# vLAR-group/OGC

Measured on AMD Instinct MI355X. Metric: point-clouds/sec (8192 pts) segnet fwd+bwd, higher is better.
Workload: dtype f32; 1 GPU; C4 KITTI-SF train_seg unsup: segnet_kitti fwd + OGC loss (dynamic+smooth+invariance) + bwd + Adam, 4 samples x 4 views x 8192 pts per GPU; n_point=8192, n_slot=10, parallelism=dp1, optimizer_stepped=True

## Files before the change

include/ogc_ops.h:

```cpp
#ifndef OGC_OPS_H
#define OGC_OPS_H

#ifdef __cplusplus
extern "C" {
#endif

typedef void *ogc_stream_t;
typedef unsigned short ogc_bf16_t;

enum {
    OGC_OK = 0,
    OGC_ERR_INVALID_ARG = -1,
    OGC_ERR_LAUNCH = -2,
    OGC_ERR_UNSUPPORTED = -3
};

#define OGC_VERSION 205
int ogc_version(void);
int ogc_distance_contracted(void);
int ogc_set_deterministic(int on);
int ogc_get_deterministic(void);
const char *ogc_last_error(void);

int ogc_furthest_point_sampling(int b, int n, int m, const float *xyz, float *temp,
                                int *idx, ogc_stream_t stream);

int ogc_furthest_point_sampling_chain(int b, int n, int m, const float *xyz, float *temp, int *idx,
                                      const int *ties_in, int *ties_out, ogc_stream_t stream);

int ogc_gather_points(int b, int c, int n, int npoints, const float *points, const int *idx,
                      float *out, ogc_stream_t stream);

int ogc_gather_points_grad(int b, int c, int n, int npoints, const float *grad_out,
                           const int *idx, float *grad_points, ogc_stream_t stream);

int ogc_knn(int b, int n, int m, int k, const float *unknown, const float *known,
            float *dist2, int *idx, ogc_stream_t stream);

int ogc_three_nn(int b, int n, int m, const float *unknown, const float *known, float *dist2,
                 int *idx, ogc_stream_t stream);

int ogc_three_interpolate(int b, int c, int m, int n, const float *points, const int *idx,
                          const float *weight, float *out, ogc_stream_t stream);

int ogc_three_interpolate_grad(int b, int c, int n, int m, const float *grad_out,
                               const int *idx, const float *weight, float *grad_points,
                               ogc_stream_t stream);

int ogc_group_points(int b, int c, int n, int npoints, int nsample, const float *points,
                     const int *idx, float *out, ogc_stream_t stream);

int ogc_group_points_grad(int b, int c, int n, int npoints, int nsample, const float *grad_out,
                          const int *idx, float *grad_points, ogc_stream_t stream);

int ogc_ball_query(int b, int n, int m, float radius, int nsample, const float *new_xyz,
                   const float *xyz, int *idx, ogc_stream_t stream);


int ogc_knn_clamped(int b, int n, int m, int k, float radius, const float *unknown,
                    const float *known, float *dist, int *idx, ogc_stream_t stream);

long long ogc_cell_grid_bytes(int b, int n);
int ogc_cell_grid_build(int b, int n, float radius, const float *xyz, void *grid, ogc_stream_t stream);
int ogc_ball_query_cells(int b, int n, float radius, int nsample, const float *xyz, const void *grid, float grid_radius, int *idx,
                         ogc_stream_t stream);
int ogc_knn_clamped_cells(int b, int n, int k, float radius, const float *xyz, void *grid, float grid_radius, float *dist, int *idx,
                          ogc_stream_t stream);

int ogc_adam_max_tensors(void);
int ogc_adam_chunk(void);
int ogc_adam_step(int n_tensors, int n_chunks, const long long *table, const int *chunks, const void *const *grad_ptrs,
                  float *step_snapshot, int *flag, double lr, double beta1, double beta2, double eps, double weight_decay,
                  ogc_stream_t stream);

int ogc_kabsch_rotation(int nb, const float *S, float *R, int *valid, ogc_stream_t stream);

int ogc_group_concat(int b, int c, int n, int npoints, int nsample, const float *xyz, const float *new_xyz,
                     const float *points, const int *idx, float *out, ogc_stream_t stream);

int ogc_group_concat_grad(int b, int c, int n, int npoints, int nsample, const float *grad_out, const int *idx,
                          float *grad_points, ogc_stream_t stream);

int ogc_group_linear_fwd(int b, int m, int n, int npoints, int nsample, int groups, const float *P, const int *idx,
                         const float *rel, const float *wx, float *y, double *stats, ogc_stream_t stream);
int ogc_group_linear_fwd_direct(int b, int m, int cf, int n, int npoints, int nsample, int groups, const float *feats,
                                const int *idx, const float *rel, const float *w, float *y, double *stats, ogc_stream_t stream);
int ogc_group_linear_fwd_direct_h(int b, int m, int cf, int n, int npoints, int nsample, int groups, const float *feats,
                                  const int *idx, const float *rel, const float *w, ogc_bf16_t *y, double *stats, ogc_stream_t stream);
int ogc_group_linear_bwd(int b, int m, int n, int npoints, int nsample, const float *grad_y, const int *idx,
                         const float *rel, float *grad_p, float *dwx, ogc_stream_t stream);

int ogc_group_reverse_chunk(int n, int npoints, int nsample);
int ogc_group_reverse(int b, int n, int npoints, int nsample, const int *idx, int *rev_start, unsigned short *rev_pos,
                      unsigned short *heads, ogc_stream_t stream);
int ogc_group_points_grad_rev(int b, int c, int n, int npoints, int nsample, const float *grad_out, const int *rev_start,
                              const unsigned short *rev_pos, const unsigned short *heads, float *grad_points,
                              ogc_stream_t stream);

int ogc_group_points_grad_rev_dwx(int b, int c, int n, int npoints, int nsample, const float *grad_out, const int *rev_start,
                                  const unsigned short *rev_pos, const unsigned short *heads, const float *rel,
// ... 61 lines not shown
                              ogc_stream_t stream);

int ogc_group_norm_maxpool_bwd_sparse(int b, int c, int p, int s, int groups, int relu, const float *x,
                                      const float *x_at_argmax, const float *gamma, const float *mean, const float *rstd, const float *out, const int *argmax,
                                      const float *grad_out, float *coef2, float *inj, float *grad_gamma,
                                      float *grad_beta, double *ws, ogc_stream_t stream);
int ogc_conv1x1_wgrad_moments_pooled(int b, int cin, int cout, int hw, int relu, int nsample, const float *y_prev,
                                     const float *pa, const float *pb, const float *y, const float *coef2,
                                     const float *inj, float *moments, ogc_stream_t stream);
int ogc_conv1x1_dgrad_adjoint_pooled(int b, int cin, int cout, int hw, int relu, int nsample, const float *w, const float *y,
                                     const float *coef2, const float *inj, const float *y_prev, const float *pa,
                                     const float *pb, const float *coef, float *grad_prev, ogc_stream_t stream);

int ogc_mlp_chain_pool_supported(int c0, int c1, int c2, int c3, int nsample);
int ogc_mlp_chain_pool(int b, int c0, int c1, int c2, int c3, int p, int nsample, const float *x, const float *wt1,
                       const float *b1, const float *wt2, const float *b2, const float *wt3, const float *b3, float *out,
                       ogc_stream_t stream);

int ogc_corr_layer_pool_supported(int cf, int c1, int c2, int c3, int nsample);
int ogc_corr_layer_pool(int b, int cf, int c1, int c2, int c3, int n1, int n2, int nsample, const float *pos1,
                        const float *pos2, const float *feat1, const float *feat2, const int *idx, const float *wt1,
                        const float *b1, const float *wt2, const float *b2, const float *wt3, const float *b3, float *out,
                        ogc_stream_t stream);

long long ogc_slot_masks_ws_floats(int b, int d, int n, int k);
int ogc_slot_masks_fwd(int b, int d, int n, int k, float temperature, const float *feats, const float *slots,
                       float *mask, ogc_stream_t stream);
int ogc_slot_masks_bwd(int b, int d, int n, int k, float temperature, const float *feats, const float *slots,
                       const float *mask, const float *grad_mask, float *grad_feats, float *grad_slots, float *ws,
                       ogc_stream_t stream);

int ogc_group_norm_stats_slots(void);
int ogc_group_norm_bwd_slots(void);
int ogc_group_norm_fwd(int b, int c, int hw, int groups, float eps, int relu, const float *x,
                       const float *gamma, const float *beta, float *y, float *mean, float *rstd,
                       double *ws, ogc_stream_t stream);
int ogc_group_norm_bwd(int b, int c, int hw, int groups, int relu, const float *x, const float *gamma,
                       const float *beta, const float *mean, const float *rstd, const float *grad_y,
                       float *grad_x, float *grad_gamma, float *grad_beta, double *ws, ogc_stream_t stream);

int ogc_group_norm_maxpool_fwd(int b, int c, int p, int s, int groups, float eps, int relu, const float *x,
                               const float *gamma, const float *beta, float *out, int *argmax, float *mean,
                               float *rstd, double *ws, ogc_stream_t stream);
int ogc_group_norm_maxpool_bwd(int b, int c, int p, int s, int groups, int relu, const float *x,
                               const float *gamma, const float *mean, const float *rstd, const float *out,
                               const int *argmax, const float *grad_out, float *grad_x, float *grad_gamma,
                               float *grad_beta, double *ws, ogc_stream_t stream);
int ogc_group_norm_maxpool_bwd_ext(int b, int c, int p, int s, int groups, int relu, const float *x,
                                   const float *x_at_argmax, const float *gamma, const float *mean, const float *rstd,
                                   const float *out, const int *argmax, const float *grad_out, float *grad_x,
                                   float *grad_gamma, float *grad_beta, double *ws, ogc_stream_t stream);

int ogc_batch_norm_fwd(int b, int c, int hw, float eps, int relu, int training, float momentum, const float *x,
                       const float *gamma, const float *beta, float *running_mean, float *running_var, float *y,
                       float *mean, float *rstd, double *ws, const double *stats, int slots, ogc_stream_t stream);
int ogc_batch_norm_bwd(int b, int c, int hw, int relu, int training, const float *x, const float *gamma,
                       const float *beta, const float *mean, const float *rstd, const float *grad_y, float *grad_x,
                       float *grad_gamma, float *grad_beta, double *ws, ogc_stream_t stream);
int ogc_batch_norm_maxpool_fwd(int b, int c, int p, int s, float eps, int relu, int training, float momentum,
                               const float *x, const float *gamma, const float *beta, float *running_mean,
                               float *running_var, float *out, int *argmax, float *mean, float *rstd, double *ws,
                               const double *stats, int slots, ogc_stream_t stream);
int ogc_batch_norm_maxpool_bwd(int b, int c, int p, int s, int relu, int training, const float *x, const float *gamma,
                               const float *mean, const float *rstd, const float *out, const int *argmax,
                               const float *grad_out, float *grad_x, float *grad_gamma, float *grad_beta, double *ws,
                               ogc_stream_t stream);

int ogc_conv1x1_wgrad(int b, int cin, int cout, int hw, const float *x, const float *dy, float *dw,
                      ogc_stream_t stream);

int ogc_conv1x1_gemm(int b, int M, int K, int hw, int transpose_a, const float *w, const float *in,
                     float *out, ogc_stream_t stream);

int ogc_conv1x1_gn_slots(void);
int ogc_conv1x1_gemm_stats_supported(int b, int M, int K, int hw, int affine);
int ogc_conv1x1_gemm_stream_supported(int b, int M, int K, int hw);
int ogc_conv1x1_gemm_any(int b, int M, int K, int hw, int transpose_a, const float *w, const float *in, float *out,
                         ogc_stream_t stream);

int ogc_set_matmul_precision(int bf16);
int ogc_conv1x1_gemm_gnstats(int b, int M, int K, int hw, int groups, const float *w, const float *in, float *out,
                             double *stats, ogc_stream_t stream);

int ogc_group_norm_coeffs(int b, int c, int hw, int groups, float eps, const float *x, const float *gamma,
                          const float *beta, const double *stats, int slots, double *ws, float *mean, float *rstd,
                          float *a, float *bb, ogc_stream_t stream);
int ogc_conv1x1_gemm_affine(int b, int M, int K, int hw, int relu, int groups, const float *w, const float *in,
                            const float *pa, const float *pb, float *out, double *stats, ogc_stream_t stream);
int ogc_conv1x1_wgrad_affine(int b, int cin, int cout, int hw, int relu, const float *x, const float *pa,
                             const float *pb, const float *dy, float *dw, ogc_stream_t stream);
int ogc_conv1x1_wgrad_affine_pooled(int b, int cin, int cout, int hw, int relu, int nsample, const float *x, const float *pa,
                                    const float *pb, const float *y, const float *coef2, const float *inj, float *dw,
                                    ogc_stream_t stream);
int ogc_conv1x1_dgrad_pooled(int b, int cin, int cout, int hw, int nsample, const float *w, const float *y, const float *coef2,
                             const float *inj, float *grad_z, ogc_stream_t stream);

int ogc_group_norm_fwd_stats(int b, int c, int hw, int groups, float eps, int relu, const float *x,
                             const float *gamma, const float *beta, float *y, float *mean, float *rstd,
                             const double *stats, int slots, ogc_stream_t stream);
int ogc_group_norm_maxpool_fwd_stats(int b, int c, int p, int s, int groups, float eps, int relu, const float *x,
                                     const float *gamma, const float *beta, float *out, int *argmax, float *mean,
                                     float *rstd, const double *stats, int slots, ogc_stream_t stream);

int ogc_conv1x1_gemm_affine_pool(int b, int M, int K, int hw, int relu, int groups, int nsample, const float *w,
                                 const float *in, const float *pa, const float *pb, const float *next_gamma,
                                 float *out, double *stats, float *yext, int *aext, ogc_stream_t stream);
int ogc_group_norm_pool_extremes(int b, int c, int p, int s, int groups, float eps, int relu, const float *yext,
                                 const int *aext, const float *gamma, const float *beta, float *out, int *argmax,
                                 float *mean, float *rstd, const double *stats, int slots, ogc_stream_t stream);

int ogc_chamfer_terms(int b, int n1, int n2, int p, const float *p1, const float *pc2, const int *idx12, const int *idx21,
                      float *dist1, float *dist2, ogc_stream_t stream);
int ogc_chamfer_terms_grad(int b, int n1, int n2, int p, const float *p1, const float *pc2, const int *idx12, const int *idx21,
                           const float *g1, const float *g2, float *grad_p1, ogc_stream_t stream);

int ogc_gather_xyz_pair(int b, int n, int m, const float *xyz, const int *idx, float *out, float *out_t, ogc_stream_t stream);
int ogc_flow_advance(int b, int n, float scale, const float *cur, const float *delta, const float *ref, float *out_delta,
                     float *out_new, float *out_new_t, float *out_flow, ogc_stream_t stream);
int ogc_linear_cn(int b, int cin, int cout, int n, const float *x, const float *weight, const float *bias, float *y,
                  ogc_stream_t stream);
int ogc_three_nn_weights(int b, int n, int mode, const float *dist2, float *weight, ogc_stream_t stream);
int ogc_soft_corr_flow(int b, int n1, int n2, int c, float support, const float *epsilon, const float *pc1, const float *pc2,
                       const float *f1, const float *f2, float *flow, ogc_stream_t stream);
int ogc_gru_reset(int b, int c, int cx, int n, int s, const float *rc, long long rc_batch_stride, const float *hx, float *out,
                  ogc_stream_t stream);
int ogc_gru_blend(int b, int c, int n, int s, const float *zc, long long zc_batch_stride, const float *qc,
                  long long qc_batch_stride, const float *h, long long h_batch_stride, float *out, ogc_stream_t stream);

int ogc_zero_arena_begin(void *base, int bytes, ogc_stream_t stream);
int ogc_zero_arena_end(void);

int ogc_group_linear_fwd_h(int b, int m, int n, int npoints, int nsample, int groups, const float *P, const int *idx,
                           const float *rel, const float *wx, ogc_bf16_t *y, double *stats, ogc_stream_t stream);
int ogc_group_linear_fwd_pt_h(int b, int m, int n, int npoints, int nsample, int groups, const float *Pt, const int *idx,
                              const float *rel, const float *wx, ogc_bf16_t *y, double *stats, ogc_stream_t stream);
int ogc_group_points_grad_rev_h(int b, int c, int n, int npoints, int nsample, const ogc_bf16_t *grad_out, const int *rev_start,
                                const unsigned short *rev_pos, const unsigned short *heads, float *grad_points,
                                ogc_stream_t stream);
int ogc_group_points_grad_rev_dwx_h(int b, int c, int n, int npoints, int nsample, const ogc_bf16_t *grad_out, const int *rev_start,
                                    const unsigned short *rev_pos, const unsigned short *heads, const float *rel,
                                    float *grad_points, float *dwx, ogc_stream_t stream);
int ogc_conv1x1_gemm_h(int b, int M, int K, int hw, int transpose_a, const float *w, const ogc_bf16_t *in, ogc_bf16_t *out,
                       ogc_stream_t stream);
int ogc_conv1x1_gemm_affine_h(int b, int M, int K, int hw, int relu, int groups, const float *w, const ogc_bf16_t *in,
                              const float *pa, const float *pb, ogc_bf16_t *out, double *stats, ogc_stream_t stream);
int ogc_conv1x1_gemm_affine_pool_h(int b, int M, int K, int hw, int relu, int groups, int nsample, const float *w,
                                   const ogc_bf16_t *in, const float *pa, const float *pb, const float *next_gamma,
                                   ogc_bf16_t *out, double *stats, float *yext, int *aext, ogc_stream_t stream);
int ogc_conv1x1_wgrad_xf_h(int b, int cin, int cout, int hw, const float *x, const ogc_bf16_t *dy, float *dw,
                           ogc_stream_t stream);
int ogc_conv1x1_wgrad_affine_h(int b, int cin, int cout, int hw, int relu, const ogc_bf16_t *x, const float *pa,
                               const float *pb, const ogc_bf16_t *dy, float *dw, ogc_stream_t stream);
int ogc_conv1x1_wgrad_affine_pooled_h(int b, int cin, int cout, int hw, int relu, int nsample, const ogc_bf16_t *x,
                                      const float *pa, const float *pb, const ogc_bf16_t *y, const float *coef2,
                                      const float *inj, float *dw, ogc_stream_t stream);
int ogc_conv1x1_dgrad_pooled_h(int b, int cin, int cout, int hw, int nsample, const float *w, const ogc_bf16_t *y,
                               const float *coef2, const float *inj, ogc_bf16_t *grad_z, ogc_stream_t stream);
int ogc_conv1x1_wgrad_moments_h(int b, int cin, int cout, int hw, int relu, const ogc_bf16_t *y_prev, const float *pa,
                                const float *pb, const ogc_bf16_t *grad_y, float *moments, ogc_stream_t stream);
int ogc_conv1x1_wgrad_moments_pooled_h(int b, int cin, int cout, int hw, int relu, int nsample, const ogc_bf16_t *y_prev,
                                       const float *pa, const float *pb, const ogc_bf16_t *y, const float *coef2,
                                       const float *inj, float *moments, ogc_stream_t stream);
int ogc_conv1x1_dgrad_adjoint_h(int b, int cin, int cout, int hw, int relu, const float *w, const ogc_bf16_t *grad_y,
                                const ogc_bf16_t *y_prev, const float *pa, const float *pb, const float *coef,
                                ogc_bf16_t *grad_prev, ogc_stream_t stream);
int ogc_conv1x1_dgrad_adjoint_pooled_h(int b, int cin, int cout, int hw, int relu, int nsample, const float *w,
// ... 16 lines not shown
```

ogc_amd/_lib.py:

```python
import ctypes
import os

_HERE = os.path.dirname(os.path.abspath(__file__))
FMAD = os.environ.get("OGC_FMAD", "0") == "1"
DETERMINISTIC = os.environ.get("OGC_DETERMINISTIC", "0") == "1"
LIB_PATH = os.path.join(_HERE, "csrc", "libogc_ops_fmad.so" if FMAD else "libogc_ops.so")

_vp = ctypes.c_void_p
_int = ctypes.c_int
_flt = ctypes.c_float
_dbl = ctypes.c_double
_ll = ctypes.c_longlong

SIGNATURES = {
    "ogc_set_deterministic": [_int],
    "ogc_group_linear_fwd_direct": [_int, _int, _int, _int, _int, _int, _int, _vp, _vp, _vp, _vp, _vp, _vp, _vp],
    "ogc_get_deterministic": [],
    "ogc_furthest_point_sampling": [_int, _int, _int, _vp, _vp, _vp, _vp],
    "ogc_furthest_point_sampling_chain": [_int, _int, _int, _vp, _vp, _vp, _vp, _vp, _vp],
    "ogc_gather_points": [_int, _int, _int, _int, _vp, _vp, _vp, _vp],
    "ogc_gather_points_grad": [_int, _int, _int, _int, _vp, _vp, _vp, _vp],
    "ogc_knn": [_int, _int, _int, _int, _vp, _vp, _vp, _vp, _vp],
    "ogc_three_nn": [_int, _int, _int, _vp, _vp, _vp, _vp, _vp],
    "ogc_three_interpolate": [_int, _int, _int, _int, _vp, _vp, _vp, _vp, _vp],
# ... 7 lines not shown
    "ogc_view_means_grad": [_int, _vp, _vp, _vp, _vp, _vp, _vp],
    "ogc_sum_ranges": [_int, _vp, _vp, _vp, _ll, _vp, _vp],
    "ogc_three_interpolate_grad_rev_bs": [_int, _int, _int, _int, _vp, _ll, _vp, _vp, _vp, _vp, _vp, _vp],
    "ogc_group_points_grad_rev": [_int, _int, _int, _int, _int, _vp, _vp, _vp, _vp, _vp, _vp],
    "ogc_group_points_grad_rev_dwx": [_int, _int, _int, _int, _int, _vp, _vp, _vp, _vp, _vp, _vp, _vp, _vp],
    "ogc_ball_query": [_int, _int, _int, _flt, _int, _vp, _vp, _vp, _vp],
    "ogc_knn_clamped": [_int, _int, _int, _int, _flt, _vp, _vp, _vp, _vp, _vp],
    "ogc_cell_grid_bytes": [_int, _int],
    "ogc_cell_grid_build": [_int, _int, _flt, _vp, _vp, _vp],
    "ogc_ball_query_cells": [_int, _int, _flt, _int, _vp, _vp, _flt, _vp, _vp],
    "ogc_knn_clamped_cells": [_int, _int, _int, _flt, _vp, _vp, _flt, _vp, _vp, _vp],
    "ogc_chamfer_terms": [_int, _int, _int, _int, _vp, _vp, _vp, _vp, _vp, _vp, _vp],
    "ogc_chamfer_terms_grad": [_int, _int, _int, _int, _vp, _vp, _vp, _vp, _vp, _vp, _vp, _vp],
    "ogc_gather_xyz_pair": [_int, _int, _int, _vp, _vp, _vp, _vp, _vp],
    "ogc_flow_advance": [_int, _int, _flt, _vp, _vp, _vp, _vp, _vp, _vp, _vp, _vp],
    "ogc_linear_cn": [_int, _int, _int, _int, _vp, _vp, _vp, _vp, _vp],
    "ogc_three_nn_weights": [_int, _int, _int, _vp, _vp, _vp],
    "ogc_soft_corr_flow": [_int, _int, _int, _int, _flt, _vp, _vp, _vp, _vp, _vp, _vp, _vp],
    "ogc_gru_reset": [_int, _int, _int, _int, _int, _vp, _ll, _vp, _vp, _vp],
    "ogc_gru_blend": [_int, _int, _int, _int, _vp, _ll, _vp, _ll, _vp, _ll, _vp, _vp],
    "ogc_zero_arena_begin": [_vp, _int, _vp],
    "ogc_zero_arena_end": [],
    "ogc_adam_max_tensors": [],
    "ogc_adam_chunk": [],
    "ogc_adam_step": [_int, _int, _vp, _vp, _vp, _vp, _vp, _dbl, _dbl, _dbl, _dbl, _dbl, _vp],
    "ogc_kabsch_rotation": [_int, _vp, _vp, _vp, _vp],
    "ogc_lsap_maximize": [_int, _int, _vp, _vp, _vp],
    "ogc_rigid_moments": [_int, _int, _int, _vp, _vp, _vp, _vp, _vp, _vp, _vp],
    "ogc_rigid_translation": [_int, _vp, _vp, _vp, _vp, _vp],
    "ogc_rigid_blend": [_int, _int, _int, _int, _int, _vp, _vp, _vp, _vp, _vp, _vp, _vp, _vp],
    "ogc_mask_iou": [_int, _int, _int, _vp, _vp, _vp, _vp, _vp],
    "ogc_matched_distance": [_int, _int, _int, _int, _int, _vp, _vp, _vp, _vp, _vp, _vp, _vp, _vp, _vp],
    "ogc_soft_nn_target": [_int, _int, _int, _int, _flt, _vp, _vp, _vp, _vp, _vp, _vp],
    "ogc_group_concat": [_int, _int, _int, _int, _int, _vp, _vp, _vp, _vp, _vp, _vp],
    "ogc_group_linear_fwd": [_int, _int, _int, _int, _int, _int, _vp, _vp, _vp, _vp, _vp, _vp, _vp],
    "ogc_group_linear_bwd": [_int, _int, _int, _int, _int, _vp, _vp, _vp, _vp, _vp, _vp],
    "ogc_group_concat_grad": [_int, _int, _int, _int, _int, _vp, _vp, _vp, _vp],
    "ogc_neighbour_consistency_fwd": [_int, _int, _int, _int, _int, _vp, _vp, _vp, _vp],
    "ogc_reverse_neighbours": [_int, _int, _int, _vp, _vp, _vp, _vp, _vp, _vp],
    "ogc_neighbour_consistency_bwd": [_int, _int, _int, _int, _int, _vp, _vp, _vp, _vp, _vp, _vp, _vp, _vp],
    "ogc_sym_eigvals": [_int, _int, _vp, _vp, _vp],
    "ogc_group_norm_fwd": [_int, _int, _int, _int, _flt, _int, _vp, _vp, _vp, _vp, _vp, _vp, _vp, _vp],
    "ogc_group_norm_bwd": [_int, _int, _int, _int, _int, _vp, _vp, _vp, _vp, _vp, _vp, _vp, _vp, _vp, _vp, _vp],
    "ogc_group_norm_maxpool_fwd": [_int, _int, _int, _int, _int, _flt, _int, _vp, _vp, _vp, _vp, _vp, _vp, _vp, _vp, _vp],
    "ogc_conv1x1_gemm": [_int, _int, _int, _int, _int, _vp, _vp, _vp, _vp],
    "ogc_attention_fwd": [_int, _int, _int, _int, _int, _flt, _vp, _int, _vp, _int, _vp, _int, _vp, _vp, _vp],
    "ogc_attention_bwd": [_int, _int, _int, _int, _int, _flt, _vp, _int, _vp, _int, _vp, _int, _vp, _vp, _vp, _vp, _int,
                          _vp, _int, _vp, _int, _vp],
    "ogc_conv1x1_gemm_affine_pool": [_int, _int, _int, _int, _int, _int, _int, _vp, _vp, _vp, _vp, _vp, _vp, _vp, _vp, _vp,
                                     _vp],
    "ogc_group_norm_pool_extremes": [_int, _int, _int, _int, _int, _flt, _int, _vp, _vp, _vp, _vp, _vp, _vp, _vp, _vp, _vp,
                                     _int, _vp],
    "ogc_small_linear_fwd": [_int, _int, _int, _vp, _vp, _vp, _vp, _vp],
    "ogc_small_linear_bwd": [_int, _int, _int, _vp, _vp, _vp, _vp, _vp, _vp, _vp],
    "ogc_conv1x1_wgrad_moments": [_int, _int, _int, _int, _int, _vp, _vp, _vp, _vp, _vp, _vp],
    "ogc_gn_moments_combine": [_int, _int, _int, _int, _int, _vp, _vp, _vp, _vp, _vp, _vp, _vp, _vp, _vp, _vp, _vp, _vp],
    "ogc_conv1x1_dgrad_adjoint": [_int, _int, _int, _int, _int, _vp, _vp, _vp, _vp, _vp, _vp, _vp, _vp],
    "ogc_group_norm_maxpool_bwd_sparse": [_int, _int, _int, _int, _int, _int, _vp, _vp, _vp, _vp, _vp, _vp, _vp, _vp, _vp, _vp,
                                          _vp, _vp, _vp, _vp],
    "ogc_group_norm_maxpool_bwd_ext": [_int, _int, _int, _int, _int, _int, _vp, _vp, _vp, _vp, _vp, _vp, _vp, _vp, _vp, _vp,
                                       _vp, _vp, _vp],
    "ogc_conv1x1_wgrad_moments_pooled": [_int, _int, _int, _int, _int, _int, _vp, _vp, _vp, _vp, _vp, _vp, _vp, _vp],
    "ogc_conv1x1_dgrad_adjoint_pooled": [_int, _int, _int, _int, _int, _int, _vp, _vp, _vp, _vp, _vp, _vp, _vp, _vp, _vp, _vp],
    "ogc_mlp_chain_pool_supported": [_int, _int, _int, _int, _int],
    "ogc_mlp_chain_pool": [_int, _int, _int, _int, _int, _int, _int, _vp, _vp, _vp, _vp, _vp, _vp, _vp, _vp, _vp],
    "ogc_corr_layer_pool_supported": [_int, _int, _int, _int, _int],
    "ogc_corr_layer_pool": [_int, _int, _int, _int, _int, _int, _int, _int, _vp, _vp, _vp, _vp, _vp, _vp, _vp, _vp, _vp, _vp,
                            _vp, _vp, _vp],
    "ogc_slot_masks_ws_floats": [_int, _int, _int, _int],
    "ogc_slot_masks_fwd": [_int, _int, _int, _int, _flt, _vp, _vp, _vp, _vp],
    "ogc_slot_masks_bwd": [_int, _int, _int, _int, _flt, _vp, _vp, _vp, _vp, _vp, _vp, _vp, _vp],
    "ogc_conv1x1_gn_slots": [],
    "ogc_conv1x1_gemm_stats_supported": [_int, _int, _int, _int, _int],
    "ogc_conv1x1_gemm_stream_supported": [_int, _int, _int, _int],
    "ogc_conv1x1_gemm_any": [_int, _int, _int, _int, _int, _vp, _vp, _vp, _vp],
    "ogc_set_matmul_precision": [_int],
    "ogc_group_norm_stats_slots": [],
    "ogc_group_norm_bwd_slots": [],
    "ogc_group_norm_coeffs": [_int, _int, _int, _int, _flt, _vp, _vp, _vp, _vp, _int, _vp, _vp, _vp, _vp, _vp, _vp],
    "ogc_conv1x1_gemm_affine": [_int, _int, _int, _int, _int, _int, _vp, _vp, _vp, _vp, _vp, _vp, _vp],
    "ogc_conv1x1_wgrad_affine": [_int, _int, _int, _int, _int, _vp, _vp, _vp, _vp, _vp, _vp],
    "ogc_conv1x1_wgrad_affine_pooled": [_int, _int, _int, _int, _int, _int, _vp, _vp, _vp, _vp, _vp, _vp, _vp, _vp],
    "ogc_conv1x1_dgrad_pooled": [_int, _int, _int, _int, _int, _vp, _vp, _vp, _vp, _vp, _vp],
    "ogc_batch_norm_fwd": [_int, _int, _int, _flt, _int, _int, _flt, _vp, _vp, _vp, _vp, _vp, _vp, _vp, _vp, _vp, _vp,
                           _int, _vp],
    "ogc_batch_norm_bwd": [_int, _int, _int, _int, _int, _vp, _vp, _vp, _vp, _vp, _vp, _vp, _vp, _vp, _vp, _vp],
    "ogc_batch_norm_maxpool_fwd": [_int, _int, _int, _int, _flt, _int, _int, _flt, _vp, _vp, _vp, _vp, _vp, _vp, _vp,
                                   _vp, _vp, _vp, _vp, _int, _vp],
    "ogc_batch_norm_maxpool_bwd": [_int, _int, _int, _int, _int, _int, _vp, _vp, _vp, _vp, _vp, _vp, _vp, _vp, _vp,
                                   _vp, _vp, _vp],
    "ogc_conv1x1_gemm_gnstats": [_int, _int, _int, _int, _int, _vp, _vp, _vp, _vp, _vp],
    "ogc_group_norm_fwd_stats": [_int, _int, _int, _int, _flt, _int, _vp, _vp, _vp, _vp, _vp, _vp, _vp, _int, _vp],
    "ogc_group_norm_maxpool_fwd_stats": [_int, _int, _int, _int, _int, _flt, _int, _vp, _vp, _vp, _vp, _vp, _vp, _vp,
                                         _vp, _int, _vp],
    "ogc_conv1x1_wgrad": [_int, _int, _int, _int, _vp, _vp, _vp, _vp],
    "ogc_group_norm_maxpool_bwd": [_int, _int, _int, _int, _int, _int, _vp, _vp, _vp, _vp, _vp, _vp, _vp, _vp, _vp, _vp,
                                   _vp, _vp],
}

for _n in ("ogc_group_linear_fwd", "ogc_group_points_grad_rev", "ogc_conv1x1_gemm", "ogc_conv1x1_gemm_affine",
           "ogc_conv1x1_gemm_affine_pool", "ogc_conv1x1_wgrad_affine", "ogc_conv1x1_wgrad_affine_pooled",
           "ogc_conv1x1_dgrad_pooled", "ogc_conv1x1_wgrad_moments", "ogc_conv1x1_wgrad_moments_pooled",
           "ogc_conv1x1_dgrad_adjoint", "ogc_conv1x1_dgrad_adjoint_pooled", "ogc_group_norm_bwd",
           "ogc_group_norm_maxpool_bwd_sparse", "ogc_group_points_grad_rev_dwx"):
    SIGNATURES[_n + "_h"] = SIGNATURES[_n]
SIGNATURES["ogc_group_linear_fwd_direct_h"] = SIGNATURES["ogc_group_linear_fwd_direct"]
SIGNATURES["ogc_conv1x1_wgrad_xf_h"] = SIGNATURES["ogc_conv1x1_wgrad"]
SIGNATURES["ogc_group_linear_fwd_pt_h"] = SIGNATURES["ogc_group_linear_fwd"]

HEADER_VERSION = 205
_lib = None
_fns = {}


class OgcOpsError(RuntimeError):
    pass


def load():
    global _lib
    if _lib is None:
        if not os.path.exists(LIB_PATH):
            raise OgcOpsError(
                "libogc_ops.so not found at %s — build it with `python ogc_amd/csrc/build.py` "
                "(there is no CPU fallback)" % LIB_PATH)
        L = ctypes.CDLL(LIB_PATH)
        for name, argtypes in SIGNATURES.items():
            fn = getattr(L, name)
            fn.argtypes = argtypes
            fn.restype = _int
        L.ogc_version.restype = _int
        if L.ogc_version() != HEADER_VERSION:
            raise OgcOpsError("libogc_ops.so at %s is version %d, this package binds version %d of include/ogc_ops.h — rebuild it "
                              "with `python ogc_amd/csrc/build.py --force`" % (LIB_PATH, L.ogc_version(), HEADER_VERSION))
        L.ogc_distance_contracted.restype = _int
        if bool(L.ogc_distance_contracted()) != FMAD:
            raise OgcOpsError("%s evaluates distances %s, OGC_FMAD asked for the other form" %
                              (LIB_PATH, "contracted (fma)" if L.ogc_distance_contracted() else "un-contracted"))
        L.ogc_slot_masks_ws_floats.restype = ctypes.c_longlong
        L.ogc_cell_grid_bytes.restype = ctypes.c_longlong
        L.ogc_last_error.restype = ctypes.c_char_p
        L.ogc_set_deterministic(1 if DETERMINISTIC else 0)
        _lib = L
    return _lib


def set_deterministic(on):
    global DETERMINISTIC
    DETERMINISTIC = bool(on)
    load().ogc_set_deterministic(1 if on else 0)


CALL_COUNTS = None

ROCTX_NAMES = {
    "ogc_furthest_point_sampling": "K1 furthest_point_sampling", "ogc_furthest_point_sampling_chain": "K1 furthest_point_sampling (chain)",
    "ogc_gather_points": "K2 gather_points", "ogc_gather_points_grad": "K3 gather_points_grad",
    "ogc_knn": "K4 knn", "ogc_knn_clamped": "K4 knn (+ sqrt + radius clamp)", "ogc_knn_clamped_cells": "K4 knn (shared cell grid)",
    "ogc_three_nn": "K5 three_nn", "ogc_three_interpolate": "K6 three_interpolate",
    "ogc_three_interpolate_grad": "K7 three_interpolate_grad", "ogc_three_interpolate_grad_rev": "K7 three_interpolate_grad (gather form)",
    "ogc_three_interpolate_grad_rev_bs": "K7 three_interpolate_grad (gather form)",
    "ogc_group_points": "K8 group_points", "ogc_group_points_grad": "K9 group_points_grad",
    "ogc_group_points_grad_rev": "K9 group_points_grad (gather form)",
    "ogc_ball_query": "K10 ball_query", "ogc_ball_query_cells": "K10 ball_query (shared cell grid)",
}
_roctx = None


def _roctx_lib():
    global _roctx
    if _roctx is None:
        _roctx = False
        if os.environ.get("OGC_ROCTX", "0") == "1":
            for name in ("librocprofiler-sdk-roctx.so", "libroctx64.so"):
                try:
                    lib = ctypes.CDLL(os.path.join(os.environ.get("ROCM_PATH", "/opt/rocm"), "lib", name))
                    lib.roctxRangePushA.argtypes = [ctypes.c_char_p]
                    lib.roctxRangePushA.restype = ctypes.c_int
                    lib.roctxRangePop.restype = ctypes.c_int
                    _roctx = lib
                    break
                except (OSError, AttributeError):
                    continue
    return _roctx


def call(name, *args):
    if CALL_COUNTS is not None:
        CALL_COUNTS[name] += 1
    fn = _fns.get(name)
    if fn is None:
        fn = _fns[name] = getattr(load(), name)
    tx = _roctx_lib()
# ... 13 lines not shown
```

ogc_amd/csrc/build.py:

```python
import os
import subprocess
import sys
from concurrent.futures import ThreadPoolExecutor

HERE = os.path.dirname(os.path.abspath(__file__))
SOURCES = ["api.hip", "det.hip", "knn.hip", "ball_query.hip", "fps.hip", "gather_group.hip", "interpolate.hip", "kabsch.hip", "small_solvers.hip", "neighbour_loss.hip", "soft_nn.hip", "seg_loss.hip", "group_norm.hip", "batch_norm.hip", "grid.hip", "conv1x1.hip", "conv1x1_h.hip", "conv1x1_wgrad.hip", "attention.hip", "slot_masks.hip", "small_linear.hip", "loss_glue.hip", "mlp_chain.hip", "gn_fused_bwd.hip", "adam.hip", "gemm_chunk.hip", "chamfer.hip", "flow_step.hip"]
HEADERS = ["ogc_common.h", "grid.h", "conv_stage.h", "conv1x1_shared.h", "act_io.h", "conv1x1_epilogue.h", os.path.join("..", "..", "include", "ogc_ops.h")]
LIB = os.path.join(HERE, "libogc_ops.so")
FMAD_SOURCES = ["knn.hip", "ball_query.hip", "fps.hip", "grid.hip"]
LIB_FMAD = os.path.join(HERE, "libogc_ops_fmad.so")
HIPCC = os.environ.get("HIPCC", "/opt/rocm/bin/hipcc")
FLAGS = [
    "--offload-arch=gfx950", "-O3", "-std=c++17", "-fPIC",
    "-ffp-contract=off",
    "-munsafe-fp-atomics",
    "-mllvm", "-amdgpu-mfma-vgpr-form=1",
    "-Wall", "-Wno-unused-function",
]


def _newer(target, deps):
    if not os.path.exists(target):
        return True
    t = os.path.getmtime(target)
    return any(os.path.getmtime(d) > t for d in deps)


def build(force=False, verbose=False):
    hdrs = [os.path.join(HERE, h) for h in HEADERS] + [os.path.abspath(__file__)]
    objs, objs_fmad, jobs = [], [], []
    for s in SOURCES:
        src = os.path.join(HERE, s)
        obj = os.path.join(HERE, s.replace(".hip", ".o"))
        objs.append(obj)
        if force or _newer(obj, [src] + hdrs):
            jobs.append([HIPCC] + FLAGS + ["-c", src, "-o", obj])
        if s in FMAD_SOURCES:
            obj_f = os.path.join(HERE, s.replace(".hip", ".fmad.o"))
            objs_fmad.append(obj_f)
            if force or _newer(obj_f, [src] + hdrs):
                jobs.append([HIPCC] + FLAGS + ["-DOGC_FMAD=1", "-c", src, "-o", obj_f])
        else:
            objs_fmad.append(obj)

    def run(cmd):
        if verbose:
            print(" ".join(cmd), flush=True)
        subprocess.check_call(cmd)

    with ThreadPoolExecutor(max_workers=min(8, max(1, len(jobs)))) as ex:
        list(ex.map(run, jobs))
    if force or jobs or _newer(LIB, objs):
        run([HIPCC, "--offload-arch=gfx950", "-shared", "-fPIC", "-o", LIB] + objs)
    if force or jobs or _newer(LIB_FMAD, objs_fmad):
        run([HIPCC, "--offload-arch=gfx950", "-shared", "-fPIC", "-o", LIB_FMAD] + objs_fmad)
    return LIB


if __name__ == "__main__":
    print(build(force="--force" in sys.argv, verbose="--verbose" in sys.argv))
```

ogc_amd/csrc/conv1x1.hip:

```cpp
#include "conv1x1_shared.h"
#include "act_io.h"
#include "conv1x1_epilogue.h"

int ogc_g_matmul_bf16 = 0;


namespace {


template <bool TRANSPOSE_A, int KQ, bool STATS, bool PRO, bool BF, bool POOL = false, typename IT = float, typename OT = float>
__global__ __launch_bounds__(WG_WAVES *OGC_WAVE) void conv1x1_gemm_kernel(int M, int K, int hw, int groups,
                                                                          const float *__restrict__ w,
                                                                          const IT *__restrict__ in,
                                                                          OT *__restrict__ out,
                                                                          double *__restrict__ stats,
                                                                          const float *__restrict__ pa,
                                                                          const float *__restrict__ pb, int pro_relu,
                                                                          PoolOut pool = PoolOut()) {
    extern __shared__ __attribute__((aligned(16))) float a_lds[];
    __shared__ double s_stats[STATS ? 64 : 1];
    __shared__ __attribute__((aligned(16))) float s_sign[POOL ? 64 : 4];
    const int lane = threadIdx.x & 63, wave = threadIdx.x >> 6;
    const int j = lane & 15, kk = lane >> 4;
    const int b = blockIdx.y;
    const int p0 = (blockIdx.x * WG_WAVES + wave) * 64;
    const int Kq = (K + 3) >> 2, a_ld = ogc_a_ld(Kq);
    const bool live = p0 < hw;
    const IT *inb = in + (size_t)b * K * hw;
    OT *outb = out + (size_t)b * M * hw;
    if (STATS && threadIdx.x < 2 * groups) s_stats[threadIdx.x] = 0.0;

    float4 xin[KQ];
#pragma unroll
    for (int q = 0; q < KQ; ++q) {
        const int row = q * 4 + kk;
        xin[q] = (live && q < Kq && row < K) ? ogc_ld4(inb + (size_t)row * hw + p0 + 4 * j) : make_float4(0.f, 0.f, 0.f, 0.f);
    }
    if (PRO) {
        constexpr int CH = 8;
#pragma unroll
        for (int q0 = 0; q0 < KQ; q0 += CH) {
            float ca[CH], cb[CH];
#pragma unroll
            for (int u = 0; u < CH; ++u) {
                const int q = q0 + u, row = q * 4 + kk;
                const bool have = q < KQ && live && q < Kq && row < K;
                ca[u] = have ? pa[(size_t)b * K + row] : 0.f;
                cb[u] = have ? pb[(size_t)b * K + row] : 0.f;
            }
#pragma unroll
            for (int u = 0; u < CH; ++u) {
                const int q = q0 + u;
                if (q < KQ) {
                    float4 v = xin[q];
                    v.x = fmaf(ca[u], v.x, cb[u]); v.y = fmaf(ca[u], v.y, cb[u]);
                    v.z = fmaf(ca[u], v.z, cb[u]); v.w = fmaf(ca[u], v.w, cb[u]);
                    if (pro_relu) { v.x = fmaxf(v.x, 0.f); v.y = fmaxf(v.y, 0.f); v.z = fmaxf(v.z, 0.f); v.w = fmaxf(v.w, 0.f); }
                    xin[q] = v;
                }
            }
        }
    }
    constexpr int GQ = (KQ + 3) / 4;
    v4s xb[BF ? GQ : 1][4];
    if constexpr (BF) {
#pragma unroll
        for (int g = 0; g < GQ; ++g) {
            float4 r[4];
#pragma unroll
            for (int i = 0; i < 4; ++i) r[i] = 4 * g + i < KQ ? xin[4 * g + i] : make_float4(0.f, 0.f, 0.f, 0.f);
            xb[g][0] = ogc_pack_bf16(r[0].x, r[1].x, r[2].x, r[3].x);
            xb[g][1] = ogc_pack_bf16(r[0].y, r[1].y, r[2].y, r[3].y);
            xb[g][2] = ogc_pack_bf16(r[0].z, r[1].z, r[2].z, r[3].z);
            xb[g][3] = ogc_pack_bf16(r[0].w, r[1].w, r[2].w, r[3].w);
        }
    }
    const int cpg = STATS ? M / groups : 1;
    for (int m0 = 0; m0 < M; m0 += 64) {
        __syncthreads();
        if constexpr (BF) {
            v4s *a_bf = reinterpret_cast<v4s *>(a_lds);
            const int Gq = (Kq + 3) >> 2;
            for (int t = threadIdx.x; t < Gq * 256; t += WG_WAVES * OGC_WAVE) {
                const int kr = t & 3, mi = (t >> 2) & 63, g = t >> 8;
                const int m = m0 + mi;
// ... 71 lines not shown
#pragma unroll
        for (int q = 0; q < KQ; ++q) {
            if (q < Kq) {
                float av[4];
#pragma unroll
                for (int a = 0; a < 4; ++a) av[a] = a_lds[(a * 16 + j) * a_ld + q * 4 + kk];
#pragma unroll
                for (int a = 0; a < 4; ++a) {
                    if (a < nblk) {
                        acc[a][0] = __builtin_amdgcn_mfma_f32_16x16x4f32(av[a], xin[q].x, acc[a][0], 0, 0, 0);
                        acc[a][1] = __builtin_amdgcn_mfma_f32_16x16x4f32(av[a], xin[q].y, acc[a][1], 0, 0, 0);
                        acc[a][2] = __builtin_amdgcn_mfma_f32_16x16x4f32(av[a], xin[q].z, acc[a][2], 0, 0, 0);
                        acc[a][3] = __builtin_amdgcn_mfma_f32_16x16x4f32(av[a], xin[q].w, acc[a][3], 0, 0, 0);
                    }
                }
            }
        }
        }
        if (live) {
            if constexpr (sizeof(OT) == 2 && (STATS || POOL)) {
#pragma unroll
                for (int a = 0; a < 4; ++a)
#pragma unroll
                    for (int c = 0; c < 4; ++c)
#pragma unroll
                        for (int r = 0; r < 4; ++r) acc[a][c][r] = ogc_as_stored<OT>(acc[a][c][r]);
            }
#pragma unroll
            for (int a = 0; a < 4; ++a)
#pragma unroll
                for (int r = 0; r < 4; ++r) {
                    const int m = m0 + a * 16 + kk * 4 + r;
                    if (m < M) {
                        const float4 o = make_float4(acc[a][0][r], acc[a][1][r], acc[a][2][r], acc[a][3][r]);
                        ogc_st4(outb + (size_t)m * hw + p0 + 4 * j, o);
                    }
                }
            if constexpr (POOL) {
                const int centres = hw / pool.s;
                const int centre = (p0 + 4 * j) / pool.s;
                const size_t o0 = ((size_t)b * M + m0 + kk * 4) * centres + centre;
                if (pool.s == 64) ogc_pool_extremes_epilogue<16>(acc, nblk, s_sign, j, kk, m0, M, centres, 64, pool.yext + o0, pool.aext + o0);
                else if (pool.s == 32) ogc_pool_extremes_epilogue<8>(acc, nblk, s_sign, j, kk, m0, M, centres, 32, pool.yext + o0, pool.aext + o0);
                else ogc_pool_extremes_epilogue<4>(acc, nblk, s_sign, j, kk, m0, M, centres, 16, pool.yext + o0, pool.aext + o0);
            }
            if (STATS) {
#pragma unroll
                for (int a = 0; a < 4; ++a) {
                    if (a < nblk) {
                        float sm = 0.f, sq = 0.f;
#pragma unroll
                        for (int r = 0; r < 4; ++r)
#pragma unroll
                            for (int c = 0; c < 4; ++c) {
                                const float v = acc[a][c][r];
                                sm += v;
                                sq += v * v;
                            }
                        sm += ogc_dpp_f32<0xB1>(sm); sq += ogc_dpp_f32<0xB1>(sq);
                        sm += ogc_dpp_f32<0x4E>(sm); sq += ogc_dpp_f32<0x4E>(sq);
                        sm += ogc_dpp_f32<0x141>(sm); sq += ogc_dpp_f32<0x141>(sq);
                        sm += ogc_dpp_f32<0x140>(sm); sq += ogc_dpp_f32<0x140>(sq);
                        const int m = m0 + a * 16 + kk * 4;
                        if (j == 0 && m < M) {
                            const int g = m / cpg;
                            atomicAdd(&s_stats[2 * g], (double)sm);
                            atomicAdd(&s_stats[2 * g + 1], (double)sq);
                        }
                    }
                }
            }
        }
    }
    if (STATS) {
        __syncthreads();
        if (threadIdx.x < 2 * groups) {
            const int slot = blockIdx.x % GN_SLOTS;
            double *dst = stats + ((size_t)slot * gridDim.y + b) * 2 * groups;
            atomicAdd(dst + threadIdx.x, s_stats[threadIdx.x]);
        }
    }
}

template <int KQ, bool PRO, bool EXACT, bool STATS = false, bool POOL = false, bool DUAL = false, bool TRANS = false>
__global__ __launch_bounds__(WG_WAVES *OGC_WAVE, DUAL ? 2 : 1) void conv1x1_gemm_stream_kernel(int M, int K, int hw, int ntiles,
                                                                                 const float *__restrict__ w,
                                                                                 const float *__restrict__ in,
                                                                                 float *__restrict__ out,
                                                                                 const float *__restrict__ pa,
                                                                                 const float *__restrict__ pb, int pro_relu,
                                                                                 int groups = 1, int nbatch = 1,
                                                                                 double *__restrict__ stats = nullptr,
                                                                                 PoolOut pool = PoolOut()) {
    extern __shared__ __attribute__((aligned(16))) float a_lds[];
    const int lane = threadIdx.x & 63, wave = __builtin_amdgcn_readfirstlane(threadIdx.x >> 6);
    const int j = lane & 15, kk = lane >> 4;
    const int Kq = (K + 3) >> 2, Mt = (M + 63) >> 6, a_ld = ogc_a_ld(Kq);
    const int tiles_per_img = hw >> 6;
    for (int mt = 0; mt < Mt; ++mt)
        ogc_stage_weight_tile<TRANS, WG_WAVES>(a_lds + (size_t)mt * 64 * a_ld, w, mt * 64, M, K, Kq);
    float *sgn_all = a_lds + (size_t)Mt * 64 * a_ld + (PRO ? WG_WAVES * 2 * FW_KQ_MAX * 4 : 0) + WG_WAVES * 4 * 16 * 2 * 2;
    if constexpr (POOL) {
        for (int t = threadIdx.x; t < Mt * 64; t += WG_WAVES * OGC_WAVE) sgn_all[t] = (t < M && pool.sign[t] < 0.f) ? -1.f : 1.f;
    }
    __syncthreads();
    const int nw = gridDim.x * WG_WAVES;
    const unsigned off_main = (unsigned)(kk * hw + 4 * j);
    const unsigned off_last = (unsigned)(min(kk, K - 1 - (Kq - 1) * 4) * hw + 4 * j);
    auto load_tile = [&](int t, float4(&x)[KQ]) {
        t = min(t, ntiles - 1);
        const int b = t / tiles_per_img, p0 = (t - b * tiles_per_img) * 64;
        const float *inb = in + (size_t)b * K * hw + p0;
#pragma unroll
        for (int q = 0; q < KQ; ++q)
            if (EXACT || q < Kq) {
                const float *rowq = inb + (size_t)(q * 4) * hw;
                x[q] = *reinterpret_cast<const float4 *>(rowq + ((EXACT ? q == KQ - 1 : q == Kq - 1) ? off_last : off_main));
            }
    };
    float *cw = a_lds + (size_t)Mt * 64 * a_ld + wave * (2 * KQ * 4);
    int coef_b = -1;
    double *sacc = reinterpret_cast<double *>(a_lds + (size_t)Mt * 64 * a_ld + (PRO ? WG_WAVES * 2 * FW_KQ_MAX * 4 : 0)) +
                   wave * (4 * 16 * 2);
    int stat_b = -1;
    auto flush_stats = [&]() {
        if constexpr (STATS) {
            if (stat_b >= 0) {
                const int cpg = M / groups;
                double *dst = stats + ((size_t)(blockIdx.x % GN_SLOTS) * nbatch + stat_b) * 2 * groups;
                if (lane < Mt * 16) {
                    const int m = (lane >> 4) * 64 + ((lane >> 2) & 3) * 16 + (lane & 3) * 4;
                    if (m < M) {
                        unsafeAtomicAdd(dst + 2 * (m / cpg), sacc[2 * lane]);
                        unsafeAtomicAdd(dst + 2 * (m / cpg) + 1, sacc[2 * lane + 1]);
                    }
                }
            }
            if (lane < 64) { sacc[2 * lane] = 0.0; sacc[2 * lane + 1] = 0.0; }
            __builtin_amdgcn_wave_barrier();
        }
    };
    auto compute_store = [&](int t, float4(&x)[KQ]) {
        const int b = t / tiles_per_img, p0 = (t - b * tiles_per_img) * 64;
        if constexpr (STATS) {
            if (b != stat_b) { flush_stats(); stat_b = b; }
        }
        if (PRO) {
            if (b != coef_b) {
                coef_b = b;
                for (int r = lane; r < KQ * 4; r += OGC_WAVE) {
                    cw[r] = r < K ? pa[(size_t)b * K + r] : 0.f;
                    cw[KQ * 4 + r] = r < K ? pb[(size_t)b * K + r] : 0.f;
                }
                __builtin_amdgcn_wave_barrier();
            }
#pragma unroll
            for (int q = 0; q < KQ; ++q) {
                if (EXACT || q < Kq) {
                    const float ca = cw[q * 4 + kk], cb = cw[KQ * 4 + q * 4 + kk];
                    float4 v = x[q];
                    v.x = fmaf(ca, v.x, cb); v.y = fmaf(ca, v.y, cb);
                    v.z = fmaf(ca, v.z, cb); v.w = fmaf(ca, v.w, cb);
                    if (pro_relu) { v.x = fmaxf(v.x, 0.f); v.y = fmaxf(v.y, 0.f); v.z = fmaxf(v.z, 0.f); v.w = fmaxf(v.w, 0.f); }
                    x[q] = v;
                }
            }
        }
        float *outb = out + (size_t)b * M * hw + p0;
        const unsigned off_out = (unsigned)(kk * 4 * hw + 4 * j);
        for (int mt = 0; mt < Mt; ++mt) {
            const float *at = a_lds + (size_t)mt * 64 * a_ld;
            const int nblk = EXACT ? 4 : min(4, (M - mt * 64 + 15) >> 4);
            v4f acc[4][4];
#pragma unroll
            for (int a = 0; a < 4; ++a)
#pragma unroll
                for (int c = 0; c < 4; ++c) acc[a][c] = (v4f){0.f, 0.f, 0.f, 0.f};
#pragma unroll
            for (int q = 0; q < KQ; ++q) {
                if (EXACT || q < Kq) {
                    float av[4];
#pragma unroll
                    for (int a = 0; a < 4; ++a) av[a] = at[(a * 16 + j) * a_ld + q * 4 + kk];
#pragma unroll
                    for (int a = 0; a < 4; ++a) {
                        if (EXACT || a < nblk) {
                            acc[a][0] = __builtin_amdgcn_mfma_f32_16x16x4f32(av[a], x[q].x, acc[a][0], 0, 0, 0);
                            acc[a][1] = __builtin_amdgcn_mfma_f32_16x16x4f32(av[a], x[q].y, acc[a][1], 0, 0, 0);
                            acc[a][2] = __builtin_amdgcn_mfma_f32_16x16x4f32(av[a], x[q].z, acc[a][2], 0, 0, 0);
                            acc[a][3] = __builtin_amdgcn_mfma_f32_16x16x4f32(av[a], x[q].w, acc[a][3], 0, 0, 0);
                        }
                    }
                }
            }
#pragma unroll
            for (int a = 0; a < 4; ++a)
#pragma unroll
                for (int r = 0; r < 4; ++r) {
                    const int m0 = mt * 64 + a * 16 + r;
                    if (EXACT || m0 + kk * 4 < M)
                        *reinterpret_cast<float4 *>(outb + (size_t)m0 * hw + off_out) =
                            make_float4(acc[a][0][r], acc[a][1][r], acc[a][2][r], acc[a][3][r]);
                }
            if constexpr (POOL) {
                const int m0p = mt * 64;
                const int centres = hw / pool.s;
                const int centre = (p0 + 4 * j) / pool.s;
                const size_t o0 = ((size_t)b * M + m0p + kk * 4) * centres + centre;
                const float *sg = sgn_all + m0p;
                if (pool.s == 64) ogc_pool_extremes_epilogue<16>(acc, nblk, sg, j, kk, m0p, M, centres, 64, pool.yext + o0, pool.aext + o0);
                else if (pool.s == 32) ogc_pool_extremes_epilogue<8>(acc, nblk, sg, j, kk, m0p, M, centres, 32, pool.yext + o0, pool.aext + o0);
                else ogc_pool_extremes_epilogue<4>(acc, nblk, sg, j, kk, m0p, M, centres, 16, pool.yext + o0, pool.aext + o0);
            }
            if constexpr (STATS) {
#pragma unroll
                for (int a = 0; a < 4; ++a) {
                    if (EXACT || a < nblk) {
                        float sm = 0.f, sq = 0.f;
#pragma unroll
                        for (int r = 0; r < 4; ++r)
#pragma unroll
                            for (int c = 0; c < 4; ++c) {
                                const float v = acc[a][c][r];
                                sm += v;
                                sq += v * v;
                            }
                        sm += ogc_dpp_f32<0xB1>(sm); sq += ogc_dpp_f32<0xB1>(sq);
                        sm += ogc_dpp_f32<0x4E>(sm); sq += ogc_dpp_f32<0x4E>(sq);
                        sm += ogc_dpp_f32<0x141>(sm); sq += ogc_dpp_f32<0x141>(sq);
                        sm += ogc_dpp_f32<0x140>(sm); sq += ogc_dpp_f32<0x140>(sq);
                        if (j == 0) {
                            const int slot = (mt * 4 + a) * 4 + kk;
                            sacc[2 * slot] += (double)sm;
                            sacc[2 * slot + 1] += (double)sq;
                        }
                    }
                }
            }
        }
    };
    const int per = (ntiles + nw - 1) / nw;
    int t = (blockIdx.x * WG_WAVES + wave) * per;
    const int t_end = min(ntiles, t + per);
    if (STATS) flush_stats();
    if constexpr (DUAL) {
        float4 x1[KQ];
        for (; t < t_end; ++t) {
            load_tile(t, x1);
            compute_store(t, x1);
        }
        if (STATS) flush_stats();
        return;
    }
    float4 xa[KQ], xb[KQ];
    if (t < t_end) {
        load_tile(t, xa);
        for (; t + 1 < t_end; t += 2) {
            load_tile(t + 1, xb);
            compute_store(t, xa);
            load_tile(t + 2, xa);
            compute_store(t + 1, xb);
        }
        if (t < t_end) compute_store(t, xa);
    }
    if (STATS) flush_stats();
}

bool gemm_stream_eligible(int b, int M, int K, int hw, bool pro, bool pool = false, bool any_precision = false) {
    const int Kq = (K + 3) / 4, Mt = (M + 63) / 64;
    const long long ntiles = (long long)b * (hw / 64);
    const size_t lds = ((size_t)Mt * 64 * ogc_a_ld(Kq) + (pro ? WG_WAVES * 2 * FW_KQ_MAX * 4 : 0)) * sizeof(float) +
                       WG_WAVES * 4 * 16 * 2 * sizeof(double) + (pool ? (size_t)Mt * 64 * sizeof(float) : 0);
    static const bool off = getenv("OGC_GEMM_STREAM") && getenv("OGC_GEMM_STREAM")[0] == '0';
    return !(off || (g_matmul_bf16 && !any_precision) || (hw & 63) != 0 || Kq <= 25 || Kq > FW_KQ_MAX || lds > 156 * 1024 || ntiles < 2048 ||
             ntiles >= (1ll << 31));
}

template <bool PRO, bool STATS = false, bool POOL = false, bool TRANS = false>
bool gemm_stream_launch(int b, int M, int K, int hw, const float *w, const float *in, float *out, const float *pa,
                        const float *pb, int pro_relu, hipStream_t s, int groups = 1, double *stats = nullptr,
                        PoolOut pool = PoolOut()) {
    const int Kq = (K + 3) / 4, Mt = (M + 63) / 64;
    const long long ntiles = (long long)b * (hw / 64);
    const size_t lds = ((size_t)Mt * 64 * ogc_a_ld(Kq) + (PRO ? WG_WAVES * 2 * FW_KQ_MAX * 4 : 0)) * sizeof(float) +
                       WG_WAVES * 4 * 16 * 2 * sizeof(double) + (POOL ? (size_t)Mt * 64 * sizeof(float) : 0);
    if (!gemm_stream_eligible(b, M, K, hw, PRO, POOL, STATS) || lds > 156 * 1024) return false;
    const int wgs = (int)(ntiles / WG_WAVES < 256 ? ntiles / WG_WAVES : 256);
#define OGC_STREAM_D(KQV, EX, DU, WGS)                                                                                       \
    do {                                                                                                                     \
        static bool raised = false;                                                                                          \
        const void *fn = reinterpret_cast<const void *>(&conv1x1_gemm_stream_kernel<KQV, PRO, EX, STATS, POOL, DU, TRANS>);         \
        if (!raised) {                                                                                                       \
            if (hipFuncSetAttribute(fn, hipFuncAttributeMaxDynamicSharedMemorySize, 156 * 1024) != hipSuccess) return false;  \
            raised = true;                                                                                                   \
        }                                                                                                                    \
        hipLaunchKernelGGL((conv1x1_gemm_stream_kernel<KQV, PRO, EX, STATS, POOL, DU, TRANS>), dim3(WGS), dim3(WG_WAVES * OGC_WAVE), \
                           lds, s, M, K, hw, (int)ntiles, w, in, out, pa, pb, pro_relu, groups, b, stats, pool);             \
    } while (0)
    static const bool dual_on = !(getenv("OGC_GEMM_STREAM_DUAL") && getenv("OGC_GEMM_STREAM_DUAL")[0] == '0');
    const bool dual = dual_on && !POOL && 2 * (lds + 1024) <= 156 * 1024 && ntiles >= 4096;
    const int wgs2 = (int)(ntiles / WG_WAVES < 512 ? ntiles / WG_WAVES : 512);
#define OGC_STREAM(KQV, EX)                                                                                                  \
    do {                                                                                                                     \
        if (dual) OGC_STREAM_D(KQV, EX, true, wgs2);                                                                         \
        else OGC_STREAM_D(KQV, EX, false, wgs);                                                                              \
    } while (0)
    const bool full_rows = M % 64 == 0;
    if (Kq == 32 && full_rows) OGC_STREAM(32, true);
    else if (Kq == 33 && full_rows) OGC_STREAM(33, true);
    else if (Kq <= 33) OGC_STREAM(33, false);
    else OGC_STREAM(40, false);
#undef OGC_STREAM
#undef OGC_STREAM_D
    return true;
}

template <bool T, bool STATS, bool PRO, bool POOL = false, typename AT = float>
int gemm_launch(int b, int M, int K, int hw, int groups, const float *w, const AT *in, AT *out, double *stats,
                const float *pa, const float *pb, int pro_relu, hipStream_t s, PoolOut pool = PoolOut()) {
    const int Kq = (K + 3) / 4;
    constexpr bool F32 = sizeof(AT) == 4;
    if constexpr (F32 && !T && (!POOL || (STATS && PRO))) {
        static const bool wide_fp32 = [] { const char *e = getenv("OGC_BF16_WIDE_STATS"); return e && e[0] == '1'; }();
        if ((!g_matmul_bf16 || (STATS && wide_fp32)) &&
            gemm_stream_launch<PRO, STATS, POOL>(b, M, K, hw, w, in, out, pa, pb, pro_relu, s, groups, stats, pool))
            return OGC_OK;
    }
    if constexpr (F32 && T && !STATS && !PRO && !POOL) {
        if (!g_matmul_bf16 && gemm_stream_launch<false, false, false, true>(b, M, K, hw, w, in, out, pa, pb, pro_relu, s))
            return OGC_OK;
    }
    if constexpr (F32) {
        if (!g_matmul_bf16 && ogc_gemm32_launch(T, STATS, PRO, POOL, b, M, K, hw, groups, w, in, out, stats, pa, pb, pro_relu, s,
                                                pool.sign, pool.yext, pool.aext, pool.s))
            return OGC_OK;
    }
    if constexpr (!F32) {
        if (ogc_gemm16_launch(T, STATS, PRO, POOL, b, M, K, hw, groups, w, in, out, stats, pa, pb, pro_relu, s, pool.sign, pool.yext,
                              pool.aext, pool.s))
            return OGC_OK;
    }
    const size_t lds = (size_t)64 * ogc_a_ld(Kq) * sizeof(float);
    dim3 grid(ogc_divup(hw, 64 * WG_WAVES), b);
#define OGC_GEMM(KQV)                                                                                                  \
    do {                                                                                                               \
        if constexpr (!F32)                                                                                            \
            hipLaunchKernelGGL((conv1x1_gemm_kernel<T, KQV, STATS, PRO, true, POOL, AT, AT>), grid,                     \
                               dim3(WG_WAVES * OGC_WAVE), lds, s, M, K, hw, groups, w, in, out, stats, pa, pb, pro_relu, pool); \
        else if (g_matmul_bf16)                                                                                        \
            hipLaunchKernelGGL((conv1x1_gemm_kernel<T, KQV, STATS, PRO, true, POOL>), grid, dim3(WG_WAVES * OGC_WAVE), \
                               lds, s, M, K, hw, groups, w, in, out, stats, pa, pb, pro_relu, pool);                   \
        else                                                                                                           \
            hipLaunchKernelGGL((conv1x1_gemm_kernel<T, KQV, STATS, PRO, false, POOL>), grid, dim3(WG_WAVES * OGC_WAVE), \
                               lds, s, M, K, hw, groups, w, in, out, stats, pa, pb, pro_relu, pool);                   \
    } while (0)
    if (Kq <= 2) OGC_GEMM(2);
    else if (Kq <= 8) OGC_GEMM(8);
    else if (Kq <= 16) OGC_GEMM(16);
    else if (Kq <= 25) OGC_GEMM(25);
    else if (POOL && !g_matmul_bf16) return OGC_ERR_UNSUPPORTED;
    else {
        if (Kq <= 33) OGC_GEMM(33);
        else OGC_GEMM(40);
    }
#undef OGC_GEMM
    return OGC_OK;
}

template <typename AT>
int gemm_check(const char *name, int b, int M, int K, int hw, const float *w, const AT *in, const AT *out) {
    OGC_REQUIRE(b >= 0 && M >= 1 && K >= 1 && hw >= 1, "%s: bad shape", name);
    OGC_REQUIRE(w && in && out, "%s: null pointer", name);
    if ((hw & 63) != 0 || K > 4 * FW_KQ_MAX || (((uintptr_t)in | (uintptr_t)out) & ogc_act_mask<AT>()) != 0) {
        ogc_set_error("%s: needs hw %% 64 == 0, K <= %d and 16-byte aligned tensors (hw=%d, K=%d)", name,
                      4 * FW_KQ_MAX, hw, K);
        return OGC_ERR_UNSUPPORTED;
    }
    if (sizeof(AT) == 2 && !g_matmul_bf16) {
        ogc_set_error("%s: 16-bit activations need ogc_set_matmul_precision(1)", name);
        return OGC_ERR_UNSUPPORTED;
    }
    OGC_REQUIRE((long long)M * hw < (1ll << 31) && (long long)K * hw < (1ll << 31) && b <= 65535,
                "%s: one sample exceeds 32-bit indexing", name);
    return OGC_OK;
}

}

namespace {
template <typename AT>
int gemm_plain_impl(const char *name, int b, int M, int K, int hw, int transpose_a, const float *w, const AT *in, AT *out,
                    ogc_stream_t stream) {
    const int rc = gemm_check(name, b, M, K, hw, w, in, out);
    if (rc != OGC_OK) return rc;
    if (b == 0) return OGC_OK;
    if (transpose_a)
        gemm_launch<true, false, false, false, AT>(b, M, K, hw, 1, w, in, out, nullptr, nullptr, nullptr, 0, (hipStream_t)stream);
    else
        gemm_launch<false, false, false, false, AT>(b, M, K, hw, 1, w, in, out, nullptr, nullptr, nullptr, 0, (hipStream_t)stream);
    OGC_CHECK_LAUNCH(name);
    return OGC_OK;
}
}

extern "C" int ogc_conv1x1_gemm(int b, int M, int K, int hw, int transpose_a, const float *w, const float *in,
                                float *out, ogc_stream_t stream) {
    return gemm_plain_impl<float>("ogc_conv1x1_gemm", b, M, K, hw, transpose_a, w, in, out, stream);
}

extern "C" int ogc_conv1x1_gemm_h(int b, int M, int K, int hw, int transpose_a, const float *w, const ogc_bf16_t *in,
                                  ogc_bf16_t *out, ogc_stream_t stream) {
    return gemm_plain_impl<ogc_bf16>("ogc_conv1x1_gemm_h", b, M, K, hw, transpose_a, w, in, out, stream);
}

extern "C" int ogc_conv1x1_gn_slots(void) { return GN_SLOTS; }

extern "C" int ogc_conv1x1_gemm_stats_supported(int b, int M, int K, int hw, int affine) {
    if (b < 1 || M < 1 || K < 1 || hw < 1) return 0;
    return (K <= 100 || g_matmul_bf16 || gemm_stream_eligible(b, M, K, hw, affine != 0, false, true)) ? 1 : 0;
}

extern "C" int ogc_conv1x1_gemm_stream_supported(int b, int M, int K, int hw) {
    if (b < 1 || M < 1 || K < 1 || hw < 1) return 0;
    return gemm_stream_eligible(b, M, K, hw, false) ? 1 : 0;
}

extern "C" int ogc_set_matmul_precision(int bf16) {
    const int previous = g_matmul_bf16;
    g_matmul_bf16 = bf16 ? 1 : 0;
    return previous;
}

extern "C" int ogc_conv1x1_gemm_gnstats(int b, int M, int K, int hw, int groups, const float *w, const float *in,
                                        float *out, double *stats, ogc_stream_t stream) {
    const int rc = gemm_check<float>("ogc_conv1x1_gemm_gnstats", b, M, K, hw, w, in, out);
    if (rc != OGC_OK) return rc;
    OGC_REQUIRE(stats, "ogc_conv1x1_gemm_gnstats: null pointer");
    if (groups < 1 || groups > 32 || M % groups != 0 || (M / groups) % 4 != 0) {
        ogc_set_error("ogc_conv1x1_gemm_gnstats: needs 1 <= groups <= 32 and (M / groups) %% 4 == 0 (M=%d, groups=%d)", M,
                      groups);
        return OGC_ERR_UNSUPPORTED;
    }
    if (K > 100 && !g_matmul_bf16 && !gemm_stream_eligible(b, M, K, hw, false, false, true)) {
        ogc_set_error("ogc_conv1x1_gemm_gnstats: not profitable for K > 100 (K=%d) on this shape; use ogc_conv1x1_gemm", K);
        return OGC_ERR_UNSUPPORTED;
    }
    if (b == 0) return OGC_OK;
    if (ogc_zero_async(stats, sizeof(double) * 2 * GN_SLOTS * (size_t)b * groups, (hipStream_t)stream) != hipSuccess) {
        ogc_set_error("ogc_conv1x1_gemm_gnstats: memset failed");
        return OGC_ERR_LAUNCH;
    }
// ... 93 lines not shown
```

ogc_amd/csrc/gemm_chunk.hip:

```cpp
#include <stdlib.h>

#include "ogc_common.h"
#include "act_io.h"
#include "conv1x1_shared.h"

namespace {

constexpr int GC_WAVES = 4;

__device__ __forceinline__ v4s gc_pack_bf16(float a, float b, float c, float d) { return ogc_pack_bf16_rr(a, b, c, d); }

template <int RB, int KQ, bool SPLIT_M, bool TRANS, bool POOLED = false, int KA = 1, typename AT = float, bool BF = false,
          bool TAB = false>
__global__ __launch_bounds__(GC_WAVES *OGC_WAVE, 2) void gemm_chunk_kernel(int M, int K, int hw, const float *__restrict__ w,
                                                                         const AT *__restrict__ in,
                                                                         AT *__restrict__ out,
                                                                         const float2 *__restrict__ coef2 = nullptr,
                                                                         const float2 *__restrict__ inj = nullptr,
                                                                         int s_shift = 0) {
    constexpr int KC = 4 * KQ, KCA = KC * KA, LD = 4 * ((KQ * KA) | 1);
    constexpr int MT = SPLIT_M ? 64 * RB : 16 * RB;
    constexpr int PER = (MT * KCA) / (GC_WAVES * OGC_WAVE);
    static_assert((MT * KCA) % (GC_WAVES * OGC_WAVE) == 0 && PER >= 1 && (KA == 1 || KA == 2), "staging split");
    extern __shared__ __attribute__((aligned(16))) float gc_lds[];
    const int t = threadIdx.x, lane = t & 63, wave = __builtin_amdgcn_readfirstlane(t >> 6);
    const int j = lane & 15, kk = lane >> 4;
    const int b = blockIdx.z;
    const int m0 = blockIdx.y * MT;
    const int wrow = SPLIT_M ? wave * 16 * RB : 0;
    const int p0 = SPLIT_M ? blockIdx.x * 64 : (blockIdx.x * GC_WAVES + wave) * 64;
    const bool active = p0 < hw;
    const int pl = active ? p0 : 0;
    const int nblk = min(RB, (M - m0 - wrow + 15) >> 4);
    const AT *inb = in + (size_t)b * K * hw + pl + 4 * j;
    const int nchunks = (K + KC - 1) / KC;

    v4f acc[RB][4];
#pragma unroll
    for (int a = 0; a < RB; ++a)
#pragma unroll
        for (int c = 0; c < 4; ++c) acc[a][c] = (v4f){0.f, 0.f, 0.f, 0.f};

    auto load_a = [&](int k0, float(&av)[PER]) {
#pragma unroll
        for (int i = 0; i < PER; ++i) {
            const int e = t + i * (GC_WAVES * OGC_WAVE);
            int mi, ki;
            if (TRANS) { mi = e % MT; ki = e / MT; } else { mi = e / KCA; ki = e % KCA; }
            const int m = m0 + mi, k = k0 + ki;
            const bool ok = m < M && k < K;
            const int mc = min(m, M - 1), kc = min(k, K - 1);
            const float v = TRANS ? w[(size_t)kc * M + mc] : w[(size_t)mc * K + kc];
            av[i] = ok ? v : 0.f;
        }
    };
    auto store_a = [&](float *dst, const float(&av)[PER]) {
#pragma unroll
        for (int i = 0; i < PER; ++i) {
            const int e = t + i * (GC_WAVES * OGC_WAVE);
            int mi, ki;
            if (TRANS) { mi = e % MT; ki = e / MT; } else { mi = e / KCA; ki = e % KCA; }
            dst[mi * LD + ki] = av[i];
        }
    };
    constexpr int NP = (POOLED && !TAB) ? KQ : 1;
    const int centres = hw >> s_shift;
    const int my_centre = (pl + 4 * j) >> s_shift, jpos = (pl + 4 * j) & ((1 << s_shift) - 1);
    const int cpw = 64 >> s_shift;
    float4 *tab = reinterpret_cast<float4 *>(gc_lds + 2 * MT * LD) + (size_t)wave * K * cpw;
    if constexpr (POOLED && TAB) {
        for (int e = lane; e < K * cpw; e += OGC_WAVE) {
            const int row = e / cpw, centre = (pl >> s_shift) + (e - row * cpw);
            const float2 c2v = coef2[(size_t)b * K + row];
            const float2 jj = centre < centres ? inj[((size_t)b * K + row) * centres + centre] : make_float2(0.f, __int_as_float(-1));
            tab[e] = make_float4(c2v.x, c2v.y, jj.x, jj.y);
        }
        __builtin_amdgcn_wave_barrier();
    }
    const int mine_c = (4 * j) >> s_shift;
    auto load_in = [&](int k0, float4(&xv)[KQ], float2(&cc)[NP], float2(&jv)[NP]) {
#pragma unroll
        for (int q = 0; q < KQ; ++q) {
            const int k = min(k0 + 4 * q + kk, K - 1);
            xv[q] = ogc_ld4(inb + (size_t)k * hw);
            if constexpr (POOLED && !TAB) {
                cc[q] = coef2[(size_t)b * K + k];
                jv[q] = inj[((size_t)b * K + k) * centres + my_centre];
            }
        }
    };
    auto rebuild = [&](int k0, float4(&xv)[KQ], const float2(&cc)[NP], const float2(&jv)[NP]) {
        if constexpr (POOLED && TAB) {
#pragma unroll
            for (int q = 0; q < KQ; ++q) {
                const float4 te = tab[min(k0 + 4 * q + kk, K - 1) * cpw + mine_c];
                const int rel = __float_as_int(te.w) - jpos;
                xv[q].x = fmaf(te.x, xv[q].x, te.y) + (rel == 0 ? te.z : 0.f);
                xv[q].y = fmaf(te.x, xv[q].y, te.y) + (rel == 1 ? te.z : 0.f);
                xv[q].z = fmaf(te.x, xv[q].z, te.y) + (rel == 2 ? te.z : 0.f);
                xv[q].w = fmaf(te.x, xv[q].w, te.y) + (rel == 3 ? te.z : 0.f);
            }
        } else if constexpr (POOLED) {
#pragma unroll
            for (int q = 0; q < KQ; ++q) {
                const int rel = __float_as_int(jv[q].y) - jpos;
                const float ag = jv[q].x;
                xv[q].x = fmaf(cc[q].x, xv[q].x, cc[q].y) + (rel == 0 ? ag : 0.f);
                xv[q].y = fmaf(cc[q].x, xv[q].y, cc[q].y) + (rel == 1 ? ag : 0.f);
                xv[q].z = fmaf(cc[q].x, xv[q].z, cc[q].y) + (rel == 2 ? ag : 0.f);
                xv[q].w = fmaf(cc[q].x, xv[q].w, cc[q].y) + (rel == 3 ? ag : 0.f);
            }
        }
        if (k0 + KC > K) {
#pragma unroll
            for (int q = 0; q < KQ; ++q)
                if (k0 + 4 * q + kk >= K) xv[q] = make_float4(0.f, 0.f, 0.f, 0.f);
        }
    };
    auto compute = [&](const float *a_lds, const float4(&xv)[KQ], int koff = 0) {
        if constexpr (BF) {
            static_assert(!BF || KQ % 4 == 0, "bf16 operands: whole groups of four row quads per input chunk");
#pragma unroll
            for (int g = 0; g < KQ / 4; ++g) {
                const float4 v0 = xv[4 * g], v1 = xv[4 * g + 1], v2 = xv[4 * g + 2], v3 = xv[4 * g + 3];
                const v4s bx = gc_pack_bf16(v0.x, v1.x, v2.x, v3.x);
                const v4s by = gc_pack_bf16(v0.y, v1.y, v2.y, v3.y);
                const v4s bz = gc_pack_bf16(v0.z, v1.z, v2.z, v3.z);
                const v4s bw = gc_pack_bf16(v0.w, v1.w, v2.w, v3.w);
                const float *ar = a_lds + (wrow + j) * LD + koff + 16 * g + kk;
#pragma unroll
                for (int a = 0; a < RB; ++a) {
                    const v4s av = gc_pack_bf16(ar[a * 16 * LD], ar[a * 16 * LD + 4], ar[a * 16 * LD + 8], ar[a * 16 * LD + 12]);
                    acc[a][0] = __builtin_amdgcn_mfma_f32_16x16x16bf16_1k(av, bx, acc[a][0], 0, 0, 0);
                    acc[a][1] = __builtin_amdgcn_mfma_f32_16x16x16bf16_1k(av, by, acc[a][1], 0, 0, 0);
                    acc[a][2] = __builtin_amdgcn_mfma_f32_16x16x16bf16_1k(av, bz, acc[a][2], 0, 0, 0);
                    acc[a][3] = __builtin_amdgcn_mfma_f32_16x16x16bf16_1k(av, bw, acc[a][3], 0, 0, 0);
                }
            }
        } else {
#pragma unroll
            for (int q = 0; q < KQ; ++q) {
                const float bx = xv[q].x, by = xv[q].y, bz = xv[q].z, bw = xv[q].w;
#pragma unroll
                for (int a = 0; a < RB; ++a) {
                    const float av = a_lds[(wrow + a * 16 + j) * LD + koff + q * 4 + kk];
                    acc[a][0] = __builtin_amdgcn_mfma_f32_16x16x4f32(av, bx, acc[a][0], 0, 0, 0);
                    acc[a][1] = __builtin_amdgcn_mfma_f32_16x16x4f32(av, by, acc[a][1], 0, 0, 0);
                    acc[a][2] = __builtin_amdgcn_mfma_f32_16x16x4f32(av, bz, acc[a][2], 0, 0, 0);
                    acc[a][3] = __builtin_amdgcn_mfma_f32_16x16x4f32(av, bw, acc[a][3], 0, 0, 0);
                }
            }
        }
    };

    float *buf0 = gc_lds, *buf1 = gc_lds + MT * LD;
    float4 x0[KQ], x1[KQ];
    float2 c0[NP], c1[NP], j0[NP], j1[NP];
    float a_next[PER];
    load_a(0, a_next);
    load_in(0, x0, c0, j0);
    store_a(buf0, a_next);
    __syncthreads();
    const bool work = nblk > 0;
    if constexpr (KA == 2) {
        const int npairs = (nchunks + 1) / 2;
        for (int p = 0; p < npairs; ++p) {
            const bool more = p + 1 < npairs;
            if (more) load_a((p + 1) * KCA, a_next);
            load_in((2 * p + 1) * KC, x1, c1, j1);
            rebuild(2 * p * KC, x0, c0, j0);
            if (work) compute(buf0, x0, 0);
            if (more) load_in((2 * p + 2) * KC, x0, c0, j0);
            rebuild((2 * p + 1) * KC, x1, c1, j1);
            if (work) compute(buf0, x1, KC);
            if (more) store_a(buf1, a_next);
            __syncthreads();
            float *tmp = buf0; buf0 = buf1; buf1 = tmp;
        }
    } else
    for (int i = 0; i < nchunks; i += 2) {
        const bool more1 = i + 1 < nchunks, more2 = i + 2 < nchunks;
        if (more1) {
            load_a((i + 1) * KC, a_next);
            load_in((i + 1) * KC, x1, c1, j1);
        }
        rebuild(i * KC, x0, c0, j0);
        if (work) compute(buf0, x0);
        if (more1) store_a(buf1, a_next);
        __syncthreads();
        if (!more1) break;
        if (more2) {
            load_a((i + 2) * KC, a_next);
            load_in((i + 2) * KC, x0, c0, j0);
        }
        rebuild((i + 1) * KC, x1, c1, j1);
        if (work) compute(buf1, x1);
        if (more2) store_a(buf0, a_next);
        __syncthreads();
    }
    if (!active) return;
    AT *ob = out + (size_t)b * M * hw + p0 + 4 * j;
#pragma unroll
    for (int a = 0; a < RB; ++a) {
        if (a < nblk) {
#pragma unroll
            for (int r = 0; r < 4; ++r) {
                const int m = m0 + wrow + a * 16 + kk * 4 + r;
                if (m < M) ogc_st4(ob + (size_t)m * hw, make_float4(acc[a][0][r], acc[a][1][r], acc[a][2][r], acc[a][3][r]));
            }
        }
    }
}

template <int RB, int KQ, bool SPLIT_M, int KA = 1>
void gemm_chunk_launch(int b, int M, int K, int hw, int transpose_a, const float *w, const float *in, float *out,
                       hipStream_t s) {
    constexpr int MT = SPLIT_M ? 64 * RB : 16 * RB;
    const size_t lds = (size_t)2 * MT * 4 * ((KQ * KA) | 1) * sizeof(float);
    dim3 grid(SPLIT_M ? hw / 64 : ogc_divup(hw, 64 * GC_WAVES), ogc_divup(M, MT), b);
#define GC_GO(TR, BFV)                                                                                                           \
    hipLaunchKernelGGL((gemm_chunk_kernel<RB, KQ, SPLIT_M, TR, false, KA, float, BFV>), grid, dim3(GC_WAVES * OGC_WAVE), lds, s, M, K, \
                       hw, w, in, out, nullptr, nullptr, 0)
    if (ogc_g_matmul_bf16) {
        if (transpose_a) GC_GO(true, true);
        else GC_GO(false, true);
    } else {
        if (transpose_a) GC_GO(true, false);
        else GC_GO(false, false);
    }
#undef GC_GO
}

}

extern "C" int ogc_conv1x1_gemm_any(int b, int M, int K, int hw, int transpose_a, const float *w, const float *in, float *out,
                                    ogc_stream_t stream) {
    OGC_REQUIRE(b >= 0 && M >= 1 && K >= 1 && hw >= 1, "ogc_conv1x1_gemm_any: bad shape");
    OGC_REQUIRE(w && in && out, "ogc_conv1x1_gemm_any: null pointer");
    if ((hw & 63) != 0 || (((uintptr_t)in | (uintptr_t)out) & 15) != 0) {
        ogc_set_error("ogc_conv1x1_gemm_any: needs hw %% 64 == 0 and 16-byte aligned tensors (hw=%d)", hw);
        return OGC_ERR_UNSUPPORTED;
    }
    OGC_REQUIRE((long long)M * hw < (1ll << 31) && (long long)K * hw < (1ll << 31) && b <= 65535,
                "ogc_conv1x1_gemm_any: one sample exceeds 32-bit indexing");
    if (b == 0) return OGC_OK;
    hipStream_t s = (hipStream_t)stream;
    const long long tiles = (long long)b * (hw / 64);
#define GC_CASE(RBV, KQV, SPLIT)                                                              \
    case RBV: gemm_chunk_launch<RBV, KQV, SPLIT>(b, M, K, hw, transpose_a, w, in, out, s); break
    if (tiles >= 4096) {
        const int ntile = ogc_divup(M, 128), rb = ogc_divup(M, 16 * ntile);
        switch (rb) {
            GC_CASE(1, 8, false); GC_CASE(2, 8, false); GC_CASE(3, 8, false); GC_CASE(4, 8, false);
            GC_CASE(5, 8, false); GC_CASE(6, 8, false); GC_CASE(7, 4, false);
            default: {
                static const char *kq = getenv("OGC_GEMM_CHUNK_KQ");
                if (kq && kq[0] == '4') gemm_chunk_launch<8, 4, false>(b, M, K, hw, transpose_a, w, in, out, s);
                else gemm_chunk_launch<8, 4, false, 2>(b, M, K, hw, transpose_a, w, in, out, s);
            }
        }
    } else {
        const bool same_rows = 128 * ogc_divup(M, 128) == 64 * ogc_divup(M, 64);
        const int rb = (M > 64 && same_rows && tiles * ogc_divup(M, 128) >= 512) ? 2 : 1;
        switch (rb) {
            GC_CASE(2, 8, true);
            default: gemm_chunk_launch<1, 8, true>(b, M, K, hw, transpose_a, w, in, out, s);
        }
    }
#undef GC_CASE
    OGC_CHECK_LAUNCH("ogc_conv1x1_gemm_any");
    return OGC_OK;
}

namespace {
template <typename AT>
int dgrad_pooled_impl(int b, int cin, int cout, int hw, int nsample, const float *w, const AT *y, const float *coef2,
                      const float *inj, AT *grad_z, ogc_stream_t stream) {
    constexpr bool BF = sizeof(AT) == 2;
    OGC_REQUIRE(b >= 0 && cin >= 1 && cout >= 1 && hw >= 1, "ogc_conv1x1_dgrad_pooled: bad shape");
    OGC_REQUIRE(w && y && coef2 && inj && grad_z, "ogc_conv1x1_dgrad_pooled: null pointer");
    const int sh = nsample == 16 ? 4 : nsample == 32 ? 5 : nsample == 64 ? 6 : -1;
    if (sh < 0 || hw % nsample != 0 || (hw & 63) != 0 || (long long)b * (hw / 64) < 1024 ||
        (((uintptr_t)y | (uintptr_t)grad_z) & ogc_act_mask<AT>()) != 0 || (((uintptr_t)coef2 | (uintptr_t)inj) & 7) != 0 ||
        (BF && !ogc_g_matmul_bf16)) {
        ogc_set_error("ogc_conv1x1_dgrad_pooled: needs nsample in {16, 32, 64} dividing hw, hw %% 64 == 0, >= 1024 tiles of 64 "
                      "positions and aligned tensors (hw=%d, nsample=%d, b=%d)", hw, nsample, b);
        return OGC_ERR_UNSUPPORTED;
    }
    OGC_REQUIRE((long long)cin * hw < (1ll << 31) && (long long)cout * hw < (1ll << 31) && b <= 65535,
                "ogc_conv1x1_dgrad_pooled: one sample exceeds 32-bit indexing");
    if (b == 0) return OGC_OK;
    hipStream_t s = (hipStream_t)stream;
    const float2 *c2 = reinterpret_cast<const float2 *>(coef2), *ij = reinterpret_cast<const float2 *>(inj);
    const int M = cin, K = cout;
    static const bool tab_off = [] { const char *e = getenv("OGC_DGRAD_POOLED_TAB"); return e && e[0] == '0'; }();
    const size_t tab_bytes = (size_t)GC_WAVES * K * (64 >> sh) * sizeof(float4);
    const bool tab = !tab_off && tab_bytes <= 24 * 1024;
    if (M <= 64) {
        constexpr int RB = 4, KQ = 4, KA = 2;
        dim3 grid(ogc_divup(hw, 64 * GC_WAVES), ogc_divup(M, 16 * RB), b);
        const size_t lds = (size_t)2 * 16 * RB * 4 * ((KQ * KA) | 1) * sizeof(float);
        if (tab)
            hipLaunchKernelGGL((gemm_chunk_kernel<RB, KQ, false, true, true, KA, AT, BF, true>), grid, dim3(GC_WAVES * OGC_WAVE),
                               lds + tab_bytes, s, M, K, hw, w, y, grad_z, c2, ij, sh);
        else
            hipLaunchKernelGGL((gemm_chunk_kernel<RB, KQ, false, true, true, KA, AT, BF>), grid, dim3(GC_WAVES * OGC_WAVE), lds, s, M,
                               K, hw, w, y, grad_z, c2, ij, sh);
    } else {
        constexpr int RB = 8, KQ = 4;
        dim3 grid(ogc_divup(hw, 64 * GC_WAVES), ogc_divup(M, 16 * RB), b);
        const size_t lds = (size_t)2 * 16 * RB * 4 * (KQ | 1) * sizeof(float);
        if (tab)
            hipLaunchKernelGGL((gemm_chunk_kernel<RB, KQ, false, true, true, 1, AT, BF, true>), grid, dim3(GC_WAVES * OGC_WAVE),
                               lds + tab_bytes, s, M, K, hw, w, y, grad_z, c2, ij, sh);
        else
            hipLaunchKernelGGL((gemm_chunk_kernel<RB, KQ, false, true, true, 1, AT, BF>), grid, dim3(GC_WAVES * OGC_WAVE), lds, s, M, K,
                               hw, w, y, grad_z, c2, ij, sh);
    }
    OGC_CHECK_LAUNCH("ogc_conv1x1_dgrad_pooled");
    return OGC_OK;
}
}

extern "C" int ogc_conv1x1_dgrad_pooled(int b, int cin, int cout, int hw, int nsample, const float *w, const float *y,
                                        const float *coef2, const float *inj, float *grad_z, ogc_stream_t stream) {
    return dgrad_pooled_impl<float>(b, cin, cout, hw, nsample, w, y, coef2, inj, grad_z, stream);
}

extern "C" int ogc_conv1x1_dgrad_pooled_h(int b, int cin, int cout, int hw, int nsample, const float *w, const ogc_bf16_t *y,
                                          const float *coef2, const float *inj, ogc_bf16_t *grad_z, ogc_stream_t stream) {
    return dgrad_pooled_impl<ogc_bf16>(b, cin, cout, hw, nsample, w, y, coef2, inj, grad_z, stream);
}
```

ogc_amd/csrc/group_norm.hip:

```cpp
#include "ogc_common.h"
#include "act_io.h"

namespace {

constexpr int GN_THREADS = 256;

__device__ __forceinline__ void gn_block_sum2(double &a, double &b, double *smem ) {
#pragma unroll
    for (int off = 32; off > 0; off >>= 1) {
        a += __shfl_down(a, off, 64);
        b += __shfl_down(b, off, 64);
    }
    const int lane = threadIdx.x & 63, wave = threadIdx.x >> 6;
    if (lane == 0) {
        smem[wave * 2] = a;
        smem[wave * 2 + 1] = b;
    }
    __syncthreads();
    if (threadIdx.x == 0) {
        a = 0.0;
        b = 0.0;
        for (int w = 0; w < GN_THREADS / 64; ++w) {
            a += smem[w * 2];
            b += smem[w * 2 + 1];
        }
    }
}

__global__ __launch_bounds__(GN_THREADS) void gn_stats_kernel(long long row_len, long long chunk_len,
                                                              const float *__restrict__ x, double *__restrict__ ws) {
    __shared__ double smem[2 * GN_THREADS / 64];
    const long long row = blockIdx.y;
    const long long begin = (long long)blockIdx.x * chunk_len;
    const long long end = min(row_len, begin + chunk_len);
    const float *p = x + row * row_len;
    double s = 0.0, ss = 0.0;
    if (((row_len | chunk_len) & 3) == 0 && ((uintptr_t)p & 15) == 0) {
        for (long long i = begin + threadIdx.x * 4; i < end; i += GN_THREADS * 4 * 4) {
            float fs = 0.0f, fss = 0.0f;
#pragma unroll
            for (int u = 0; u < 4; ++u) {
                const long long j = i + (long long)u * GN_THREADS * 4;
                if (j < end) {
                    const float4 v = *reinterpret_cast<const float4 *>(p + j);
                    fs += (v.x + v.y) + (v.z + v.w);
                    fss += (v.x * v.x + v.y * v.y) + (v.z * v.z + v.w * v.w);
                }
            }
            s += fs;
            ss += fss;
        }
    } else {
        for (long long i = begin + threadIdx.x; i < end; i += GN_THREADS) {
            const float v = p[i];
            s += v;
            ss += (double)v * v;
        }
    }
    gn_block_sum2(s, ss, smem);
    if (threadIdx.x == 0) {
        double *dst = ws + ((size_t)blockIdx.x * gridDim.y + row) * 2;
        dst[0] = s;
        dst[1] = ss;
    }
}

__device__ __forceinline__ void gn_sum_slots(const double *__restrict__ first, size_t stride, int slots, double &sum,
                                             double &sumsq) {
    for (int s0 = 0; s0 < slots; s0 += 8) {
        double2 v[8];
#pragma unroll
        for (int u = 0; u < 8; ++u)
            v[u] = *reinterpret_cast<const double2 *>(first + (size_t)min(s0 + u, slots - 1) * stride);
#pragma unroll
        for (int u = 0; u < 8; ++u)
            if (s0 + u < slots) {
                sum += v[u].x;
                sumsq += v[u].y;
            }
    }
}

template <bool RELU>
__global__ __launch_bounds__(GN_THREADS) void gn_apply_kernel(int c, int hw, int groups, float eps,
// ... 280 lines not shown
    if (xext && !(rstd[b * groups + ch / (c / groups)] * gamma[ch] != 0.f)) xext = nullptr;
    const size_t base = ((size_t)b * c + ch) * p;
    double ds = 0.0, db = 0.0;
    for (int pr = blockIdx.x * GN_THREADS + threadIdx.x; pr < p; pr += gridDim.x * GN_THREADS) {
        float g = gout[base + pr];
        if (RELU && !(out[base + pr] > 0.f)) g = 0.f;
        ds += (double)g * (double)(xext ? xext[base + pr] : ogc_ld1(x + (base + pr) * s + arg[base + pr]));
        db += g;
    }
    gn_block_sum2(ds, db, smem);
    if (threadIdx.x == 0) {
        double *dst = dsdb + (((size_t)blockIdx.x * gridDim.z + b) * c + ch) * 2;
        dst[0] = ds;
        dst[1] = db;
    }
}

template <bool RELU>
__global__ __launch_bounds__(GN_THREADS) void gn_maxpool_bwd_dx_kernel(int c, int p, int s, int groups,
                                                                       const float *__restrict__ x,
                                                                       const float *__restrict__ gamma,
                                                                       const float *__restrict__ mean,
                                                                       const float *__restrict__ rstd,
                                                                       const double *__restrict__ dsdb, int slots,
                                                                       const float *__restrict__ out,
                                                                       const int *__restrict__ arg,
                                                                       const float *__restrict__ gout,
                                                                       float *__restrict__ dx,
                                                                       float *__restrict__ dgamma,
                                                                       float *__restrict__ dbeta) {
    const int b = blockIdx.z, ch = blockIdx.y;
    const int cg = c / groups, row = b * groups + ch / cg;
    const float a = rstd[row] * gamma[ch];
    float c2, c3;
    gn_bwd_prologue(c, groups, (double)cg * p * s, slots, gamma, mean, rstd, dsdb, dgamma, dbeta, c2, c3);
    const int L = s >> 2;
    const int rows_per_block = GN_THREADS / L;
    const int sub = threadIdx.x % L;
    const size_t base = ((size_t)b * c + ch) * p;
    for (int pr = blockIdx.x * rows_per_block + threadIdx.x / L; pr < p; pr += gridDim.x * rows_per_block) {
        const size_t off = (base + pr) * s + sub * 4;
        const float4 v = *reinterpret_cast<const float4 *>(x + off);
        float g = gout[base + pr];
        if (RELU && !(out[base + pr] > 0.f)) g = 0.f;
        const int rel = arg[base + pr] - sub * 4;
        const float ag = a * g;
        float4 o;
        o.x = fmaf(c2, v.x, c3) + (rel == 0 ? ag : 0.f);
        o.y = fmaf(c2, v.y, c3) + (rel == 1 ? ag : 0.f);
        o.z = fmaf(c2, v.z, c3) + (rel == 2 ? ag : 0.f);
        o.w = fmaf(c2, v.w, c3) + (rel == 3 ? ag : 0.f);
        *reinterpret_cast<float4 *>(dx + off) = o;
    }
}

template <bool RELU>
__global__ __launch_bounds__(GN_THREADS) void gn_maxpool_bwd_sparse_kernel(int c, int p, int s, int groups,
                                                                           const float *__restrict__ gamma,
                                                                           const float *__restrict__ mean,
                                                                           const float *__restrict__ rstd,
                                                                           const double *__restrict__ dsdb, int slots,
                                                                           const float *__restrict__ out,
                                                                           const int *__restrict__ arg,
                                                                           const float *__restrict__ gout,
                                                                           float2 *__restrict__ coef2,
                                                                           float2 *__restrict__ inj,
                                                                           float *__restrict__ dgamma,
                                                                           float *__restrict__ dbeta) {
    const int b = blockIdx.z, ch = blockIdx.y;
    const int cg = c / groups, row = b * groups + ch / cg;
    const float a = rstd[row] * gamma[ch];
    float c2, c3;
    gn_bwd_prologue(c, groups, (double)cg * p * s, slots, gamma, mean, rstd, dsdb, dgamma, dbeta, c2, c3);
    const size_t base = ((size_t)b * c + ch) * p;
    for (int pr = blockIdx.x * GN_THREADS + threadIdx.x; pr < p; pr += gridDim.x * GN_THREADS) {
        float g = gout[base + pr];
        if (RELU && !(out[base + pr] > 0.f)) g = 0.f;
        inj[base + pr] = make_float2(a * g, __int_as_float(arg[base + pr]));
    }
    if (blockIdx.x == 0 && threadIdx.x == 0) coef2[(size_t)b * c + ch] = make_float2(c2, c3);
}

constexpr int GN_STATS_SLOTS = 32;
constexpr int GN_BWD_SLOTS = 8;

int hw_chunks(int b, int c, int hw) {
    int chunks = 1;
    while ((long long)b * c * chunks < 2048 && hw / (chunks * 2) >= 4096 && chunks < GN_BWD_SLOTS) chunks *= 2;
    return chunks;
}

int launch_gn_stats(int rows, long long row_len, const float *x, double *ws, hipStream_t s) {
    int chunks = 1;
    while ((long long)rows * chunks < 2048 && row_len / (chunks * 2) >= 16384 && chunks < GN_STATS_SLOTS) chunks *= 2;
    long long chunk_len = (row_len + chunks - 1) / chunks;
    chunk_len = (chunk_len + 3) / 4 * 4;
    const int slots = (int)ogc_divup(row_len, chunk_len);
    hipLaunchKernelGGL(gn_stats_kernel, dim3(slots, rows), dim3(GN_THREADS), 0, s, row_len, chunk_len, x, ws);
    return slots;
}

}

namespace {
int gn_fwd_impl(const char *name, int b, int c, int hw, int groups, float eps, int relu, const float *x,
                const float *gamma, const float *beta, float *y, float *mean, float *rstd, double *ws,
                const double *stats, int slots, ogc_stream_t stream) {
    OGC_REQUIRE(b >= 0 && c >= 1 && hw >= 1 && groups >= 1 && c % groups == 0, "%s: bad shape", name);
    if (b == 0) return OGC_OK;
    OGC_REQUIRE(x && gamma && beta && y && mean && rstd && (ws || stats), "%s: null pointer", name);
    OGC_REQUIRE((long long)c * hw < (1ll << 31) && b <= 65535, "%s: one sample exceeds 32-bit indexing", name);
    hipStream_t s = (hipStream_t)stream;
    if (!stats) {
        const int rows = b * groups;
        const long long row_len = (long long)(c / groups) * hw;
        slots = launch_gn_stats(rows, row_len, x, ws, s);
        stats = ws;
    }
    dim3 grid(hw_chunks(b, c, hw), c, b);
    if (relu)
        hipLaunchKernelGGL(gn_apply_kernel<true>, grid, dim3(GN_THREADS), 0, s, c, hw, groups, eps, x, gamma, beta, stats,
                           slots, y, mean, rstd);
    else
        hipLaunchKernelGGL(gn_apply_kernel<false>, grid, dim3(GN_THREADS), 0, s, c, hw, groups, eps, x, gamma, beta,
                           stats, slots, y, mean, rstd);
    OGC_CHECK_LAUNCH(name);
    return OGC_OK;
}
}

namespace {
__global__ void gn_coeffs_kernel(int b, int c, int hw, int groups, float eps, const float *__restrict__ gamma,
                                 const float *__restrict__ beta, const double *__restrict__ stats, int slots,
                                 float *__restrict__ mean_out, float *__restrict__ rstd_out, float *__restrict__ a_out,
                                 float *__restrict__ bb_out) {
    const int t = blockIdx.x * blockDim.x + threadIdx.x;
    if (t >= b * c) return;
    const int bi = t / c, ch = t % c;
    const int cg = c / groups, g = ch / cg, row = bi * groups + g;
    const double n = (double)cg * hw;
    double sum = 0.0, sumsq = 0.0;
    gn_sum_slots(stats + (size_t)row * 2, (size_t)b * groups * 2, slots, sum, sumsq);
    const double m = sum / n;
    const double var = fmax(sumsq / n - m * m, 0.0);
    const float mean = (float)m;
    const float rstd = (float)(1.0 / sqrt(var + (double)eps));
    if (ch == g * cg) {
        mean_out[row] = mean;
        rstd_out[row] = rstd;
    }
    const float a = rstd * gamma[ch];
    a_out[t] = a;
    bb_out[t] = beta[ch] - mean * a;
}
}

extern "C" int ogc_group_norm_coeffs(int b, int c, int hw, int groups, float eps, const float *x, const float *gamma,
                                     const float *beta, const double *stats, int slots, double *ws, float *mean,
                                     float *rstd, float *a, float *bb, ogc_stream_t stream) {
    OGC_REQUIRE(b >= 0 && c >= 1 && hw >= 1 && groups >= 1 && c % groups == 0, "ogc_group_norm_coeffs: bad shape");
    if (b == 0) return OGC_OK;
    OGC_REQUIRE(gamma && beta && mean && rstd && a && bb && (stats || (ws && x)), "ogc_group_norm_coeffs: null pointer");
    hipStream_t s = (hipStream_t)stream;
    if (!stats) {
        const int rows = b * groups;
        const long long row_len = (long long)(c / groups) * hw;
        slots = launch_gn_stats(rows, row_len, x, ws, s);
        stats = ws;
    }
    hipLaunchKernelGGL(gn_coeffs_kernel, dim3(ogc_divup(b * c, 256)), dim3(256), 0, s, b, c, hw, groups, eps, gamma, beta,
                       stats, slots, mean, rstd, a, bb);
    OGC_CHECK_LAUNCH("ogc_group_norm_coeffs");
    return OGC_OK;
}

extern "C" int ogc_group_norm_stats_slots(void) { return GN_STATS_SLOTS; }
extern "C" int ogc_group_norm_bwd_slots(void) { return GN_BWD_SLOTS; }

extern "C" int ogc_group_norm_fwd(int b, int c, int hw, int groups, float eps, int relu, const float *x,
                                  const float *gamma, const float *beta, float *y, float *mean, float *rstd,
                                  double *ws, ogc_stream_t stream) {
    return gn_fwd_impl("ogc_group_norm_fwd", b, c, hw, groups, eps, relu, x, gamma, beta, y, mean, rstd, ws, nullptr, 0,
                       stream);
}

extern "C" int ogc_group_norm_fwd_stats(int b, int c, int hw, int groups, float eps, int relu, const float *x,
                                        const float *gamma, const float *beta, float *y, float *mean, float *rstd,
                                        const double *stats, int slots, ogc_stream_t stream) {
    OGC_REQUIRE(stats && slots >= 1, "ogc_group_norm_fwd_stats: no statistics");
    return gn_fwd_impl("ogc_group_norm_fwd_stats", b, c, hw, groups, eps, relu, x, gamma, beta, y, mean, rstd, nullptr,
                       stats, slots, stream);
}

namespace {
template <typename AT>
int gn_bwd_impl(int b, int c, int hw, int groups, int relu, const AT *x, const float *gamma, const float *beta, const float *mean,
                const float *rstd, const AT *grad_y, AT *grad_x, float *grad_gamma, float *grad_beta, double *ws,
                ogc_stream_t stream) {
    OGC_REQUIRE(b >= 0 && c >= 1 && hw >= 1 && groups >= 1 && c % groups == 0, "ogc_group_norm_bwd: bad shape");
    if (b == 0) return OGC_OK;
    if (sizeof(AT) == 2 && ((hw & 3) != 0 || (((uintptr_t)x | (uintptr_t)grad_y | (uintptr_t)grad_x) & 7) != 0)) {
        ogc_set_error("ogc_group_norm_bwd_h: needs hw %% 4 == 0 and 8-byte aligned tensors");
        return OGC_ERR_UNSUPPORTED;
    }
    OGC_REQUIRE(x && gamma && beta && mean && rstd && grad_y && grad_x && grad_gamma && grad_beta && ws,
                "ogc_group_norm_bwd: null pointer");
    hipStream_t s = (hipStream_t)stream;
    double *dsdb = ws;
    dim3 grid(hw_chunks(b, c, hw), c, b);
    const int slots = (int)grid.x;
    if (relu) {
        hipLaunchKernelGGL((gn_bwd_sums_kernel<true, AT>), grid, dim3(GN_THREADS), 0, s, c, hw, groups, x, gamma, beta, mean,
                           rstd, grad_y, dsdb);
        hipLaunchKernelGGL((gn_bwd_dx_kernel<true, AT>), grid, dim3(GN_THREADS), 0, s, c, hw, groups, x, gamma, beta, mean,
                           rstd, dsdb, slots, grad_y, grad_x, grad_gamma, grad_beta);
    } else {
        hipLaunchKernelGGL((gn_bwd_sums_kernel<false, AT>), grid, dim3(GN_THREADS), 0, s, c, hw, groups, x, gamma, beta, mean,
                           rstd, grad_y, dsdb);
        hipLaunchKernelGGL((gn_bwd_dx_kernel<false, AT>), grid, dim3(GN_THREADS), 0, s, c, hw, groups, x, gamma, beta, mean,
                           rstd, dsdb, slots, grad_y, grad_x, grad_gamma, grad_beta);
    }
    OGC_CHECK_LAUNCH("ogc_group_norm_bwd");
    return OGC_OK;
}
}

extern "C" int ogc_group_norm_bwd(int b, int c, int hw, int groups, int relu, const float *x, const float *gamma,
                                  const float *beta, const float *mean, const float *rstd, const float *grad_y,
                                  float *grad_x, float *grad_gamma, float *grad_beta, double *ws,
                                  ogc_stream_t stream) {
    return gn_bwd_impl<float>(b, c, hw, groups, relu, x, gamma, beta, mean, rstd, grad_y, grad_x, grad_gamma, grad_beta, ws, stream);
}

extern "C" int ogc_group_norm_bwd_h(int b, int c, int hw, int groups, int relu, const ogc_bf16_t *x, const float *gamma,
                                    const float *beta, const float *mean, const float *rstd, const ogc_bf16_t *grad_y,
                                    ogc_bf16_t *grad_x, float *grad_gamma, float *grad_beta, double *ws,
                                    ogc_stream_t stream) {
    return gn_bwd_impl<ogc_bf16>(b, c, hw, groups, relu, x, gamma, beta, mean, rstd, grad_y, grad_x, grad_gamma, grad_beta, ws, stream);
}

static bool gn_pool_shape_ok(int s) { return s >= 4 && s <= 256 && (s & (s - 1)) == 0; }

namespace {
int gn_pool_fwd_impl(const char *name, int b, int c, int p, int s, int groups, float eps, int relu, const float *x,
                     const float *gamma, const float *beta, float *out, int *argmax, float *mean, float *rstd,
                     double *ws, const double *stats, int slots, ogc_stream_t stream) {
    OGC_REQUIRE(b >= 0 && c >= 1 && p >= 1 && groups >= 1 && c % groups == 0, "%s: bad shape", name);
    if (!gn_pool_shape_ok(s) || ((uintptr_t)x & 15) != 0) {
        ogc_set_error("%s: nsample=%d must be a power of two in [4,256] and x 16-byte aligned", name, s);
        return OGC_ERR_UNSUPPORTED;
    }
    if (b == 0) return OGC_OK;
    OGC_REQUIRE(x && gamma && beta && out && argmax && mean && rstd && (ws || stats), "%s: null pointer", name);
    OGC_REQUIRE((long long)c * p * s < (1ll << 31) && b <= 65535, "%s: one sample exceeds 32-bit indexing", name);
    hipStream_t st = (hipStream_t)stream;
    if (!stats) {
        const int rows = b * groups;
        const long long row_len = (long long)(c / groups) * p * s;
        slots = launch_gn_stats(rows, row_len, x, ws, st);
        stats = ws;
    }
    const int rows_per_block = GN_THREADS / (s / 4);
    int bx = ogc_divup(p, rows_per_block);
    while (bx > 1 && (long long)bx * c * b > 8192) bx = (bx + 1) / 2;
    dim3 grid(bx, c, b);
    if (relu)
        hipLaunchKernelGGL(gn_apply_maxpool_kernel<true>, grid, dim3(GN_THREADS), 0, st, c, p, s, groups, eps, x, gamma,
                           beta, stats, slots, out, argmax, mean, rstd);
    else
        hipLaunchKernelGGL(gn_apply_maxpool_kernel<false>, grid, dim3(GN_THREADS), 0, st, c, p, s, groups, eps, x,
                           gamma, beta, stats, slots, out, argmax, mean, rstd);
    OGC_CHECK_LAUNCH(name);
    return OGC_OK;
}
}

extern "C" int ogc_group_norm_maxpool_fwd(int b, int c, int p, int s, int groups, float eps, int relu, const float *x,
                                          const float *gamma, const float *beta, float *out, int *argmax,
                                          float *mean, float *rstd, double *ws, ogc_stream_t stream) {
    return gn_pool_fwd_impl("ogc_group_norm_maxpool_fwd", b, c, p, s, groups, eps, relu, x, gamma, beta, out, argmax,
                            mean, rstd, ws, nullptr, 0, stream);
}

extern "C" int ogc_group_norm_maxpool_fwd_stats(int b, int c, int p, int s, int groups, float eps, int relu,
                                                const float *x, const float *gamma, const float *beta, float *out,
                                                int *argmax, float *mean, float *rstd, const double *stats, int slots,
                                                ogc_stream_t stream) {
    OGC_REQUIRE(stats && slots >= 1, "ogc_group_norm_maxpool_fwd_stats: no statistics");
    return gn_pool_fwd_impl("ogc_group_norm_maxpool_fwd_stats", b, c, p, s, groups, eps, relu, x, gamma, beta, out,
                            argmax, mean, rstd, nullptr, stats, slots, stream);
}

extern "C" int ogc_group_norm_pool_extremes(int b, int c, int p, int s, int groups, float eps, int relu,
                                            const float *yext, const int *aext, const float *gamma, const float *beta,
                                            float *out, int *argmax, float *mean, float *rstd, const double *stats,
                                            int slots, ogc_stream_t stream) {
    OGC_REQUIRE(b >= 0 && c >= 1 && p >= 1 && s >= 1 && groups >= 1 && c % groups == 0 && slots >= 1,
                "ogc_group_norm_pool_extremes: bad shape");
    if (b == 0) return OGC_OK;
    OGC_REQUIRE(yext && aext && gamma && beta && out && argmax && mean && rstd && stats,
                "ogc_group_norm_pool_extremes: null pointer");
    OGC_REQUIRE(b <= 65535, "ogc_group_norm_pool_extremes: too many samples for one grid");
    const dim3 grid(c, b);
    hipStream_t st = (hipStream_t)stream;
    if (relu)
        hipLaunchKernelGGL(gn_pool_extremes_kernel<true>, grid, dim3(GN_THREADS), 0, st, c, p, s, groups, eps, yext, aext,
                           gamma, beta, stats, slots, out, argmax, mean, rstd);
    else
        hipLaunchKernelGGL(gn_pool_extremes_kernel<false>, grid, dim3(GN_THREADS), 0, st, c, p, s, groups, eps, yext, aext,
                           gamma, beta, stats, slots, out, argmax, mean, rstd);
    OGC_CHECK_LAUNCH("ogc_group_norm_pool_extremes");
    return OGC_OK;
}

// ... 112 lines not shown
```

ogc_amd/fused.py:

```python
import weakref

import torch
import torch.nn.functional as F
from torch.autograd import Function

from .pointnet2 import pointnet2 as _api



import collections as _collections
import functools as _functools

from .utils.zero_arena import zeroed_empty

GATE_MISSES = _collections.Counter()


def deterministic():
    from . import _lib
    return _lib.DETERMINISTIC

ACT16 = __import__("os").environ.get("OGC_ACT16", "1") != "0"


# ... 564 lines not shown


@_gate
def rigid_residual_available(mask, loss_norm):
    return (mask.is_cuda and mask.dtype == torch.float32 and loss_norm in (1, 2) and mask.shape[-1] <= 32
            and getattr(_api._native, "rigid_blend_wrapper", None) is not None)


def rigid_residual(pc, pc2, mask, loss_norm):
    nat = _api._native
    pc, pc2, mask = pc.contiguous(), pc2.contiguous(), mask.contiguous()
    VB, N, K = mask.shape
    dev = mask.device
    with torch.no_grad():
        mom = zeroed_empty(VB * K * 16, torch.float64, dev)
        S = torch.empty(VB * K, 3, 3, dtype=torch.float32, device=dev)
        means = torch.empty(VB * K, 6, dtype=torch.float32, device=dev)
        nat.rigid_moments_wrapper(VB, N, K, pc, pc2, mask.detach(), mom, S, means)
        R = torch.empty_like(S)
        valid = torch.empty(VB * K, dtype=torch.int32, device=dev)
        nat.kabsch_rotation_wrapper(VB * K, S, R, valid)
        t = torch.empty(VB * K, 3, dtype=torch.float32, device=dev)
        nat.rigid_translation_wrapper(VB * K, means, valid, R, t)
    return _RigidBlend.apply(pc, pc2, mask, R, t, int(loss_norm))


class _MatchedDistance(Function):

    @staticmethod
    def forward(ctx, mask1, mask2, col12, col21, p):
        nat = _api._native
        PB, N, K = mask1.shape
        d12 = torch.empty(PB, N, dtype=torch.float32, device=mask1.device)
        d21 = torch.empty_like(d12)
        nat.matched_distance_wrapper(PB, N, K, p, 0, mask1, mask2, col12, col21, None, None, d12, d21)
        ctx.save_for_backward(mask1, mask2, col12, col21)
        ctx.p = p
        return d12, d21

    @staticmethod
    def backward(ctx, g12, g21):
        nat = _api._native
        mask1, mask2, col12, col21 = ctx.saved_tensors
        PB, N, K = mask1.shape
        gm1, gm2 = torch.empty_like(mask1), torch.empty_like(mask2)
        nat.matched_distance_wrapper(PB, N, K, ctx.p, 1, mask1, mask2, col12, col21, g12.contiguous(), g21.contiguous(),
                                     gm1, gm2)
        return gm1, gm2, None, None, None


@_gate
def matched_distance_available(mask, loss_norm, cross_entropy):
    return (mask.is_cuda and mask.dtype == torch.float32 and not cross_entropy and loss_norm in (1, 2)
            and mask.shape[-1] <= 32 and getattr(_api._native, "matched_distance_wrapper", None) is not None
            and getattr(_api._native, "lsap_maximize_wrapper", None) is not None)


def matched_distances(mask1, mask2, loss_norm):
    nat = _api._native
    mask1, mask2 = mask1.contiguous(), mask2.contiguous()
    PB, N, K = mask1.shape
    dev = mask1.device
    with torch.no_grad():
        counts = zeroed_empty(PB * K * K, torch.int32, dev)
        iou = torch.empty(PB, K, K, dtype=torch.float32, device=dev)
        nat.mask_iou_wrapper(PB, N, K, mask1.detach(), mask2.detach(), counts, iou)
        both = torch.stack([iou, iou.transpose(1, 2)]).contiguous()
        cols = torch.empty(2 * PB, K, dtype=torch.int32, device=dev)
        nat.lsap_maximize_wrapper(2 * PB, K, both, cols)
    return _MatchedDistance.apply(mask1, mask2, cols[:PB], cols[PB:], int(loss_norm))


FUSED_GN_BACKWARD_MAX_WIDTH = 64
FUSED_GN_BACKWARD = True
ACT16_MOMENT_WIDTH = int(__import__("os").environ.get("OGC_ACT16_MOMENT_WIDTH", "64"))


def _moment_width(t):
    return ACT16_MOMENT_WIDTH if t.dtype is torch.bfloat16 else FUSED_GN_BACKWARD_MAX_WIDTH


def _pool_moment_cout(t):
    return ACT16_MOMENT_WIDTH if t.dtype is torch.bfloat16 else max(FUSED_GN_BACKWARD_MAX_WIDTH, SPARSE_POOL_MAX_COUT)


def _norm_act_conv_forward(y_prev, stats_prev, gn_weight, gn_bias, conv_weight, gn_groups, eps, relu, next_groups, pool,
                           next_gamma):
    nat = _api._native
    B, cin = y_prev.shape[0], y_prev.shape[1]
    cout = conv_weight.shape[0]
    hw = y_prev.numel() // (B * cin)
    dev = y_prev.device
    mean = torch.empty(B * gn_groups, dtype=torch.float32, device=dev)
    rstd = torch.empty_like(mean)
    a = torch.empty(B * cin, dtype=torch.float32, device=dev)
    bb = torch.empty_like(a)
    gamma, beta = gn_weight.contiguous(), gn_bias.contiguous()
    if stats_prev is not None:
        nat.group_norm_coeffs_wrapper(B, cin, hw, gn_groups, eps, None, gamma, beta, stats_prev,
                                      stats_prev.numel() // (2 * B * gn_groups), None, mean, rstd, a, bb)
    else:
        ws = nat.group_norm_ws(B, cin, gn_groups, False, dev)
        nat.group_norm_coeffs_wrapper(B, cin, hw, gn_groups, eps, y_prev, gamma, beta, None, 0, ws, mean, rstd, a, bb)
    y = torch.empty((B, cout) + tuple(y_prev.shape[2:]), dtype=y_prev.dtype, device=dev)
    w = conv_weight.contiguous()
    stats = extremes = None
    if (next_groups > 0 and next_groups <= 32 and cout % next_groups == 0 and (cout // next_groups) % 4 == 0
            and (cin <= 100 or _stats_ok(nat, B, cout, cin, hw, True))):
        stats = zeroed_empty(nat.conv1x1_gn_slots() * B * next_groups * 2, torch.float64, dev)
        if (pool and next_gamma is not None and (cin <= 100 or POOL_EXTREMES_WIDE)
                and getattr(nat, "conv1x1_gemm_affine_pool_wrapper", None) is not None):
            centres = hw // pool
            yext = torch.empty(B, cout, centres, dtype=torch.float32, device=dev)
            aext = torch.empty(B, cout, centres, dtype=torch.int32, device=dev)
            nat.conv1x1_gemm_affine_pool_wrapper(B, cout, cin, hw, relu, next_groups, pool, w, y_prev, a, bb,
                                                 next_gamma.contiguous(), y, stats, yext, aext)
            extremes = (yext, aext)
        else:
            nat.conv1x1_gemm_affine_wrapper(B, cout, cin, hw, relu, next_groups, w, y_prev, a, bb, y, stats)
    else:
        nat.conv1x1_gemm_affine_wrapper(B, cout, cin, hw, relu, 0, w, y_prev, a, bb, y, None)
    return y, stats, extremes, mean, rstd, a, bb


class _NormActConv(Function):

    @staticmethod
    def forward(ctx, y_prev, stats_prev, gn_weight, gn_bias, conv_weight, gn_groups, eps, relu, next_groups, pool=0,
                next_gamma=None):
        ctx.set_materialize_grads(False)
        y_prev = y_prev.contiguous()
        y, stats, extremes, mean, rstd, a, bb = _norm_act_conv_forward(y_prev, stats_prev, gn_weight, gn_bias, conv_weight,
                                                                       gn_groups, eps, relu, next_groups, pool, next_gamma)
        hw = y_prev.numel() // (y_prev.shape[0] * y_prev.shape[1])
        ctx.save_for_backward(y_prev, gn_weight, gn_bias, conv_weight, mean, rstd, a, bb)
        ctx.cfg = (gn_groups, relu, hw)
        if extremes is not None:
            ctx.mark_non_differentiable(stats, *extremes)
            return (y, stats) + extremes
        if stats is not None:
            ctx.mark_non_differentiable(stats)
        return y, stats

    @staticmethod
    def backward(ctx, grad_y, _grad_stats=None, *_grad_extremes):
        if grad_y is None:
            return (None,) * 11
        nat = _api._native
        y_prev, gn_weight, gn_bias, conv_weight, mean, rstd, a, bb = ctx.saved_tensors
        gn_groups, relu, hw = ctx.cfg
        B, cin = y_prev.shape[0], y_prev.shape[1]
        cout = conv_weight.shape[0]
        grad_y = grad_y.contiguous()
        w = conv_weight.contiguous()
        grad_w = zeroed_empty((cout, cin), torch.float32, y_prev.device)
        if (FUSED_GN_BACKWARD and getattr(nat, "conv1x1_dgrad_adjoint_wrapper", None) is not None and hw % 64 == 0
                and cout <= _moment_width(y_prev) and cin <= _moment_width(y_prev) and gn_groups <= 32
                and cin % gn_groups == 0):
            dev = y_prev.device
            moments = zeroed_empty((B, 2, cout, cin), torch.float32, dev)
            nat.conv1x1_wgrad_moments_wrapper(B, cin, cout, hw, relu, y_prev, a, bb, grad_y, moments)
            coef = torch.empty(B, cin, 3, dtype=torch.float32, device=dev)
            ggb = zeroed_empty((2, cin), torch.float32, dev)
            gw, gb = ggb[0], ggb[1]
            nat.gn_moments_combine_wrapper(B, cin, cout, hw, gn_groups, moments, w.view(cout, cin), a, bb, mean, rstd,
                                           gn_weight.contiguous(), grad_w, coef, gw, gb)
            grad_prev = torch.empty_like(y_prev)
            nat.conv1x1_dgrad_adjoint_wrapper(B, cin, cout, hw, relu, w.view(cout, cin), grad_y, y_prev, a, bb, coef, grad_prev)
            return grad_prev, None, gw, gb, grad_w.view_as(conv_weight), None, None, None, None, None, None
        nat.conv1x1_wgrad_affine_wrapper(B, cin, cout, hw, relu, y_prev, a, bb, grad_y, grad_w)
        if y_prev.dtype is torch.bfloat16 or (_gemm_ok(cout, hw) and _plain_gemm_mine(cout, (B, cin, hw))):
            grad_z = torch.empty_like(y_prev)
            nat.conv1x1_gemm_wrapper(B, cin, cout, hw, 1, w, grad_y, grad_z)
        else:
            grad_z = _product(w.view(cout, cin), grad_y.reshape(B, cout, hw), True).view_as(y_prev)
        grad_prev = torch.empty_like(y_prev)
        gw, gb = torch.empty_like(gn_weight), torch.empty_like(gn_bias)
        ws = nat.group_norm_ws(B, cin, gn_groups, True, y_prev.device)
        nat.group_norm_bwd_wrapper(B, cin, hw, gn_groups, relu, y_prev, gn_weight.contiguous(),
                                   gn_bias.contiguous(), mean, rstd, grad_z, grad_prev, gw, gb, ws)
        return grad_prev, None, gw, gb, grad_w.view_as(conv_weight), None, None, None, None, None, None


@_gate
def norm_act_conv_available(y_prev, gn, conv):
    if deterministic():
        return False
    if not (y_prev.is_cuda and _is_act(y_prev) and gn.affine and conv.bias is None and conv.groups == 1
            and all(k == 1 for k in conv.kernel_size) and all(v == 1 for v in conv.stride)
            and all(v == 0 for v in conv.padding)
            and getattr(_api._native, "conv1x1_gemm_affine_wrapper", None) is not None):
        return False
    hw = y_prev.numel() // max(y_prev.shape[0] * y_prev.shape[1], 1)
    if y_prev.dtype is torch.bfloat16 and _api._native.get_matmul_precision() != "bf16":
        return False
    return _gemm_ok(y_prev.shape[1], hw)


def act16_middle_ok(y_prev, gn, conv):
    return norm_act_conv_available(y_prev, gn, conv) and conv.weight.shape[0] <= 160


def norm_act_conv(y_prev, stats_prev, gn, relu, conv, next_gn=None, pool=0):
    next_groups = next_gn.num_groups if (next_gn is not None and next_gn.affine) else 0
    res = _NormActConv.apply(y_prev, stats_prev, gn.weight, gn.bias, conv.weight, gn.num_groups, gn.eps, bool(relu),
                             next_groups, int(pool) if (pool in (16, 32, 64) and next_groups) else 0,
                             next_gn.weight if next_groups else None)
    if pool:
        return res[0], res[1], (tuple(res[2:]) if len(res) > 2 else None)
    return res[0], res[1]


SPARSE_POOL_BACKWARD = True
SPARSE_POOL_MAX_COUT = 64
WIDE_POOL_BACKWARD = _os.environ.get("OGC_WIDE_POOL", "1") != "0"

class _NormActConvPool(Function):

    @staticmethod
    def forward(ctx, y_prev, stats_prev, gn_weight, gn_bias, conv_weight, gn_groups, eps, relu, gn2_weight, gn2_bias,
                groups2, eps2, relu2):
        nat = _api._native
        y_prev = y_prev.contiguous()
        B, cin, P, S = y_prev.shape
        cout = conv_weight.shape[0]
        y, stats, extremes, mean, rstd, a, bb = _norm_act_conv_forward(y_prev, stats_prev, gn_weight, gn_bias, conv_weight,
                                                                       gn_groups, eps, relu, groups2, S, gn2_weight)
        dev = y_prev.device
        out = torch.empty(B, cout, P, dtype=torch.float32, device=dev)
        arg = torch.empty(B, cout, P, dtype=torch.int32, device=dev)
        mean2 = torch.empty(B * groups2, dtype=torch.float32, device=dev)
        rstd2 = torch.empty_like(mean2)
        g2, b2 = gn2_weight.contiguous(), gn2_bias.contiguous()
        nat.group_norm_pool_extremes_wrapper(B, cout, P, S, groups2, eps2, relu2, extremes[0], extremes[1], g2, b2, out, arg,
                                             mean2, rstd2, stats, stats.numel() // (2 * B * groups2))
        ctx.save_for_backward(y_prev, gn_weight, gn_bias, conv_weight, mean, rstd, a, bb, y, gn2_weight, mean2, rstd2, out, arg,
                              extremes[0])
        ctx.cfg = (gn_groups, relu, groups2, relu2)
        return out

    @staticmethod
    def backward(ctx, grad_out):
        nat = _api._native
        (y_prev, gn_weight, gn_bias, conv_weight, mean, rstd, a, bb, y, gn2_weight, mean2, rstd2, out, arg,
         yext) = ctx.saved_tensors
        gn_groups, relu, groups2, relu2 = ctx.cfg
        B, cin, P, S = y_prev.shape
        cout, hw, dev = conv_weight.shape[0], P * S, y_prev.device
        coef2 = torch.empty(B, cout, 2, dtype=torch.float32, device=dev)
        inj = torch.empty(B, cout, P, 2, dtype=torch.float32, device=dev)
        gw2, gb2 = torch.empty_like(gn2_weight), torch.empty_like(gn2_weight)
        ws = nat.group_norm_ws(B, cout, groups2, True, dev)
        nat.group_norm_maxpool_bwd_sparse_wrapper(B, cout, P, S, groups2, relu2, y, gn2_weight.contiguous(), mean2,
                                                  rstd2, out, arg, grad_out.contiguous(), coef2, inj, gw2, gb2, ws,
                                                  yext if POOL_SUMS_FROM_EXTREMES else None)
        w = conv_weight.contiguous().view(cout, cin)
        if cin > _moment_width(y_prev) or cout > _pool_moment_cout(y_prev):
            grad_w = zeroed_empty((cout, cin), torch.float32, dev)
            nat.conv1x1_wgrad_affine_pooled_wrapper(B, cin, cout, hw, relu, S, y_prev, a, bb, y, coef2, inj, grad_w)
            grad_z = torch.empty_like(y_prev)
            nat.conv1x1_dgrad_pooled_wrapper(B, cin, cout, hw, S, w, y, coef2, inj, grad_z)
            grad_prev = torch.empty_like(y_prev)
            gw, gb = torch.empty_like(gn_weight), torch.empty_like(gn_bias)
            ws = nat.group_norm_ws(B, cin, gn_groups, True, dev)
            nat.group_norm_bwd_wrapper(B, cin, hw, gn_groups, relu, y_prev, gn_weight.contiguous(), gn_bias.contiguous(), mean,
                                       rstd, grad_z, grad_prev, gw, gb, ws)
            return (grad_prev, None, gw, gb, grad_w.view_as(conv_weight), None, None, None, gw2, gb2, None, None, None)
        moments = zeroed_empty((B, 2, cout, cin), torch.float32, dev)
        nat.conv1x1_wgrad_moments_pooled_wrapper(B, cin, cout, hw, relu, S, y_prev, a, bb, y, coef2, inj, moments)
        coef = torch.empty(B, cin, 3, dtype=torch.float32, device=dev)
        ggb = zeroed_empty((2, cin), torch.float32, dev)
        gw, gb = ggb[0], ggb[1]
        grad_w = torch.empty(cout, cin, dtype=torch.float32, device=dev)
        nat.gn_moments_combine_wrapper(B, cin, cout, hw, gn_groups, moments, w, a, bb, mean, rstd,
                                       gn_weight.contiguous(), grad_w, coef, gw, gb)
        grad_prev = torch.empty_like(y_prev)
        nat.conv1x1_dgrad_adjoint_pooled_wrapper(B, cin, cout, hw, relu, S, w, y, coef2, inj, y_prev, a, bb, coef, grad_prev)
        return (grad_prev, None, gw, gb, grad_w.view_as(conv_weight), None, None, None, gw2, gb2, None, None, None)


@_gate
def norm_act_conv_pool_available(y_prev, gn, conv, next_gn):
    nat = _api._native
    if not (SPARSE_POOL_BACKWARD and FUSED_GN_BACKWARD and y_prev.dim() == 4 and y_prev.shape[-1] in (16, 32, 64)
            and next_gn is not None and next_gn.affine and norm_act_conv_available(y_prev, gn, conv)
            and getattr(nat, "conv1x1_dgrad_adjoint_pooled_wrapper", None) is not None
            and getattr(nat, "conv1x1_gemm_affine_pool_wrapper", None) is not None):
        return False
    cin, cout, g, g2 = y_prev.shape[1], conv.weight.shape[0], gn.num_groups, next_gn.num_groups
    if cin > _moment_width(y_prev) or cout > _pool_moment_cout(y_prev):
        B, hw = y_prev.shape[0], y_prev.shape[2] * y_prev.shape[3]
        return (WIDE_POOL_BACKWARD and getattr(nat, "conv1x1_dgrad_pooled_wrapper", None) is not None
                and hw % 64 == 0 and B * (hw // 64) >= 1024 and B <= 65535
                and g <= 32 and cin % g == 0 and g2 <= 32 and cout % g2 == 0 and (cout // g2) % 4 == 0
                and (cin <= 100 or (POOL_EXTREMES_WIDE and _stats_ok(nat, B, cout, cin, hw, True))))
    kq = (cout + 3) // 4
    lds = (64 * 4 * (kq | 1) + 320) * 4 + 4 * cout * (64 // y_prev.shape[-1]) * 16
    return (lds <= 65536 and (y_prev.shape[2] * y_prev.shape[3]) % 64 == 0 and cin <= _moment_width(y_prev)
            and cout <= _pool_moment_cout(y_prev) and g <= 32 and cin % g == 0
            and g2 <= 32 and cout % g2 == 0 and (cout // g2) % 4 == 0)


def norm_act_conv_pool(y_prev, stats_prev, gn, relu, conv, next_gn, next_relu):
    return _NormActConvPool.apply(y_prev, stats_prev, gn.weight, gn.bias, conv.weight, gn.num_groups, gn.eps, bool(relu),
                                  next_gn.weight, next_gn.bias, next_gn.num_groups, next_gn.eps, bool(next_relu))


class _SelfAttentionCore(Function):

    @staticmethod
    def forward(ctx, qkv, n_head):
        nat = _api._native
        qkv = qkv.contiguous()
        B, L, E3 = qkv.shape
        E = E3 // 3
        out = torch.empty(B, L, E, dtype=torch.float32, device=qkv.device)
        prob = torch.empty(B, n_head, L, L, dtype=torch.float32, device=qkv.device)
        scale = (E // n_head) ** -0.5
        nat.attention_fwd_wrapper(n_head, scale, qkv[:, :, :E], qkv[:, :, E:2 * E], qkv[:, :, 2 * E:], out, prob)
        ctx.save_for_backward(qkv, out, prob)
        ctx.cfg = (n_head, scale)
        return out

    @staticmethod
    def backward(ctx, grad_out):
        qkv, out, prob = ctx.saved_tensors
        n_head, scale = ctx.cfg
        E = qkv.shape[2] // 3
        grad = torch.empty_like(qkv)
        _api._native.attention_bwd_wrapper(n_head, scale, qkv[:, :, :E], qkv[:, :, E:2 * E], qkv[:, :, 2 * E:], out, prob,
                                           grad_out.contiguous(), grad[:, :, :E], grad[:, :, E:2 * E], grad[:, :, 2 * E:])
        return grad, None


class _CrossAttentionCore(Function):

    @staticmethod
    def forward(ctx, q, kv, n_head):
        nat = _api._native
        q, kv = q.contiguous(), kv.contiguous()
        B, Lq, E = q.shape
        Lk = kv.shape[1]
        out = torch.empty(B, Lq, E, dtype=torch.float32, device=q.device)
        prob = torch.empty(B, n_head, Lq, Lk, dtype=torch.float32, device=q.device)
        scale = (E // n_head) ** -0.5
        nat.attention_fwd_wrapper(n_head, scale, q, kv[:, :, :E], kv[:, :, E:], out, prob)
# ... 271 lines not shown
```

ogc_amd/pointnet2_cuda.py:

```python
import torch

from . import _lib


def _check(t, dtype, name):
    try:
        if t.is_cuda and t.dtype is dtype and t.is_contiguous():
            return t.data_ptr()
    except AttributeError:
        pass
    if not isinstance(t, torch.Tensor):
        raise TypeError("%s must be a torch.Tensor" % name)
    if t.device.type != "cuda":
        raise RuntimeError("%s must be a CUDA tensor (HIP device); ogc_amd has no CPU path" % name)
    if not t.is_contiguous():
        raise RuntimeError("%s must be contiguous" % name)
    if t.dtype != dtype:
        raise RuntimeError("%s must be %s, got %s" % (name, dtype, t.dtype))
    return t.data_ptr()


def _f(t, name):
    return _check(t, torch.float32, name)

# ... 298 lines not shown


def group_linear_fwd_pt_wrapper(b, m, n, npoints, nsample, groups, Pt, idx, rel, wx, y, stats):
    _run("ogc_group_linear_fwd_pt_h", Pt, b, m, n, npoints, nsample, int(groups), _f(Pt, "Pt"), _i(idx, "idx"), _f(rel, "rel"),
         _f(wx, "wx"), _check(y, torch.bfloat16, "y"), _opt(stats, torch.float64, "stats"))


def group_linear_fwd_direct_wrapper(b, m, cf, n, npoints, nsample, groups, feats, idx, rel, w, y, stats):
    h, (yp,) = _acts((y,), ("y",))
    _run("ogc_group_linear_fwd_direct" + h, feats, b, m, cf, n, npoints, nsample, int(groups), _f(feats, "feats"), _i(idx, "idx"),
         _f(rel, "rel"), _f(w, "w"), yp, _opt(stats, torch.float64, "stats"))


def group_linear_bwd_wrapper(b, m, n, npoints, nsample, grad_y, idx, rel, grad_p, dwx):
    _run("ogc_group_linear_bwd", grad_y, b, m, n, npoints, nsample, _f(grad_y, "grad_y"), _i(idx, "idx"), _f(rel, "rel"),
         _f(grad_p, "grad_p"), _f(dwx, "dwx"))


def soft_nn_target_wrapper(b, n1, n2, k, temperature, p1, p2, mask1, mask2, target):
    _run("ogc_soft_nn_target", p1, b, n1, n2, k, float(temperature), _f(p1, "p1"), _f(p2, "p2"), _f(mask1, "mask1"),
         _f(mask2, "mask2"), _f(target, "target"))


def rigid_moments_wrapper(vb, n, k, pc, pc2, mask, mom, S, means):
    _run("ogc_rigid_moments", pc, vb, n, k, _f(pc, "pc"), _f(pc2, "pc2"), _f(mask, "mask"),
         _check(mom, torch.float64, "mom"), _f(S, "S"), _f(means, "means"))


def rigid_translation_wrapper(total, means, valid, R, t):
    _run("ogc_rigid_translation", means, total, _f(means, "means"), _i(valid, "valid"), _f(R, "R"), _f(t, "t"))


def rigid_blend_wrapper(vb, n, k, p, backward, pc, pc2, mask, R, t, grad_out, out):
    _run("ogc_rigid_blend", pc, vb, n, k, int(p), int(backward), _f(pc, "pc"), _f(pc2, "pc2"), _f(mask, "mask"),
         _f(R, "R"), _f(t, "t"), 0 if grad_out is None else _f(grad_out, "grad_out"), _f(out, "out"))


def mask_iou_wrapper(pb, n, k, mask1, mask2, counts, iou):
    _run("ogc_mask_iou", mask1, pb, n, k, _f(mask1, "mask1"), _f(mask2, "mask2"), _i(counts, "counts"), _f(iou, "iou"))


def matched_distance_wrapper(pb, n, k, p, backward, mask1, mask2, col12, col21, grad12, grad21, out1, out2):
    _run("ogc_matched_distance", mask1, pb, n, k, int(p), int(backward), _f(mask1, "mask1"), _f(mask2, "mask2"),
         _i(col12, "col12"), _i(col21, "col21"), 0 if grad12 is None else _f(grad12, "grad12"),
         0 if grad21 is None else _f(grad21, "grad21"), _f(out1, "out1"), _f(out2, "out2"))


def lsap_maximize_wrapper(np_, k, score, col4row):
    _run("ogc_lsap_maximize", score, np_, k, _f(score, "score"), _i(col4row, "col4row"))


def sym_eigvals_wrapper(nb, k, A, w):
    _run("ogc_sym_eigvals", A, nb, k, _check(A, torch.float64, "A"), _check(w, torch.float64, "w"))


def neighbour_consistency_fwd_wrapper(b, n, c, k, p, mask, idx, out):
    _run("ogc_neighbour_consistency_fwd", mask, b, n, c, k, int(p), _f(mask, "mask"), _i(idx, "idx"), _f(out, "out"))


def reverse_neighbours_wrapper(b, n, k, idx, rev_start, rev_src, rev_mult, ws):
    _run("ogc_reverse_neighbours", idx, b, n, k, _i(idx, "idx"), _i(rev_start, "rev_start"), _i(rev_src, "rev_src"),
         _i(rev_mult, "rev_mult"), _i(ws, "ws"))


def neighbour_consistency_bwd_wrapper(b, n, c, k, p, mask, idx, rev_start, rev_src, rev_mult, grad_out, grad_mask):
    _run("ogc_neighbour_consistency_bwd", mask, b, n, c, k, int(p), _f(mask, "mask"), _i(idx, "idx"),
         _i(rev_start, "rev_start"), _i(rev_src, "rev_src"), _i(rev_mult, "rev_mult"), _f(grad_out, "grad_out"),
         _f(grad_mask, "grad_mask"))


def group_norm_fwd_wrapper(b, c, hw, groups, eps, relu, x, gamma, beta, y, mean, rstd, ws):
    _run("ogc_group_norm_fwd", x, b, c, hw, groups, float(eps), int(relu), _f(x, "x"), _f(gamma, "gamma"),
         _f(beta, "beta"), _f(y, "y"), _f(mean, "mean"), _f(rstd, "rstd"), _check(ws, torch.float64, "ws"))


def group_norm_bwd_wrapper(b, c, hw, groups, relu, x, gamma, beta, mean, rstd, grad_y, grad_x, grad_gamma, grad_beta,
                           ws):
    h, (xp, gyp, gxp) = _acts((x, grad_y, grad_x), ("x", "grad_y", "grad_x"))
    _run("ogc_group_norm_bwd" + h, x, b, c, hw, groups, int(relu), xp, _f(gamma, "gamma"), _f(beta, "beta"),
         _f(mean, "mean"), _f(rstd, "rstd"), gyp, gxp,
         _f(grad_gamma, "grad_gamma"), _f(grad_beta, "grad_beta"), _check(ws, torch.float64, "ws"))


def group_norm_maxpool_fwd_wrapper(b, c, p, s, groups, eps, relu, x, gamma, beta, out, argmax, mean, rstd, ws):
    _run("ogc_group_norm_maxpool_fwd", x, b, c, p, s, groups, float(eps), int(relu), _f(x, "x"), _f(gamma, "gamma"),
         _f(beta, "beta"), _f(out, "out"), _i(argmax, "argmax"), _f(mean, "mean"), _f(rstd, "rstd"),
         _check(ws, torch.float64, "ws"))


def group_norm_maxpool_bwd_wrapper(b, c, p, s, groups, relu, x, gamma, mean, rstd, out, argmax, grad_out, grad_x,
                                   grad_gamma, grad_beta, ws):
    _run("ogc_group_norm_maxpool_bwd", x, b, c, p, s, groups, int(relu), _f(x, "x"), _f(gamma, "gamma"),
         _f(mean, "mean"), _f(rstd, "rstd"), _f(out, "out"), _i(argmax, "argmax"), _f(grad_out, "grad_out"),
         _f(grad_x, "grad_x"), _f(grad_gamma, "grad_gamma"), _f(grad_beta, "grad_beta"),
         _check(ws, torch.float64, "ws"))


def group_norm_maxpool_bwd_ext_wrapper(b, c, p, s, groups, relu, x, x_at_argmax, gamma, mean, rstd, out, argmax, grad_out,
                                       grad_x, grad_gamma, grad_beta, ws):
    _run("ogc_group_norm_maxpool_bwd_ext", x, b, c, p, s, groups, int(relu), _f(x, "x"), _f(x_at_argmax, "x_at_argmax"),
         _f(gamma, "gamma"), _f(mean, "mean"), _f(rstd, "rstd"), _f(out, "out"), _i(argmax, "argmax"),
         _f(grad_out, "grad_out"), _f(grad_x, "grad_x"), _f(grad_gamma, "grad_gamma"), _f(grad_beta, "grad_beta"),
         _check(ws, torch.float64, "ws"))


def conv1x1_wgrad_wrapper(b, cin, cout, hw, x, dy, dw):
    if dy.dtype is torch.bfloat16:
        _run("ogc_conv1x1_wgrad_xf_h", x, b, cin, cout, hw, _f(x, "x"), _check(dy, torch.bfloat16, "dy"), _f(dw, "dw"))
        return
    _run("ogc_conv1x1_wgrad", x, b, cin, cout, hw, _f(x, "x"), _f(dy, "dy"), _f(dw, "dw"))


def _opt(t, dtype, name):
    return 0 if t is None else _check(t, dtype, name)


def batch_norm_fwd_wrapper(b, c, hw, eps, relu, training, momentum, x, gamma, beta, running_mean, running_var, y, mean,
                           rstd, ws, stats, slots):
    _run("ogc_batch_norm_fwd", x, b, c, hw, float(eps), int(relu), int(training), float(momentum), _f(x, "x"),
         _f(gamma, "gamma"), _f(beta, "beta"), _opt(running_mean, torch.float32, "running_mean"),
         _opt(running_var, torch.float32, "running_var"), _f(y, "y"), _opt(mean, torch.float32, "mean"),
         _opt(rstd, torch.float32, "rstd"), _opt(ws, torch.float64, "ws"), _opt(stats, torch.float64, "stats"), int(slots))


def batch_norm_bwd_wrapper(b, c, hw, relu, training, x, gamma, beta, mean, rstd, grad_y, grad_x, grad_gamma, grad_beta,
                           ws):
    _run("ogc_batch_norm_bwd", x, b, c, hw, int(relu), int(training), _f(x, "x"), _f(gamma, "gamma"), _f(beta, "beta"),
         _f(mean, "mean"), _f(rstd, "rstd"), _f(grad_y, "grad_y"), _f(grad_x, "grad_x"), _f(grad_gamma, "grad_gamma"),
         _f(grad_beta, "grad_beta"), _check(ws, torch.float64, "ws"))


def batch_norm_maxpool_fwd_wrapper(b, c, p, s, eps, relu, training, momentum, x, gamma, beta, running_mean, running_var,
                                   out, argmax, mean, rstd, ws, stats, slots):
    _run("ogc_batch_norm_maxpool_fwd", x, b, c, p, s, float(eps), int(relu), int(training), float(momentum), _f(x, "x"),
         _f(gamma, "gamma"), _f(beta, "beta"), _opt(running_mean, torch.float32, "running_mean"),
         _opt(running_var, torch.float32, "running_var"), _f(out, "out"), _i(argmax, "argmax"),
         _opt(mean, torch.float32, "mean"), _opt(rstd, torch.float32, "rstd"), _opt(ws, torch.float64, "ws"),
         _opt(stats, torch.float64, "stats"), int(slots))


def batch_norm_maxpool_bwd_wrapper(b, c, p, s, relu, training, x, gamma, mean, rstd, out, argmax, grad_out, grad_x,
                                   grad_gamma, grad_beta, ws):
    _run("ogc_batch_norm_maxpool_bwd", x, b, c, p, s, int(relu), int(training), _f(x, "x"), _f(gamma, "gamma"),
         _f(mean, "mean"), _f(rstd, "rstd"), _f(out, "out"), _i(argmax, "argmax"), _f(grad_out, "grad_out"),
         _f(grad_x, "grad_x"), _f(grad_gamma, "grad_gamma"), _f(grad_beta, "grad_beta"), _check(ws, torch.float64, "ws"))


def group_norm_coeffs_wrapper(b, c, hw, groups, eps, x, gamma, beta, stats, slots, ws, mean, rstd, a, bb):
    _run("ogc_group_norm_coeffs", gamma, b, c, hw, groups, float(eps), _opt(x, torch.float32, "x"), _f(gamma, "gamma"),
         _f(beta, "beta"), _opt(stats, torch.float64, "stats"), int(slots), _opt(ws, torch.float64, "ws"),
         _f(mean, "mean"), _f(rstd, "rstd"), _f(a, "a"), _f(bb, "bb"))


def conv1x1_gemm_affine_wrapper(b, M, K, hw, relu, groups, w, inp, pa, pb, out, stats):
    h, (ip, op) = _acts((inp, out), ("in", "out"))
    _run("ogc_conv1x1_gemm_affine" + h, inp, b, M, K, hw, int(relu), int(groups), _f(w, "w"), ip, _f(pa, "pa"),
         _f(pb, "pb"), op, _opt(stats, torch.float64, "stats"))


def conv1x1_gemm_affine_pool_wrapper(b, M, K, hw, relu, groups, nsample, w, inp, pa, pb, next_gamma, out, stats, yext,
                                     aext):
    h, (ip, op) = _acts((inp, out), ("in", "out"))
    _run("ogc_conv1x1_gemm_affine_pool" + h, inp, b, M, K, hw, int(relu), int(groups), int(nsample), _f(w, "w"),
         ip, _f(pa, "pa"), _f(pb, "pb"), _f(next_gamma, "next_gamma"), op,
         _check(stats, torch.float64, "stats"), _f(yext, "yext"), _i(aext, "aext"))

# ... 55 lines not shown


def group_norm_maxpool_bwd_sparse_wrapper(b, c, p, s, groups, relu, x, gamma, mean, rstd, out, argmax, grad_out, coef2, inj,
                                          grad_gamma, grad_beta, ws, x_at_argmax=None):
    h, (xp,) = _acts((x,), ("x",))
    _run("ogc_group_norm_maxpool_bwd_sparse" + h, x, b, c, p, s, groups, int(relu), xp,
         _opt(x_at_argmax, torch.float32, "x_at_argmax"), _f(gamma, "gamma"),
         _f(mean, "mean"), _f(rstd, "rstd"), _f(out, "out"), _i(argmax, "argmax"), _f(grad_out, "grad_out"),
         _f(coef2, "coef2"), _f(inj, "inj"), _f(grad_gamma, "grad_gamma"), _f(grad_beta, "grad_beta"),
         _check(ws, torch.float64, "ws"))


def conv1x1_wgrad_moments_pooled_wrapper(b, cin, cout, hw, relu, nsample, y_prev, pa, pb, y, coef2, inj, moments):
    h, (ypp, yp) = _acts((y_prev, y), ("y_prev", "y"))
    _run("ogc_conv1x1_wgrad_moments_pooled" + h, y_prev, b, cin, cout, hw, int(relu), nsample, ypp, _f(pa, "pa"),
         _f(pb, "pb"), yp, _f(coef2, "coef2"), _f(inj, "inj"), _f(moments, "moments"))


def conv1x1_dgrad_adjoint_pooled_wrapper(b, cin, cout, hw, relu, nsample, w, y, coef2, inj, y_prev, pa, pb, coef, grad_prev):
    h, (yp, ypp, op) = _acts((y, y_prev, grad_prev), ("y", "y_prev", "grad_prev"))
    _run("ogc_conv1x1_dgrad_adjoint_pooled" + h, y, b, cin, cout, hw, int(relu), nsample, _f(w, "w"), yp,
         _f(coef2, "coef2"), _f(inj, "inj"), ypp, _f(pa, "pa"), _f(pb, "pb"), _f(coef, "coef"), op)


def mlp_chain_pool_supported(c0, c1, c2, c3, nsample):
    return bool(_lib.load().ogc_mlp_chain_pool_supported(c0, c1, c2, c3, nsample))


def mlp_chain_pool_wrapper(x, wts, biases, out):
    B, c0, P, S = x.shape
    c = [w.shape[1] for w in wts] + [0]
    _run("ogc_mlp_chain_pool", x, B, c0, c[0], c[1], c[2] if len(wts) > 2 else 0, P, S, _f(x, "x"),
         _f(wts[0], "wt1"), _f(biases[0], "b1"), _f(wts[1], "wt2"), _f(biases[1], "b2"),
         _f(wts[2], "wt3") if len(wts) > 2 else None, _f(biases[2], "b3") if len(wts) > 2 else None, _f(out, "out"))


def corr_layer_pool_supported(cf, c1, c2, c3, nsample):
    return bool(_lib.load().ogc_corr_layer_pool_supported(cf, c1, c2, c3, nsample))


def corr_layer_pool_wrapper(pos1, pos2, feat1, feat2, idx, wts, biases, out):
    B, cf, n1 = feat1.shape
    _run("ogc_corr_layer_pool", feat1, B, cf, wts[0].shape[1], wts[1].shape[1], wts[2].shape[1], n1, feat2.shape[2],
         idx.shape[2], _f(pos1, "pos1"), _f(pos2, "pos2"), _f(feat1, "feat1"), _f(feat2, "feat2"), _i(idx, "idx"),
         _f(wts[0], "wt1"), _f(biases[0], "b1"), _f(wts[1], "wt2"), _f(biases[1], "b2"), _f(wts[2], "wt3"),
         _f(biases[2], "b3"), _f(out, "out"))


def small_linear_fwd_wrapper(x, weight, bias, y):
    rows, n_in = x.shape
    _run("ogc_small_linear_fwd", x, rows, n_in, weight.shape[0], _f(x, "x"), _f(weight, "weight"),
         None if bias is None else _f(bias, "bias"), _f(y, "y"))


def small_linear_bwd_wrapper(x, weight, grad_y, grad_x, grad_weight, grad_bias):
    rows, n_in = x.shape
    _run("ogc_small_linear_bwd", x, rows, n_in, weight.shape[0], _f(x, "x"), _f(weight, "weight"), _f(grad_y, "grad_y"),
         None if grad_x is None else _f(grad_x, "grad_x"), None if grad_weight is None else _f(grad_weight, "grad_weight"),
         None if grad_bias is None else _f(grad_bias, "grad_bias"))


def slot_masks_fwd_wrapper(temperature, feats, slots, mask):
    b, d, n = feats.shape
    _run("ogc_slot_masks_fwd", feats, b, d, n, slots.shape[2], float(temperature), _f(feats, "feats"),
         _f(slots, "slots"), _f(mask, "mask"))


def slot_masks_bwd_wrapper(temperature, feats, slots, mask, grad_mask, grad_feats, grad_slots):
    b, d, n = feats.shape
    k = slots.shape[2]
    ws = torch.empty(max(int(_lib.load().ogc_slot_masks_ws_floats(b, d, n, k)), 1), dtype=torch.float32,
                     device=feats.device)
    _run("ogc_slot_masks_bwd", feats, b, d, n, k, float(temperature), _f(feats, "feats"), _f(slots, "slots"),
         _f(mask, "mask"), _f(grad_mask, "grad_mask"), _f(grad_feats, "grad_feats"), _f(grad_slots, "grad_slots"),
         _f(ws, "ws"))


def group_norm_ws(b, c, groups, backward, device):
    L = _lib.load()
    n = 2 * b * c * L.ogc_group_norm_bwd_slots() if backward else 2 * b * groups * L.ogc_group_norm_stats_slots()
    return torch.empty(max(n, 1), dtype=torch.float64, device=device)


_precision = "fp32"


def set_matmul_precision(mode):
    global _precision
    if mode not in ("fp32", "bf16"):
        raise ValueError("matmul precision must be 'fp32' or 'bf16'")
    previous = "bf16" if _lib.load().ogc_set_matmul_precision(1 if mode == "bf16" else 0) else "fp32"
    _precision = mode
    return previous


def get_matmul_precision():
    return _precision


def conv1x1_gemm_stream_supported(b, m, k, hw):
    return bool(_lib.load().ogc_conv1x1_gemm_stream_supported(int(b), int(m), int(k), int(hw)))


def conv1x1_gemm_stats_supported(b, m, k, hw, affine):
    return bool(_lib.load().ogc_conv1x1_gemm_stats_supported(int(b), int(m), int(k), int(hw), 1 if affine else 0))


def conv1x1_gn_slots():
    return _lib.load().ogc_conv1x1_gn_slots()


def conv1x1_gemm_gnstats_wrapper(b, M, K, hw, groups, w, inp, out, stats):
    _run("ogc_conv1x1_gemm_gnstats", inp, b, M, K, hw, groups, _f(w, "w"), _f(inp, "in"), _f(out, "out"),
         _check(stats, torch.float64, "stats"))


def group_norm_fwd_stats_wrapper(b, c, hw, groups, eps, relu, x, gamma, beta, y, mean, rstd, stats, slots):
    _run("ogc_group_norm_fwd_stats", x, b, c, hw, groups, float(eps), int(relu), _f(x, "x"), _f(gamma, "gamma"),
         _f(beta, "beta"), _f(y, "y"), _f(mean, "mean"), _f(rstd, "rstd"), _check(stats, torch.float64, "stats"),
         int(slots))


def group_norm_maxpool_fwd_stats_wrapper(b, c, p, s, groups, eps, relu, x, gamma, beta, out, argmax, mean, rstd, stats,
                                         slots):
    _run("ogc_group_norm_maxpool_fwd_stats", x, b, c, p, s, groups, float(eps), int(relu), _f(x, "x"),
         _f(gamma, "gamma"), _f(beta, "beta"), _f(out, "out"), _i(argmax, "argmax"), _f(mean, "mean"),
         _f(rstd, "rstd"), _check(stats, torch.float64, "stats"), int(slots))


def conv1x1_gemm_wrapper(b, M, K, hw, transpose_a, w, inp, out):
    h, (ip, op) = _acts((inp, out), ("in", "out"))
    _run("ogc_conv1x1_gemm" + h, inp, b, M, K, hw, int(transpose_a), _f(w, "w"), ip, op)


def conv1x1_gemm_any_wrapper(b, M, K, hw, transpose_a, w, inp, out):
    _run("ogc_conv1x1_gemm_any", inp, b, M, K, hw, int(transpose_a), _f(w, "w"), _f(inp, "in"), _f(out, "out"))


def conv1x1_wgrad_affine_pooled_wrapper(b, cin, cout, hw, relu, nsample, x, pa, pb, y, coef2, inj, dw):
    h, (xp, yp) = _acts((x, y), ("x", "y"))
    _run("ogc_conv1x1_wgrad_affine_pooled" + h, x, b, cin, cout, hw, int(relu), nsample, xp, _f(pa, "pa"), _f(pb, "pb"),
         yp, _f(coef2, "coef2"), _f(inj, "inj"), _f(dw, "dw"))


def conv1x1_dgrad_pooled_wrapper(b, cin, cout, hw, nsample, w, y, coef2, inj, grad_z):
    h, (yp, gp) = _acts((y, grad_z), ("y", "grad_z"))
    _run("ogc_conv1x1_dgrad_pooled" + h, y, b, cin, cout, hw, nsample, _f(w, "w"), yp, _f(coef2, "coef2"), _f(inj, "inj"), gp)
```

Measured before the change: 1566 point-clouds/s.

## Fuse GroupNorm backward reductions into conv1x1 dgrad GEMM epilogue

Adds a GNB mode to the streaming conv1x1 GEMM kernel and to the pooled dgrad path. While it writes grad_z, the kernel also accumulates the per-channel GroupNorm backward sums (ds/db) in double precision, using LDS staging and atomics into slotted buffers. A new gn_bwd_dx kernel then computes grad_x and the gamma/beta grads from those precomputed sums, so the separate reduction pass over grad_z and y_prev is no longer needed. The cost is extra LDS, y_prev reads and atomics inside the GEMM, plus narrower eligibility: fp32 only, hw divisible by 64, Kq of at most 33.

```diff
diff --git a/include/ogc_ops.h b/include/ogc_ops.h
--- a/include/ogc_ops.h
+++ b/include/ogc_ops.h
@@ -15,7 +15,7 @@
     OGC_ERR_UNSUPPORTED = -3
 };
 
-#define OGC_VERSION 205
+#define OGC_VERSION 206
 int ogc_version(void);
 int ogc_distance_contracted(void);
 int ogc_set_deterministic(int on);
@@ -243,6 +243,16 @@
 int ogc_conv1x1_gemm_gnstats(int b, int M, int K, int hw, int groups, const float *w, const float *in, float *out,
                              double *stats, ogc_stream_t stream);
 
+int ogc_conv1x1_dgrad_gnsums(int b, int cin, int cout, int hw, int groups, int relu, const float *w, const float *grad_y,
+                             const float *y_prev, const float *gamma, const float *beta, const float *mean, const float *rstd,
+                             float *grad_z, double *dsdb, ogc_stream_t stream);
+int ogc_conv1x1_dgrad_pooled_gnsums(int b, int cin, int cout, int hw, int nsample, int groups, int relu, const float *w,
+                                    const float *y, const float *coef2, const float *inj, const float *y_prev, const float *gamma,
+                                    const float *beta, const float *mean, const float *rstd, float *grad_z, double *dsdb,
+                                    ogc_stream_t stream);
+int ogc_group_norm_bwd_dx(int b, int c, int hw, int groups, int relu, const float *x, const float *gamma, const float *beta,
+                          const float *mean, const float *rstd, const float *grad_y, float *grad_x, float *grad_gamma,
+                          float *grad_beta, const double *dsdb, ogc_stream_t stream);
 int ogc_group_norm_coeffs(int b, int c, int hw, int groups, float eps, const float *x, const float *gamma,
                           const float *beta, const double *stats, int slots, double *ws, float *mean, float *rstd,
                           float *a, float *bb, ogc_stream_t stream);
diff --git a/ogc_amd/_lib.py b/ogc_amd/_lib.py
--- a/ogc_amd/_lib.py
+++ b/ogc_amd/_lib.py
@@ -113,6 +113,10 @@
     "ogc_conv1x1_wgrad_affine": [_int, _int, _int, _int, _int, _vp, _vp, _vp, _vp, _vp, _vp],
     "ogc_conv1x1_wgrad_affine_pooled": [_int, _int, _int, _int, _int, _int, _vp, _vp, _vp, _vp, _vp, _vp, _vp, _vp],
     "ogc_conv1x1_dgrad_pooled": [_int, _int, _int, _int, _int, _vp, _vp, _vp, _vp, _vp, _vp],
+    "ogc_conv1x1_dgrad_gnsums": [_int, _int, _int, _int, _int, _int, _vp, _vp, _vp, _vp, _vp, _vp, _vp, _vp, _vp, _vp],
+    "ogc_conv1x1_dgrad_pooled_gnsums": [_int, _int, _int, _int, _int, _int, _int, _vp, _vp, _vp, _vp, _vp, _vp, _vp, _vp, _vp,
+                                        _vp, _vp, _vp],
+    "ogc_group_norm_bwd_dx": [_int, _int, _int, _int, _int, _vp, _vp, _vp, _vp, _vp, _vp, _vp, _vp, _vp, _vp, _vp],
     "ogc_batch_norm_fwd": [_int, _int, _int, _flt, _int, _int, _flt, _vp, _vp, _vp, _vp, _vp, _vp, _vp, _vp, _vp, _vp,
                            _int, _vp],
     "ogc_batch_norm_bwd": [_int, _int, _int, _int, _int, _vp, _vp, _vp, _vp, _vp, _vp, _vp, _vp, _vp, _vp, _vp],
@@ -139,7 +143,7 @@
 SIGNATURES["ogc_conv1x1_wgrad_xf_h"] = SIGNATURES["ogc_conv1x1_wgrad"]
 SIGNATURES["ogc_group_linear_fwd_pt_h"] = SIGNATURES["ogc_group_linear_fwd"]
 
-HEADER_VERSION = 205
+HEADER_VERSION = 206
 _lib = None
 _fns = {}
 
diff --git a/ogc_amd/csrc/build.py b/ogc_amd/csrc/build.py
--- a/ogc_amd/csrc/build.py
+++ b/ogc_amd/csrc/build.py
@@ -5,7 +5,7 @@
 
 HERE = os.path.dirname(os.path.abspath(__file__))
 SOURCES = ["api.hip", "det.hip", "knn.hip", "ball_query.hip", "fps.hip", "gather_group.hip", "interpolate.hip", "kabsch.hip", "small_solvers.hip", "neighbour_loss.hip", "soft_nn.hip", "seg_loss.hip", "group_norm.hip", "batch_norm.hip", "grid.hip", "conv1x1.hip", "conv1x1_h.hip", "conv1x1_wgrad.hip", "attention.hip", "slot_masks.hip", "small_linear.hip", "loss_glue.hip", "mlp_chain.hip", "gn_fused_bwd.hip", "adam.hip", "gemm_chunk.hip", "chamfer.hip", "flow_step.hip"]
-HEADERS = ["ogc_common.h", "grid.h", "conv_stage.h", "conv1x1_shared.h", "act_io.h", "conv1x1_epilogue.h", os.path.join("..", "..", "include", "ogc_ops.h")]
+HEADERS = ["ogc_common.h", "grid.h", "conv_stage.h", "conv1x1_shared.h", "act_io.h", "conv1x1_epilogue.h", "gn_bwd_epilogue.h", os.path.join("..", "..", "include", "ogc_ops.h")]
 LIB = os.path.join(HERE, "libogc_ops.so")
 FMAD_SOURCES = ["knn.hip", "ball_query.hip", "fps.hip", "grid.hip"]
 LIB_FMAD = os.path.join(HERE, "libogc_ops_fmad.so")
diff --git a/ogc_amd/csrc/conv1x1.hip b/ogc_amd/csrc/conv1x1.hip
--- a/ogc_amd/csrc/conv1x1.hip
+++ b/ogc_amd/csrc/conv1x1.hip
@@ -1,6 +1,7 @@
 #include "conv1x1_shared.h"
 #include "act_io.h"
 #include "conv1x1_epilogue.h"
+#include "gn_bwd_epilogue.h"
 
 int ogc_g_matmul_bf16 = 0;
 
@@ -238,7 +239,8 @@
     }
 }
 
-template <int KQ, bool PRO, bool EXACT, bool STATS = false, bool POOL = false, bool DUAL = false, bool TRANS = false>
+template <int KQ, bool PRO, bool EXACT, bool STATS = false, bool POOL = false, bool DUAL = false, bool TRANS = false,
+          bool GNB = false>
 __global__ __launch_bounds__(WG_WAVES *OGC_WAVE, DUAL ? 2 : 1) void conv1x1_gemm_stream_kernel(int M, int K, int hw, int ntiles,
                                                                                  const float *__restrict__ w,
                                                                                  const float *__restrict__ in,
@@ -247,7 +249,8 @@
                                                                                  const float *__restrict__ pb, int pro_relu,
                                                                                  int groups = 1, int nbatch = 1,
                                                                                  double *__restrict__ stats = nullptr,
-                                                                                 PoolOut pool = PoolOut()) {
+                                                                                 PoolOut pool = PoolOut(),
+                                                                                 GnBwdSums gnb = GnBwdSums()) {
     extern __shared__ __attribute__((aligned(16))) float a_lds[];
     const int lane = threadIdx.x & 63, wave = __builtin_amdgcn_readfirstlane(threadIdx.x >> 6);
     const int j = lane & 15, kk = lane >> 4;
@@ -259,6 +262,35 @@
     if constexpr (POOL) {
         for (int t = threadIdx.x; t < Mt * 64; t += WG_WAVES * OGC_WAVE) sgn_all[t] = (t < M && pool.sign[t] < 0.f) ? -1.f : 1.f;
     }
+    static_assert(!GNB || (TRANS && !PRO && !STATS && !POOL), "GroupNorm sums: the plain input gradient only");
+    float2 *gco = reinterpret_cast<float2 *>(a_lds + (size_t)Mt * 64 * a_ld);
+    double *gred = reinterpret_cast<double *>(gco + 2 * Mt * 64);
+    int gb_first = 0, gb_count = 0;
+    if constexpr (GNB) {
+        const int wg_per = WG_WAVES * ((ntiles + gridDim.x * WG_WAVES - 1) / (gridDim.x * WG_WAVES));
+        const int wg_t0 = blockIdx.x * wg_per, wg_t1 = min(ntiles, wg_t0 + wg_per);
+        if (wg_t0 < wg_t1) {
+            gb_first = wg_t0 / tiles_per_img;
+            gb_count = (wg_t1 - 1) / tiles_per_img - gb_first + 1;
+        }
+        for (int e = threadIdx.x; e < 2 * Mt * 64; e += WG_WAVES * OGC_WAVE) {
+            const int sl = e / (Mt * 64), row = e - sl * (Mt * 64);
+            gco[e] = ogc_gnb_coef(gnb, min(gb_first + sl, nbatch - 1), min(row, M - 1), M);
+            gred[2 * e] = 0.0;
+            gred[2 * e + 1] = 0.0;
+        }
+    }
+    auto gnb_flush = [&]() {
+        if constexpr (GNB) {
+            __syncthreads();
+            for (int e = threadIdx.x; e < gb_count * Mt * 64 * 2; e += WG_WAVES * OGC_WAVE) {
+                const int sl = e / (Mt * 64 * 2), rem = e - sl * (Mt * 64 * 2);
+                if ((rem >> 1) < M)
+                    unsafeAtomicAdd(gnb.dsdb + (((size_t)(blockIdx.x % OGC_GN_BWD_SLOTS) * nbatch + gb_first + sl) * M) * 2 + rem,
+                                    gred[e]);
+            }
+        }
+    };
     __syncthreads();
     const int nw = gridDim.x * WG_WAVES;
     const unsigned off_main = (unsigned)(kk * hw + 4 * j);
@@ -324,9 +356,24 @@
         }
         float *outb = out + (size_t)b * M * hw + p0;
         const unsigned off_out = (unsigned)(kk * 4 * hw + 4 * j);
+        constexpr int YA = GNB ? (DUAL ? 1 : 4) : 1;
+        const float *yb = GNB ? gnb.y + (size_t)b * M * hw + p0 : nullptr;
+        auto load_y = [&](int mt, int a, float4(&v)[4]) {
+#pragma unroll
+            for (int r = 0; r < 4; ++r) {
+                const int m0 = mt * 64 + a * 16 + r;
+                if (EXACT) v[r] = *reinterpret_cast<const float4 *>(yb + (size_t)m0 * hw + off_out);
+                else v[r] = *reinterpret_cast<const float4 *>(yb + (size_t)min(m0 + kk * 4, M - 1) * hw + 4 * j);
+            }
+        };
         for (int mt = 0; mt < Mt; ++mt) {
             const float *at = a_lds + (size_t)mt * 64 * a_ld;
             const int nblk = EXACT ? 4 : min(4, (M - mt * 64 + 15) >> 4);
+            float4 yv[YA][4];
+            if constexpr (GNB) {
+#pragma unroll
+                for (int a = 0; a < YA; ++a) load_y(mt, a, yv[a]);
+            }
             v4f acc[4][4];
 #pragma unroll
             for (int a = 0; a < 4; ++a)
@@ -367,6 +414,26 @@
                 if (pool.s == 64) ogc_pool_extremes_epilogue<16>(acc, nblk, sg, j, kk, m0p, M, centres, 64, pool.yext + o0, pool.aext + o0);
                 else if (pool.s == 32) ogc_pool_extremes_epilogue<8>(acc, nblk, sg, j, kk, m0p, M, centres, 32, pool.yext + o0, pool.aext + o0);
                 else ogc_pool_extremes_epilogue<4>(acc, nblk, sg, j, kk, m0p, M, centres, 16, pool.yext + o0, pool.aext + o0);
+            }
+            if constexpr (GNB) {
+                const int sl = b - gb_first;
+                const float2 *co = gco + sl * (Mt * 64) + mt * 64 + kk * 4;
+                double *red = gred + ((size_t)sl * (Mt * 64) + mt * 64 + kk * 4) * 2;
+#pragma unroll
+                for (int a = 0; a < 4; ++a) {
+                    double s[4], sb[4], k[2];
+#pragma unroll
+                    for (int r = 0; r < 4; ++r)
+                        ogc_gnb_partials(make_float4(acc[a][0][r], acc[a][1][r], acc[a][2][r], acc[a][3][r]), yv[a % YA][r],
+                                         co[a * 16 + r], gnb.relu != 0, s[r], sb[r]);
+                    if (a + YA < 4) load_y(mt, a + YA, yv[a % YA]);
+                    ogc_gnb_row_reduce(s, sb, j, k);
+                    if (j < 4) {
+                        const int row = a * 16 + ((j >> 1) & 1);
+                        if (EXACT || mt * 64 + kk * 4 + row < M) atomicAdd(red + 2 * row + (j & 1), k[0]);
+                        if (EXACT || mt * 64 + kk * 4 + row + 2 < M) atomicAdd(red + 2 * (row + 2) + (j & 1), k[1]);
+                    }
+                }
             }
             if constexpr (STATS) {
 #pragma unroll
@@ -406,6 +473,7 @@
             compute_store(t, x1);
         }
         if (STATS) flush_stats();
+        gnb_flush();
         return;
     }
     float4 xa[KQ], xb[KQ];
@@ -420,6 +488,7 @@
         if (t < t_end) compute_store(t, xa);
     }
     if (STATS) flush_stats();
+    gnb_flush();
 }
 
 bool gemm_stream_eligible(int b, int M, int K, int hw, bool pro, bool pool = false, bool any_precision = false) {
@@ -432,40 +501,53 @@
              ntiles >= (1ll << 31));
 }
 
-template <bool PRO, bool STATS = false, bool POOL = false, bool TRANS = false>
+template <bool PRO, bool STATS = false, bool POOL = false, bool TRANS = false, bool GNB = false>
 bool gemm_stream_launch(int b, int M, int K, int hw, const float *w, const float *in, float *out, const float *pa,
                         const float *pb, int pro_relu, hipStream_t s, int groups = 1, double *stats = nullptr,
-                        PoolOut pool = PoolOut()) {
+                        PoolOut pool = PoolOut(), const GnBwdSums &gnb = GnBwdSums()) {
     const int Kq = (K + 3) / 4, Mt = (M + 63) / 64;
     const long long ntiles = (long long)b * (hw / 64);
-    const size_t lds = ((size_t)Mt * 64 * ogc_a_ld(Kq) + (PRO ? WG_WAVES * 2 * FW_KQ_MAX * 4 : 0)) * sizeof(float) +
-                       WG_WAVES * 4 * 16 * 2 * sizeof(double) + (POOL ? (size_t)Mt * 64 * sizeof(float) : 0);
+    const size_t lds = GNB ? (size_t)Mt * 64 * ogc_a_ld(Kq) * sizeof(float) + (size_t)2 * Mt * 64 * (sizeof(float2) + 2 * sizeof(double))
+                           : ((size_t)Mt * 64 * ogc_a_ld(Kq) + (PRO ? WG_WAVES * 2 * FW_KQ_MAX * 4 : 0)) * sizeof(float) +
+                                 WG_WAVES * 4 * 16 * 2 * sizeof(double) + (POOL ? (size_t)Mt * 64 * sizeof(float) : 0);
     if (!gemm_stream_eligible(b, M, K, hw, PRO, POOL, STATS) || lds > 156 * 1024) return false;
+    if (GNB && Kq > 33) return false;
     const int wgs = (int)(ntiles / WG_WAVES < 256 ? ntiles / WG_WAVES : 256);
 #define OGC_STREAM_D(KQV, EX, DU, WGS)                                                                                       \
     do {                                                                                                                     \
         static bool raised = false;                                                                                          \
-        const void *fn = reinterpret_cast<const void *>(&conv1x1_gemm_stream_kernel<KQV, PRO, EX, STATS, POOL, DU, TRANS>);         \
+        const void *fn = reinterpret_cast<const void *>(&conv1x1_gemm_stream_kernel<KQV, PRO, EX, STATS, POOL, DU, TRANS, GNB>);    \
         if (!raised) {                                                                                                       \
             if (hipFuncSetAttribute(fn, hipFuncAttributeMaxDynamicSharedMemorySize, 156 * 1024) != hipSuccess) return false;  \
             raised = true;                                                                                                   \
         }                                                                                                                    \
-        hipLaunchKernelGGL((conv1x1_gemm_stream_kernel<KQV, PRO, EX, STATS, POOL, DU, TRANS>), dim3(WGS), dim3(WG_WAVES * OGC_WAVE), \
-                           lds, s, M, K, hw, (int)ntiles, w, in, out, pa, pb, pro_relu, groups, b, stats, pool);             \
+        hipLaunchKernelGGL((conv1x1_gemm_stream_kernel<KQV, PRO, EX, STATS, POOL, DU, TRANS, GNB>), dim3(WGS),               \
+                           dim3(WG_WAVES * OGC_WAVE), lds, s, M, K, hw, (int)ntiles, w, in, out, pa, pb, pro_relu, groups, b,  \
+                           stats, pool, gnb);                                                                                \
     } while (0)
     static const bool dual_on = !(getenv("OGC_GEMM_STREAM_DUAL") && getenv("OGC_GEMM_STREAM_DUAL")[0] == '0');
-    const bool dual = dual_on && !POOL && 2 * (lds + 1024) <= 156 * 1024 && ntiles >= 4096;
+    const bool full_rows = M % 64 == 0;
+    const bool dual = dual_on && !POOL && 2 * (lds + 1024) <= 156 * 1024 && ntiles >= 4096 && (!GNB || full_rows);
     const int wgs2 = (int)(ntiles / WG_WAVES < 512 ? ntiles / WG_WAVES : 512);
+    if (GNB) {
+        const long long nwv = (long long)(dual ? wgs2 : wgs) * WG_WAVES;
+        if (WG_WAVES * ((ntiles + nwv - 1) / nwv) > hw / 64) return false;
+    }
 #define OGC_STREAM(KQV, EX)                                                                                                  \
     do {                                                                                                                     \
         if (dual) OGC_STREAM_D(KQV, EX, true, wgs2);                                                                         \
         else OGC_STREAM_D(KQV, EX, false, wgs);                                                                              \
     } while (0)
-    const bool full_rows = M % 64 == 0;
-    if (Kq == 32 && full_rows) OGC_STREAM(32, true);
-    else if (Kq == 33 && full_rows) OGC_STREAM(33, true);
-    else if (Kq <= 33) OGC_STREAM(33, false);
-    else OGC_STREAM(40, false);
+    if constexpr (GNB) {
+        if (Kq == 32 && full_rows) OGC_STREAM(32, true);
+        else if (Kq == 33 && full_rows) OGC_STREAM(33, true);
+        else OGC_STREAM_D(33, false, false, wgs);
+    } else {
+        if (Kq == 32 && full_rows) OGC_STREAM(32, true);
+        else if (Kq == 33 && full_rows) OGC_STREAM(33, true);
+        else if (Kq <= 33) OGC_STREAM(33, false);
+        else OGC_STREAM(40, false);
+    }
 #undef OGC_STREAM
 #undef OGC_STREAM_D
     return true;
@@ -523,6 +605,17 @@
     return OGC_OK;
 }
 
+}
+
+bool ogc_gemm_stream_dgrad_gnsums_launch(int b, int M, int K, int hw, const float *w, const float *in, float *out,
+                                         const GnBwdSums &gnb, hipStream_t s) {
+    if (g_matmul_bf16) return false;
+    return gemm_stream_launch<false, false, false, true, true>(b, M, K, hw, w, in, out, nullptr, nullptr, 0, s, 1, nullptr,
+                                                               PoolOut(), gnb);
+}
+
+namespace {
+
 template <typename AT>
 int gemm_check(const char *name, int b, int M, int K, int hw, const float *w, const AT *in, const AT *out) {
     OGC_REQUIRE(b >= 0 && M >= 1 && K >= 1 && hw >= 1, "%s: bad shape", name);
diff --git a/ogc_amd/csrc/gemm_chunk.hip b/ogc_amd/csrc/gemm_chunk.hip
--- a/ogc_amd/csrc/gemm_chunk.hip
+++ b/ogc_amd/csrc/gemm_chunk.hip
@@ -3,6 +3,7 @@
 #include "ogc_common.h"
 #include "act_io.h"
 #include "conv1x1_shared.h"
+#include "gn_bwd_epilogue.h"
 
 namespace {
 
@@ -11,13 +12,13 @@
 __device__ __forceinline__ v4s gc_pack_bf16(float a, float b, float c, float d) { return ogc_pack_bf16_rr(a, b, c, d); }
 
 template <int RB, int KQ, bool SPLIT_M, bool TRANS, bool POOLED = false, int KA = 1, typename AT = float, bool BF = false,
-          bool TAB = false>
+          bool TAB = false, bool GNB = false>
 __global__ __launch_bounds__(GC_WAVES *OGC_WAVE, 2) void gemm_chunk_kernel(int M, int K, int hw, const float *__restrict__ w,
                                                                          const AT *__restrict__ in,
                                                                          AT *__restrict__ out,
                                                                          const float2 *__restrict__ coef2 = nullptr,
                                                                          const float2 *__restrict__ inj = nullptr,
-                                                                         int s_shift = 0) {
+                                                                         int s_shift = 0, GnBwdSums gnb = GnBwdSums()) {
     constexpr int KC = 4 * KQ, KCA = KC * KA, LD = 4 * ((KQ * KA) | 1);
     constexpr int MT = SPLIT_M ? 64 * RB : 16 * RB;
     constexpr int PER = (MT * KCA) / (GC_WAVES * OGC_WAVE);
@@ -34,6 +35,17 @@
     const int nblk = min(RB, (M - m0 - wrow + 15) >> 4);
     const AT *inb = in + (size_t)b * K * hw + pl + 4 * j;
     const int nchunks = (K + KC - 1) / KC;
+    constexpr int GROWS = GNB ? MT : 1;
+    __shared__ float2 gnb_co[GROWS];
+    __shared__ double gnb_red[2 * GROWS];
+    if constexpr (GNB) {
+        static_assert(!GNB || (TRANS && !BF && sizeof(AT) == 4), "GroupNorm sums: fp32 input gradients only");
+        for (int e = t; e < MT; e += GC_WAVES * OGC_WAVE) {
+            gnb_co[e] = ogc_gnb_coef(gnb, b, min(m0 + e, M - 1), M);
+            gnb_red[2 * e] = 0.0;
+            gnb_red[2 * e + 1] = 0.0;
+        }
+    }
 
     v4f acc[RB][4];
 #pragma unroll
@@ -198,26 +210,67 @@
         if (more2) store_a(buf0, a_next);
         __syncthreads();
     }
-    if (!active) return;
     AT *ob = out + (size_t)b * M * hw + p0 + 4 * j;
-#pragma unroll
-    for (int a = 0; a < RB; ++a) {
-        if (a < nblk) {
-#pragma unroll
-            for (int r = 0; r < 4; ++r) {
-                const int m = m0 + wrow + a * 16 + kk * 4 + r;
-                if (m < M) ogc_st4(ob + (size_t)m * hw, make_float4(acc[a][0][r], acc[a][1][r], acc[a][2][r], acc[a][3][r]));
-            }
-        }
+    auto store_block = [&](int a) {
+#pragma unroll
+        for (int r = 0; r < 4; ++r) {
+            const int m = m0 + wrow + a * 16 + kk * 4 + r;
+            if (m < M) ogc_st4(ob + (size_t)m * hw, make_float4(acc[a][0][r], acc[a][1][r], acc[a][2][r], acc[a][3][r]));
+        }
+    };
+    if constexpr (!GNB) {
+        if (!active) return;
+#pragma unroll
+        for (int a = 0; a < RB; ++a)
+            if (a < nblk) store_block(a);
+    } else {
+        if (active) {
+            const float *yb = gnb.y + (size_t)b * M * hw + p0 + 4 * j;
+            const int rbase = wrow + kk * 4;
+            auto load_y = [&](int a, float4(&v)[4]) {
+#pragma unroll
+                for (int r = 0; r < 4; ++r)
+                    v[r] = *reinterpret_cast<const float4 *>(yb + (size_t)min(m0 + rbase + a * 16 + r, M - 1) * hw);
+            };
+            float4 yv[2][4];
+            if (nblk > 0) load_y(0, yv[0]);
+#pragma unroll
+            for (int a = 0; a < RB; ++a) {
+                if (a < nblk) {
+                    if (a + 1 < nblk) load_y(a + 1, yv[(a + 1) & 1]);
+                    store_block(a);
+                    double s[4], sb[4], k[2];
+#pragma unroll
+                    for (int r = 0; r < 4; ++r)
+                        ogc_gnb_partials(make_float4(acc[a][0][r], acc[a][1][r], acc[a][2][r], acc[a][3][r]), yv[a & 1][r],
+                                         gnb_co[rbase + a * 16 + r], gnb.relu != 0, s[r], sb[r]);
+                    ogc_gnb_row_reduce(s, sb, j, k);
+                    if (j < 4) {
+                        const int row = rbase + a * 16 + ((j >> 1) & 1);
+                        if (m0 + row < M) atomicAdd(&gnb_red[2 * row + (j & 1)], k[0]);
+                        if (m0 + row + 2 < M) atomicAdd(&gnb_red[2 * (row + 2) + (j & 1)], k[1]);
+                    }
+                }
+            }
+        }
+        __syncthreads();
+        double *dst = gnb.dsdb + (((size_t)(blockIdx.x % OGC_GN_BWD_SLOTS) * gnb.nb + b) * M + m0) * 2;
+        for (int e = t; e < 2 * MT; e += GC_WAVES * OGC_WAVE)
+            if (m0 + (e >> 1) < M) unsafeAtomicAdd(dst + e, gnb_red[e]);
     }
 }
 
 template <int RB, int KQ, bool SPLIT_M, int KA = 1>
 void gemm_chunk_launch(int b, int M, int K, int hw, int transpose_a, const float *w, const float *in, float *out,
-                       hipStream_t s) {
+                       hipStream_t s, const GnBwdSums *gnb = nullptr) {
     constexpr int MT = SPLIT_M ? 64 * RB : 16 * RB;
     const size_t lds = (size_t)2 * MT * 4 * ((KQ * KA) | 1) * sizeof(float);
     dim3 grid(SPLIT_M ? hw / 64 : ogc_divup(hw, 64 * GC_WAVES), ogc_divup(M, MT), b);
+    if (gnb) {
+        hipLaunchKernelGGL((gemm_chunk_kernel<RB, KQ, SPLIT_M, true, false, KA, float, false, false, true>), grid,
+                           dim3(GC_WAVES * OGC_WAVE), lds, s, M, K, hw, w, in, out, nullptr, nullptr, 0, *gnb);
+        return;
+    }
 #define GC_GO(TR, BFV)                                                                                                           \
     hipLaunchKernelGGL((gemm_chunk_kernel<RB, KQ, SPLIT_M, TR, false, KA, float, BFV>), grid, dim3(GC_WAVES * OGC_WAVE), lds, s, M, K, \
                        hw, w, in, out, nullptr, nullptr, 0)
@@ -231,6 +284,48 @@
 #undef GC_GO
 }
 
+void gemm_any_dispatch(int b, int M, int K, int hw, int transpose_a, const float *w, const float *in, float *out, hipStream_t s,
+                       const GnBwdSums *gnb = nullptr) {
+    const long long tiles = (long long)b * (hw / 64);
+#define GC_CASE(RBV, KQV, SPLIT)                                                              \
+    case RBV: gemm_chunk_launch<RBV, KQV, SPLIT>(b, M, K, hw, transpose_a, w, in, out, s, gnb); break
+    if (tiles >= 4096) {
+        const int ntile = ogc_divup(M, 128), rb = ogc_divup(M, 16 * ntile);
+        switch (rb) {
+            GC_CASE(1, 8, false); GC_CASE(2, 8, false); GC_CASE(3, 8, false); GC_CASE(4, 8, false);
+            GC_CASE(5, 8, false); GC_CASE(6, 8, false); GC_CASE(7, 4, false);
+            default: {
+                static const char *kq = getenv("OGC_GEMM_CHUNK_KQ");
+                if (kq && kq[0] == '4' && !gnb) gemm_chunk_launch<8, 4, false>(b, M, K, hw, transpose_a, w, in, out, s);
+                else gemm_chunk_launch<8, 4, false, 2>(b, M, K, hw, transpose_a, w, in, out, s, gnb);
+            }
+        }
+    } else {
+        const bool same_rows = 128 * ogc_divup(M, 128) == 64 * ogc_divup(M, 64);
+        const int rb = (M > 64 && same_rows && tiles * ogc_divup(M, 128) >= 512) ? 2 : 1;
+        switch (rb) {
+            GC_CASE(2, 8, true);
+            default: gemm_chunk_launch<1, 8, true>(b, M, K, hw, transpose_a, w, in, out, s, gnb);
+        }
+    }
+#undef GC_CASE
+}
+
+int gnb_check(const char *name, int b, int cin, int groups, const float *y_prev, const float *gamma, const float *beta,
+              const float *mean, const float *rstd, double *dsdb, hipStream_t s) {
+    OGC_REQUIRE(y_prev && gamma && beta && mean && rstd && dsdb, "%s: null pointer", name);
+    OGC_REQUIRE(groups >= 1 && cin % groups == 0, "%s: bad shape", name);
+    if (ogc_g_matmul_bf16 || ((uintptr_t)y_prev & 15) != 0 || ((uintptr_t)dsdb & 7) != 0) {
+        ogc_set_error("%s: needs fp32 operands (ogc_set_matmul_precision(0)) and aligned tensors", name);
+        return OGC_ERR_UNSUPPORTED;
+    }
+    if (b > 0 && ogc_zero_async(dsdb, sizeof(double) * 2 * OGC_GN_BWD_SLOTS * (size_t)b * cin, s) != hipSuccess) {
+        ogc_set_error("%s: memset failed", name);
+        return OGC_ERR_LAUNCH;
+    }
+    return OGC_OK;
+}
+
 }
 
 extern "C" int ogc_conv1x1_gemm_any(int b, int M, int K, int hw, int transpose_a, const float *w, const float *in, float *out,
@@ -244,38 +339,40 @@
     OGC_REQUIRE((long long)M * hw < (1ll << 31) && (long long)K * hw < (1ll << 31) && b <= 65535,
                 "ogc_conv1x1_gemm_any: one sample exceeds 32-bit indexing");
     if (b == 0) return OGC_OK;
+    gemm_any_dispatch(b, M, K, hw, transpose_a, w, in, out, (hipStream_t)stream);
+    OGC_CHECK_LAUNCH("ogc_conv1x1_gemm_any");
+    return OGC_OK;
+}
+
+extern "C" int ogc_conv1x1_dgrad_gnsums(int b, int cin, int cout, int hw, int groups, int relu, const float *w,
+                                        const float *grad_y, const float *y_prev, const float *gamma, const float *beta,
+                                        const float *mean, const float *rstd, float *grad_z, double *dsdb, ogc_stream_t stream) {
+    const int M = cin, K = cout;
+    OGC_REQUIRE(b >= 0 && M >= 1 && K >= 1 && hw >= 1, "ogc_conv1x1_dgrad_gnsums: bad shape");
+    OGC_REQUIRE(w && grad_y && grad_z, "ogc_conv1x1_dgrad_gnsums: null pointer");
+    if ((hw & 63) != 0 || (((uintptr_t)grad_y | (uintptr_t)grad_z) & 15) != 0) {
+        ogc_set_error("ogc_conv1x1_dgrad_gnsums: needs hw %% 64 == 0 and 16-byte aligned tensors (hw=%d)", hw);
+        return OGC_ERR_UNSUPPORTED;
+    }
+    OGC_REQUIRE((long long)M * hw < (1ll << 31) && (long long)K * hw < (1ll << 31) && b <= 65535,
+                "ogc_conv1x1_dgrad_gnsums: one sample exceeds 32-bit indexing");
     hipStream_t s = (hipStream_t)stream;
-    const long long tiles = (long long)b * (hw / 64);
-#define GC_CASE(RBV, KQV, SPLIT)                                                              \
-    case RBV: gemm_chunk_launch<RBV, KQV, SPLIT>(b, M, K, hw, transpose_a, w, in, out, s); break
-    if (tiles >= 4096) {
-        const int ntile = ogc_divup(M, 128), rb = ogc_divup(M, 16 * ntile);
-        switch (rb) {
-            GC_CASE(1, 8, false); GC_CASE(2, 8, false); GC_CASE(3, 8, false); GC_CASE(4, 8, false);
-            GC_CASE(5, 8, false); GC_CASE(6, 8, false); GC_CASE(7, 4, false);
-            default: {
-                static const char *kq = getenv("OGC_GEMM_CHUNK_KQ");
-                if (kq && kq[0] == '4') gemm_chunk_launch<8, 4, false>(b, M, K, hw, transpose_a, w, in, out, s);
-                else gemm_chunk_launch<8, 4, false, 2>(b, M, K, hw, transpose_a, w, in, out, s);
-            }
-        }
-    } else {
-        const bool same_rows = 128 * ogc_divup(M, 128) == 64 * ogc_divup(M, 64);
-        const int rb = (M > 64 && same_rows && tiles * ogc_divup(M, 128) >= 512) ? 2 : 1;
-        switch (rb) {
-            GC_CASE(2, 8, true);
-            default: gemm_chunk_launch<1, 8, true>(b, M, K, hw, transpose_a, w, in, out, s);
-        }
-    }
-#undef GC_CASE
-    OGC_CHECK_LAUNCH("ogc_conv1x1_gemm_any");
+    const int rc = gnb_check("ogc_conv1x1_dgrad_gnsums", b, cin, groups, y_prev, gamma, beta, mean, rstd, dsdb, s);
+    if (rc != OGC_OK) return rc;
+    if (b == 0) return OGC_OK;
+    GnBwdSums gnb;
+    gnb.y = y_prev; gnb.gamma = gamma; gnb.beta = beta; gnb.mean = mean; gnb.rstd = rstd; gnb.dsdb = dsdb;
+    gnb.groups = groups; gnb.relu = relu; gnb.nb = b;
+    if (!ogc_gemm_stream_dgrad_gnsums_launch(b, M, K, hw, w, grad_y, grad_z, gnb, s))
+        gemm_any_dispatch(b, M, K, hw, 1, w, grad_y, grad_z, s, &gnb);
+    OGC_CHECK_LAUNCH("ogc_conv1x1_dgrad_gnsums");
     return OGC_OK;
 }
 
 namespace {
 template <typename AT>
 int dgrad_pooled_impl(int b, int cin, int cout, int hw, int nsample, const float *w, const AT *y, const float *coef2,
-                      const float *inj, AT *grad_z, ogc_stream_t stream) {
+                      const float *inj, AT *grad_z, ogc_stream_t stream, const GnBwdSums *gnb = nullptr) {
     constexpr bool BF = sizeof(AT) == 2;
     OGC_REQUIRE(b >= 0 && cin >= 1 && cout >= 1 && hw >= 1, "ogc_conv1x1_dgrad_pooled: bad shape");
     OGC_REQUIRE(w && y && coef2 && inj && grad_z, "ogc_conv1x1_dgrad_pooled: null pointer");
@@ -296,27 +393,32 @@
     static const bool tab_off = [] { const char *e = getenv("OGC_DGRAD_POOLED_TAB"); return e && e[0] == '0'; }();
     const size_t tab_bytes = (size_t)GC_WAVES * K * (64 >> sh) * sizeof(float4);
     const bool tab = !tab_off && tab_bytes <= 24 * 1024;
+#define GC_POOLED(RBV, KQV, KAV, TABV, LDSV)                                                                                     \
+    do {                                                                                                                         \
+        if constexpr (!BF) {                                                                                                     \
+            if (gnb) {                                                                                                           \
+                hipLaunchKernelGGL((gemm_chunk_kernel<RBV, KQV, false, true, true, KAV, AT, BF, TABV, true>), grid,              \
+                                   dim3(GC_WAVES * OGC_WAVE), LDSV, s, M, K, hw, w, y, grad_z, c2, ij, sh, *gnb);                \
+                break;                                                                                                           \
+            }                                                                                                                    \
+        }                                                                                                                        \
+        hipLaunchKernelGGL((gemm_chunk_kernel<RBV, KQV, false, true, true, KAV, AT, BF, TABV>), grid, dim3(GC_WAVES * OGC_WAVE), \
+                           LDSV, s, M, K, hw, w, y, grad_z, c2, ij, sh);                                                         \
+    } while (0)
     if (M <= 64) {
         constexpr int RB = 4, KQ = 4, KA = 2;
         dim3 grid(ogc_divup(hw, 64 * GC_WAVES), ogc_divup(M, 16 * RB), b);
         const size_t lds = (size_t)2 * 16 * RB * 4 * ((KQ * KA) | 1) * sizeof(float);
-        if (tab)
-            hipLaunchKernelGGL((gemm_chunk_kernel<RB, KQ, false, true, true, KA, AT, BF, true>), grid, dim3(GC_WAVES * OGC_WAVE),
-                               lds + tab_bytes, s, M, K, hw, w, y, grad_z, c2, ij, sh);
-        else
-            hipLaunchKernelGGL((gemm_chunk_kernel<RB, KQ, false, true, true, KA, AT, BF>), grid, dim3(GC_WAVES * OGC_WAVE), lds, s, M,
-                               K, hw, w, y, grad_z, c2, ij, sh);
+        if (tab) GC_POOLED(RB, KQ, KA, true, lds + tab_bytes);
+        else GC_POOLED(RB, KQ, KA, false, lds);
     } else {
         constexpr int RB = 8, KQ = 4;
         dim3 grid(ogc_divup(hw, 64 * GC_WAVES), ogc_divup(M, 16 * RB), b);
         const size_t lds = (size_t)2 * 16 * RB * 4 * (KQ | 1) * sizeof(float);
-        if (tab)
-            hipLaunchKernelGGL((gemm_chunk_kernel<RB, KQ, false, true, true, 1, AT, BF, true>), grid, dim3(GC_WAVES * OGC_WAVE),
-                               lds + tab_bytes, s, M, K, hw, w, y, grad_z, c2, ij, sh);
-        else
-            hipLaunchKernelGGL((gemm_chunk_kernel<RB, KQ, false, true, true, 1, AT, BF>), grid, dim3(GC_WAVES * OGC_WAVE), lds, s, M, K,
-                               hw, w, y, grad_z, c2, ij, sh);
-    }
+        if (tab) GC_POOLED(RB, KQ, 1, true, lds + tab_bytes);
+        else GC_POOLED(RB, KQ, 1, false, lds);
+    }
+#undef GC_POOLED
     OGC_CHECK_LAUNCH("ogc_conv1x1_dgrad_pooled");
     return OGC_OK;
 }
@@ -331,3 +433,17 @@
                                           const float *coef2, const float *inj, ogc_bf16_t *grad_z, ogc_stream_t stream) {
     return dgrad_pooled_impl<ogc_bf16>(b, cin, cout, hw, nsample, w, y, coef2, inj, grad_z, stream);
 }
+
+extern "C" int ogc_conv1x1_dgrad_pooled_gnsums(int b, int cin, int cout, int hw, int nsample, int groups, int relu, const float *w,
+                                               const float *y, const float *coef2, const float *inj, const float *y_prev,
+                                               const float *gamma, const float *beta, const float *mean, const float *rstd,
+                                               float *grad_z, double *dsdb, ogc_stream_t stream) {
+    OGC_REQUIRE(b >= 0 && cin >= 1 && cout >= 1 && hw >= 1, "ogc_conv1x1_dgrad_pooled_gnsums: bad shape");
+    const int rc = gnb_check("ogc_conv1x1_dgrad_pooled_gnsums", b, cin, groups, y_prev, gamma, beta, mean, rstd, dsdb,
+                             (hipStream_t)stream);
+    if (rc != OGC_OK) return rc;
+    GnBwdSums gnb;
+    gnb.y = y_prev; gnb.gamma = gamma; gnb.beta = beta; gnb.mean = mean; gnb.rstd = rstd; gnb.dsdb = dsdb;
+    gnb.groups = groups; gnb.relu = relu; gnb.nb = b;
+    return dgrad_pooled_impl<float>(b, cin, cout, hw, nsample, w, y, coef2, inj, grad_z, stream, &gnb);
+}
diff --git a/ogc_amd/csrc/gn_bwd_epilogue.h b/ogc_amd/csrc/gn_bwd_epilogue.h
--- /dev/null
+++ b/ogc_amd/csrc/gn_bwd_epilogue.h
@@ -0,0 +1,57 @@
+#pragma once
+#include "ogc_common.h"
+
+constexpr int OGC_GN_BWD_SLOTS = 8;
+
+struct GnBwdSums {
+    const float *y = nullptr;
+    const float *gamma = nullptr, *beta = nullptr;
+    const float *mean = nullptr, *rstd = nullptr;
+    double *dsdb = nullptr;
+    int groups = 1, relu = 0, nb = 1;
+};
+
+__device__ __forceinline__ float2 ogc_gnb_coef(const GnBwdSums &g, int b, int m, int M) {
+    const int row = b * g.groups + m / (M / g.groups);
+    const float a = g.rstd[row] * g.gamma[m];
+    const float bb = g.beta[m] - g.mean[row] * a;
+    return make_float2(a, bb);
+}
+
+__device__ __forceinline__ void ogc_gnb_partials(float4 d, const float4 v, const float2 co, const bool relu, double &s,
+                                                 double &sb) {
+    if (relu) {
+        d.x = fmaf(co.x, v.x, co.y) > 0.f ? d.x : 0.f; d.y = fmaf(co.x, v.y, co.y) > 0.f ? d.y : 0.f;
+        d.z = fmaf(co.x, v.z, co.y) > 0.f ? d.z : 0.f; d.w = fmaf(co.x, v.w, co.y) > 0.f ? d.w : 0.f;
+    }
+    s = (double)((d.x * v.x + d.y * v.y) + (d.z * v.z + d.w * v.w));
+    sb = (double)((d.x + d.y) + (d.z + d.w));
+}
+
+template <int CTRL>
+__device__ __forceinline__ double ogc_dpp_f64(double v) {
+    const int lo = __builtin_amdgcn_update_dpp(0, __double2loint(v), CTRL, 0xF, 0xF, true);
+    const int hi = __builtin_amdgcn_update_dpp(0, __double2hiint(v), CTRL, 0xF, 0xF, true);
+    return __hiloint2double(hi, lo);
+}
+
+__device__ __forceinline__ void ogc_gnb_row_reduce(const double (&s)[4], const double (&sb)[4], int j, double (&k)[2]) {
+    const bool b0 = (j & 1) != 0, b1 = (j & 2) != 0;
+    double k1[4];
+#pragma unroll
+    for (int r = 0; r < 4; ++r) {
+        const double keep = b0 ? sb[r] : s[r], send = b0 ? s[r] : sb[r];
+        k1[r] = keep + ogc_dpp_f64<0xB1>(send);
+    }
+#pragma unroll
+    for (int h = 0; h < 2; ++h) {
+        const double keep = b1 ? k1[2 * h + 1] : k1[2 * h], send = b1 ? k1[2 * h] : k1[2 * h + 1];
+        double v = keep + ogc_dpp_f64<0x4E>(send);
+        v += ogc_dpp_f64<0x124>(v);
+        v += ogc_dpp_f64<0x128>(v);
+        k[h] = v;
+    }
+}
+
+bool ogc_gemm_stream_dgrad_gnsums_launch(int b, int M, int K, int hw, const float *w, const float *in, float *out,
+                                         const GnBwdSums &gnb, hipStream_t s);
diff --git a/ogc_amd/csrc/group_norm.hip b/ogc_amd/csrc/group_norm.hip
--- a/ogc_amd/csrc/group_norm.hip
+++ b/ogc_amd/csrc/group_norm.hip
@@ -1,5 +1,6 @@
 #include "ogc_common.h"
 #include "act_io.h"
+#include "gn_bwd_epilogue.h"
 
 namespace {
 
@@ -446,7 +447,7 @@
 }
 
 constexpr int GN_STATS_SLOTS = 32;
-constexpr int GN_BWD_SLOTS = 8;
+constexpr int GN_BWD_SLOTS = OGC_GN_BWD_SLOTS;
 
 int hw_chunks(int b, int c, int hw) {
     int chunks = 1;
@@ -594,6 +595,27 @@
                                   float *grad_x, float *grad_gamma, float *grad_beta, double *ws,
                                   ogc_stream_t stream) {
     return gn_bwd_impl<float>(b, c, hw, groups, relu, x, gamma, beta, mean, rstd, grad_y, grad_x, grad_gamma, grad_beta, ws, stream);
+}
+
+extern "C" int ogc_group_norm_bwd_dx(int b, int c, int hw, int groups, int relu, const float *x, const float *gamma,
+                                     const float *beta, const float *mean, const float *rstd, const float *grad_y,
+                                     float *grad_x, float *grad_gamma, float *grad_beta, const double *dsdb,
+                                     ogc_stream_t stream) {
+    OGC_REQUIRE(b >= 0 && c >= 1 && hw >= 1 && groups >= 1 && c % groups == 0, "ogc_group_norm_bwd_dx: bad shape");
+    if (b == 0) return OGC_OK;
+    OGC_REQUIRE(x && gamma && beta && mean && rstd && grad_y && grad_x && grad_gamma && grad_beta && dsdb,
+                "ogc_group_norm_bwd_dx: null pointer");
+    OGC_REQUIRE((long long)c * hw < (1ll << 31) && b <= 65535, "ogc_group_norm_bwd_dx: one sample exceeds 32-bit indexing");
+    hipStream_t s = (hipStream_t)stream;
+    dim3 grid(hw_chunks(b, c, hw), c, b);
+    if (relu)
+        hipLaunchKernelGGL((gn_bwd_dx_kernel<true, float>), grid, dim3(GN_THREADS), 0, s, c, hw, groups, x, gamma, beta, mean, rstd,
+                           dsdb, GN_BWD_SLOTS, grad_y, grad_x, grad_gamma, grad_beta);
+    else
+        hipLaunchKernelGGL((gn_bwd_dx_kernel<false, float>), grid, dim3(GN_THREADS), 0, s, c, hw, groups, x, gamma, beta, mean, rstd,
+                           dsdb, GN_BWD_SLOTS, grad_y, grad_x, grad_gamma, grad_beta);
+    OGC_CHECK_LAUNCH("ogc_group_norm_bwd_dx");
+    return OGC_OK;
 }
 
 extern "C" int ogc_group_norm_bwd_h(int b, int c, int hw, int groups, int relu, const ogc_bf16_t *x, const float *gamma,
diff --git a/ogc_amd/fused.py b/ogc_amd/fused.py
--- a/ogc_amd/fused.py
+++ b/ogc_amd/fused.py
@@ -670,6 +670,23 @@
 
 def _pool_moment_cout(t):
     return ACT16_MOMENT_WIDTH if t.dtype is torch.bfloat16 else max(FUSED_GN_BACKWARD_MAX_WIDTH, SPARSE_POOL_MAX_COUT)
+
+
+GN_BWD_EPILOGUE = True
+
+
+def _gn_bwd_epilogue_ok(y_prev, grad_y3, pooled):
+    nat = _api._native
+    B, cout, hw = grad_y3.shape
+    cin = y_prev.shape[1]
+    if not (GN_BWD_EPILOGUE and y_prev.dtype is torch.float32 and nat.get_matmul_precision() == "fp32" and hw % 64 == 0
+            and B <= 65535 and getattr(nat, "conv1x1_dgrad_gnsums_wrapper", None) is not None):
+        return False
+    if pooled:
+        return True
+    if nat.conv1x1_gemm_stream_supported(B, cin, cout, hw):
+        return DGRAD_STREAM and _gemm_ok(cout, hw) and cout <= 132 and B <= 128
+    return not (_gemm_ok(cout, hw) and _plain_gemm_mine(cout, (B, cin, hw))) and gemm_any_available(grad_y3)
 
 
 def _norm_act_conv_forward(y_prev, stats_prev, gn_weight, gn_bias, conv_weight, gn_groups, eps, relu, next_groups, pool,
@@ -757,6 +774,17 @@
             nat.conv1x1_dgrad_adjoint_wrapper(B, cin, cout, hw, relu, w.view(cout, cin), grad_y, y_prev, a, bb, coef, grad_prev)
             return grad_prev, None, gw, gb, grad_w.view_as(conv_weight), None, None, None, None, None, None
         nat.conv1x1_wgrad_affine_wrapper(B, cin, cout, hw, relu, y_prev, a, bb, grad_y, grad_w)
+        if _gn_bwd_epilogue_ok(y_prev, grad_y.view(B, cout, hw), False):
+            grad_z = torch.empty_like(y_prev)
+            dsdb = zeroed_empty(2 * B * cin * nat.group_norm_bwd_slots(), torch.float64, y_prev.device)
+            gamma, beta = gn_weight.contiguous(), gn_bias.contiguous()
+            nat.conv1x1_dgrad_gnsums_wrapper(B, cin, cout, hw, gn_groups, relu, w.view(cout, cin), grad_y, y_prev, gamma, beta,
+                                             mean, rstd, grad_z, dsdb)
+            grad_prev = torch.empty_like(y_prev)
+            gw, gb = torch.empty_like(gn_weight), torch.empty_like(gn_bias)
+            nat.group_norm_bwd_dx_wrapper(B, cin, hw, gn_groups, relu, y_prev, gamma, beta, mean, rstd, grad_z, grad_prev, gw, gb,
+                                          dsdb)
+            return grad_prev, None, gw, gb, grad_w.view_as(conv_weight), None, None, None, None, None, None
         if y_prev.dtype is torch.bfloat16 or (_gemm_ok(cout, hw) and _plain_gemm_mine(cout, (B, cin, hw))):
             grad_z = torch.empty_like(y_prev)
             nat.conv1x1_gemm_wrapper(B, cin, cout, hw, 1, w, grad_y, grad_z)
@@ -847,9 +875,17 @@
             grad_w = zeroed_empty((cout, cin), torch.float32, dev)
             nat.conv1x1_wgrad_affine_pooled_wrapper(B, cin, cout, hw, relu, S, y_prev, a, bb, y, coef2, inj, grad_w)
             grad_z = torch.empty_like(y_prev)
-            nat.conv1x1_dgrad_pooled_wrapper(B, cin, cout, hw, S, w, y, coef2, inj, grad_z)
             grad_prev = torch.empty_like(y_prev)
             gw, gb = torch.empty_like(gn_weight), torch.empty_like(gn_bias)
+            if _gn_bwd_epilogue_ok(y_prev, y.view(B, cout, hw), True):
+                dsdb = zeroed_empty(2 * B * cin * nat.group_norm_bwd_slots(), torch.float64, dev)
+                gamma, beta = gn_weight.contiguous(), gn_bias.contiguous()
+                nat.conv1x1_dgrad_pooled_gnsums_wrapper(B, cin, cout, hw, S, gn_groups, relu, w, y, coef2, inj, y_prev, gamma,
+                                                        beta, mean, rstd, grad_z, dsdb)
+                nat.group_norm_bwd_dx_wrapper(B, cin, hw, gn_groups, relu, y_prev, gamma, beta, mean, rstd, grad_z, grad_prev,
+                                              gw, gb, dsdb)
+                return (grad_prev, None, gw, gb, grad_w.view_as(conv_weight), None, None, None, gw2, gb2, None, None, None)
+            nat.conv1x1_dgrad_pooled_wrapper(B, cin, cout, hw, S, w, y, coef2, inj, grad_z)
             ws = nat.group_norm_ws(B, cin, gn_groups, True, dev)
             nat.group_norm_bwd_wrapper(B, cin, hw, gn_groups, relu, y_prev, gn_weight.contiguous(), gn_bias.contiguous(), mean,
                                        rstd, grad_z, grad_prev, gw, gb, ws)
diff --git a/ogc_amd/pointnet2_cuda.py b/ogc_amd/pointnet2_cuda.py
--- a/ogc_amd/pointnet2_cuda.py
+++ b/ogc_amd/pointnet2_cuda.py
@@ -404,6 +404,12 @@
          _f(grad_gamma, "grad_gamma"), _f(grad_beta, "grad_beta"), _check(ws, torch.float64, "ws"))
 
 
+def group_norm_bwd_dx_wrapper(b, c, hw, groups, relu, x, gamma, beta, mean, rstd, grad_y, grad_x, grad_gamma, grad_beta, dsdb):
+    _run("ogc_group_norm_bwd_dx", x, b, c, hw, groups, int(relu), _f(x, "x"), _f(gamma, "gamma"), _f(beta, "beta"),
+         _f(mean, "mean"), _f(rstd, "rstd"), _f(grad_y, "grad_y"), _f(grad_x, "grad_x"), _f(grad_gamma, "grad_gamma"),
+         _f(grad_beta, "grad_beta"), _check(dsdb, torch.float64, "dsdb"))
+
+
 def group_norm_maxpool_fwd_wrapper(b, c, p, s, groups, eps, relu, x, gamma, beta, out, argmax, mean, rstd, ws):
     _run("ogc_group_norm_maxpool_fwd", x, b, c, p, s, groups, float(eps), int(relu), _f(x, "x"), _f(gamma, "gamma"),
          _f(beta, "beta"), _f(out, "out"), _i(argmax, "argmax"), _f(mean, "mean"), _f(rstd, "rstd"),
@@ -625,6 +631,10 @@
     return torch.empty(max(n, 1), dtype=torch.float64, device=device)
 
 
+def group_norm_bwd_slots():
+    return _lib.load().ogc_group_norm_bwd_slots()
+
+
 _precision = "fp32"
 
 
@@ -686,6 +696,19 @@
          yp, _f(coef2, "coef2"), _f(inj, "inj"), _f(dw, "dw"))
 
 
+def conv1x1_dgrad_gnsums_wrapper(b, cin, cout, hw, groups, relu, w, grad_y, y_prev, gamma, beta, mean, rstd, grad_z, dsdb):
+    _run("ogc_conv1x1_dgrad_gnsums", grad_y, b, cin, cout, hw, groups, int(relu), _f(w, "w"), _f(grad_y, "grad_y"),
+         _f(y_prev, "y_prev"), _f(gamma, "gamma"), _f(beta, "beta"), _f(mean, "mean"), _f(rstd, "rstd"), _f(grad_z, "grad_z"),
+         _check(dsdb, torch.float64, "dsdb"))
+
+
+def conv1x1_dgrad_pooled_gnsums_wrapper(b, cin, cout, hw, nsample, groups, relu, w, y, coef2, inj, y_prev, gamma, beta, mean,
+                                        rstd, grad_z, dsdb):
+    _run("ogc_conv1x1_dgrad_pooled_gnsums", y, b, cin, cout, hw, nsample, groups, int(relu), _f(w, "w"), _f(y, "y"),
+         _f(coef2, "coef2"), _f(inj, "inj"), _f(y_prev, "y_prev"), _f(gamma, "gamma"), _f(beta, "beta"), _f(mean, "mean"),
+         _f(rstd, "rstd"), _f(grad_z, "grad_z"), _check(dsdb, torch.float64, "dsdb"))
+
+
 def conv1x1_dgrad_pooled_wrapper(b, cin, cout, hw, nsample, w, y, coef2, inj, grad_z):
     h, (yp, gp) = _acts((y, grad_z), ("y", "grad_z"))
     _run("ogc_conv1x1_dgrad_pooled" + h, y, b, cin, cout, hw, nsample, _f(w, "w"), yp, _f(coef2, "coef2"), _f(inj, "inj"), gp)
```

Measured after the change: 1588 point-clouds/s, median of 5. 1.4% higher.
